# ayotoasset/AdditiveCausalExpansion

Measured on NVIDIA B200. Metric: nadam_iters_per_sec, higher is better.
Workload: dtype f64

## Files before the change

additivecausalexpansion_b200/_lib.py:

```python
from __future__ import annotations

import ctypes as C
import os
import subprocess

_HERE = os.path.dirname(os.path.abspath(__file__))
SO_PATH = os.environ.get("ACE_B200_LIB") or os.path.join(_HERE, "libace_b200.so")
CSRC = os.path.join(_HERE, "csrc")
HEADER = os.path.join(os.path.dirname(_HERE), "include", "ace_b200.h")

c_double_p = C.POINTER(C.c_double)
c_int_p = C.POINTER(C.c_int)


class AceFitConfig(C.Structure):

    _fields_ = [
        ("kernel", C.c_int),
        ("optimizer", C.c_int),
        ("learning_rate", C.c_double),
        ("beta1", C.c_double),
        ("beta2", C.c_double),
        ("momentum", C.c_double),
        ("norm_clip", C.c_int),
        ("clip_at", C.c_double),
        ("std_y", C.c_double),
        ("device", C.c_int),
        ("use_graph", C.c_int),
    ]


def build(force: bool = False, verbose: bool = False) -> str:
    srcs = [os.path.join(CSRC, f) for f in os.listdir(CSRC) if f.endswith((".cu", ".cuh", ".inl"))] + [HEADER]
    stale = (not os.path.exists(SO_PATH)) or any(os.path.getmtime(s) > os.path.getmtime(SO_PATH) for s in srcs)
    if force or stale:
        cmd = ["make", "-j", str(min(8, os.cpu_count() or 1)), "-C", CSRC, "../libace_b200.so"] + (["-B"] if force else [])
        subprocess.check_call(cmd, stdout=None if verbose else subprocess.DEVNULL)
    return SO_PATH


_LIB = None

_d, _i, _p, _ip = C.c_double, C.c_int, c_double_p, c_int_p
_vp = C.c_void_p
SIGNATURES = {
    "ace_last_error": (C.c_char_p, []),
    "ace_version": (C.c_char_p, []),
    "ace_device_count": (_i, []),
    "ace_set_device": (_i, [_i]),
    "ace_kernmat_SE_cpp": (_i, [_p, _p, _p, _p, _i, _i, _i, _i, _p, _p, _p]),
    "ace_kernmat_Matern32_cpp": (_i, [_p, _p, _p, _p, _i, _i, _i, _i, _p, _p, _p]),
    "ace_kernmat_SE_symmetric_cpp": (_i, [_p, _p, _i, _i, _i, _p, _p, _p]),
    "ace_kernmat_Matern32_symmetric_cpp": (_i, [_p, _p, _i, _i, _i, _p, _p, _p]),
    "ace_invkernel_cpp": (_i, [_p, _i, _d, _p, _p]),
    "ace_grad_SE_cpp": (_i, [_p, _p, _p, _p, _p, _p, _p, _p, _p, C.c_uint, _d, _i, _i, _p]),
    "ace_grad_Matern_cpp": (_i, [_p, _p, _p, _p, _p, _p, _p, _p, _p, C.c_uint, _d, _i, _i, _p]),
    "ace_stats_cpp": (_i, [_p, _p, _p, _p, _d, _d, _i, _p]),
    "ace_mu_solution_cpp": (_i, [_p, _p, _i, _p]),
    "ace_pred_cpp": (_i, [_p, _d, _d, _p, _p, _p, _d, _d, _i, _i, _p, _p, _p]),
    "ace_pred_marginal_cpp": (_i, [_p, _p, _d, _d, _p, _p, _p, _d, _d, _d, _i, _i, _i, _i, _p, _p, _p, _p]),
    "ace_norm_clip_cpp": (None, [_i, _p, _i, _d]),
    "ace_Nesterov_cpp": (_i, [_d, _d, _p, _p, _p, _i]),
    "ace_Nadam_cpp": (_i, [_d, _d, _d, _d, _d, _p, _p, _p, _p, _i]),
    "ace_Adam_cpp": (_i, [_d, _d, _d, _d, _d, _p, _p, _p, _p, _i]),
    "ace_fit_default_config": (None, [C.POINTER(AceFitConfig)]),
    "ace_fit_create": (_i, [C.POINTER(_vp), _p, _p, _p, _i, _i, _i, _p, C.POINTER(AceFitConfig)]),
    "ace_fit_destroy": (_i, [_vp]),
    "ace_fit_para_update": (_i, [_vp, _i, _p, _p]),
    "ace_fit_run": (_i, [_vp, _i, _i, _d, _d, _p, _ip]),
    "ace_fit_get_train_stats": (_i, [_vp, _p]),
    "ace_comm_unique_id": (_i, [C.c_char_p]),
    "ace_shard_plan": (_i, [_i, _i, _i, _ip, _ip]),
    "ace_fit_shard": (_i, [_vp, C.c_char_p, _i, _i]),
    "ace_fit_shard_emulate": (_i, [_vp, _i]),
    "ace_dbg_shard_trace_dump": (_i, [_i]),
    "ace_fit_upload_data": (_i, [_vp, _p, _p, _p]),
    "ace_fit_kernel_launches": (_i, [_vp, _ip]),
    "ace_fit_timer_start": (_i, [_vp]),
    "ace_fit_timer_stop": (_i, [_vp, _p]),
    "ace_fit_get_parameters": (_i, [_vp, _p]),
    "ace_fit_set_parameters": (_i, [_vp, _p]),
    "ace_fit_get_gradients": (_i, [_vp, _p]),
    "ace_fit_get_optimizer_state": (_i, [_vp, _p, _p]),
    "ace_fit_get_invKmatn": (_i, [_vp, _p]),
    "ace_fit_get_alpha": (_i, [_vp, _p]),
    "ace_fit_dims": (_i, [_vp, _ip, _ip, _ip, _ip]),
    "ace_fit_last_timing": (_i, [_vp, _p]),
    "ace_fit_predict": (_i, [_vp, _p, _p, _i, _d, _d, _p, _p, _p]),
    "ace_fit_predict_marginal": (_i, [_vp, _p, _p, _p, _i, _d, _d, _d, _i, _p, _p, _p, _p]),
    "ace_fit_predict_marginal_batch": (_i, [_vp, _p, _p, _p, _i, _d, _d, _d, C.POINTER(C.c_ubyte), _i, _p, _p, _p, _p, _ip]),
    "ace_dbg_gemm_nt": (_i, [_p, _p, _p, _i, _i, _i, _d, _d, _i]),
    "ace_dbg_spd_inverse": (_i, [_p, _i, _p, _p, _p, _p]),
    "ace_dbg_spd_inverse_fused": (_i, [_p, _i, _p, _p]),
    "ace_dbg_diag_block": (_i, [_p, _i, _p, _p, _p, _p]),
    "ace_dbg_diag_block_timeline": (_i, [C.POINTER(C.c_longlong), _i]),
    "ace_bench_dense": (_i, [_i, _i, _p]),
    "ace_dbg_set_trtri_max_h": (_i, [_i]),
    "ace_dbg_trtri_raw": (_i, [_p, _i, _p, _p, _p, _p]),
    "ace_dbg_uut_engines": (_i, [_p, _i, C.POINTER(C.c_int), _i, _p, _p, _p]),
    "ace_dbg_fit_set_uut_engine": (_i, [_vp, _i]),
    "ace_ncs_basis": (_i, [_p, _i, _p, _i, _p]),
    "ace_ncs_basis_deriv": (_i, [_p, _i, _p, _i, _p]),
    "ace_normalize_train": (_i, [_p, _p, _p, _i, _i, _i, _p]),
    "ace_normalize_test": (_i, [_p, _p, _i, _i, _i, _p]),
    "ace_normalize_train_gpu": (_i, [_p, _p, _p, _i, _i, _i, _p]),
    "ace_normalize_test_gpu": (_i, [_p, _p, _i, _i, _i, _p]),
}


def lib():
    global _LIB
    if _LIB is None:
        if not os.path.exists(SO_PATH):
            raise RuntimeError(
                f"{SO_PATH} is missing: run `python -c 'import __graft_entry__ as g; g.build()'` "
                "(there is no CPU fallback for the ACE hot path)")
        L = C.CDLL(SO_PATH)
        for name, (res, args) in SIGNATURES.items():
            fn = getattr(L, name)
            fn.restype = res
            fn.argtypes = args
        _LIB = L
    return _LIB


class AceError(RuntimeError):
    def __init__(self, status: int, where: str):
        self.status = status
        msg = lib().ace_last_error()
        super().__init__(f"{where}: status {status}: {msg.decode() if msg else ''}")


class NotFiniteError(AceError, FloatingPointError):
    """The reference's stop("Some gradients are not finite, NaN, or NA. ...")."""


ACE_ERR_NOT_FINITE = 1073741824


def check(status: int, where: str) -> None:
    if status == 0:
        return
    if status == ACE_ERR_NOT_FINITE:
        raise NotFiniteError(status, where)
    raise AceError(status, where)
```

additivecausalexpansion_b200/api.py:

```python
from __future__ import annotations

import ctypes as C

import numpy as np

from ._lib import AceError, c_double_p, check, lib


def _f(a, two_d=False):
    a = np.asfortranarray(np.asarray(a, dtype=np.float64))
    if two_d and a.ndim == 1:
        a = np.asfortranarray(a.reshape(-1, 1))
    return a


def _p(a):
    return None if a is None else a.ctypes.data_as(c_double_p)


def _inplace(a, name):
    if not (isinstance(a, np.ndarray) and a.dtype == np.float64 and a.flags.c_contiguous):
        raise TypeError(f"{name} must be a C-contiguous float64 ndarray (it is updated in place)")
    return a


def _kernmat(fn, name, X1, X2, Z1, Z2, parameters, elements=True):
    X1, X2, Z1, Z2 = _f(X1, True), _f(X2, True), _f(Z1, True), _f(Z2, True)
    par = _f(parameters).ravel()
    n1, n2, p, Bz = X1.shape[0], X2.shape[0], X2.shape[1], Z1.shape[1]
    full = np.empty((n1, n2), order="F")
    el = np.empty((n1, n2, Bz + 1), order="F") if elements else None
    check(fn(_p(X1), _p(X2), _p(Z1), _p(Z2), n1, n2, p, Bz, _p(par), _p(full), _p(el)), name)
    return {"full": full, "elements": el}


def _kernmat_sym(fn, name, X, Z, parameters, elements=True):
    X, Z = _f(X, True), _f(Z, True)
    par = _f(parameters).ravel()
    n, p, Bz = X.shape[0], X.shape[1], Z.shape[1]
    full = np.empty((n, n), order="F")
    el = np.empty((n, n, Bz + 1), order="F") if elements else None
    check(fn(_p(X), _p(Z), n, p, Bz, _p(par), _p(full), _p(el)), name)
    return {"full": full, "elements": el}


def kernmat_SE_cpp(X1, X2, Z1, Z2, parameters, elements=True):
    return _kernmat(lib().ace_kernmat_SE_cpp, "kernmat_SE_cpp", X1, X2, Z1, Z2, parameters, elements)


def kernmat_SE_symmetric_cpp(X, Z, parameters, elements=True):
    return _kernmat_sym(lib().ace_kernmat_SE_symmetric_cpp, "kernmat_SE_symmetric_cpp", X, Z, parameters, elements)


def kernmat_Matern32_cpp(X1, X2, Z1, Z2, parameters, elements=True):
    return _kernmat(lib().ace_kernmat_Matern32_cpp, "kernmat_Matern32_cpp", X1, X2, Z1, Z2, parameters, elements)


def kernmat_Matern32_symmetric_cpp(X, Z, parameters, elements=True):
    return _kernmat_sym(lib().ace_kernmat_Matern32_symmetric_cpp, "kernmat_Matern32_symmetric_cpp", X, Z,
                        parameters, elements)


def invkernel_cpp(pdmat, sigma):
    K = _f(pdmat)
    n = K.shape[0]
    eig = np.empty(n)
    inv = np.empty((n, n), order="F")
    check(lib().ace_invkernel_cpp(_p(K), n, float(sigma), _p(eig), _p(inv)), "invkernel_cpp")
    return {"eigenval": eig, "inv": inv}


def _grad(fn, name, y, X, Z, Kfull, K, invKmatn, eigenval, parameters, stats, B, std_y):
    y, X, Z = _f(y).ravel(), _f(X, True), _f(Z, True)
    invKmatn, eigenval, par = _f(invKmatn), _f(eigenval).ravel(), _f(parameters).ravel()
    _inplace(stats, "stats")
    n, p = X.shape
    g = np.empty(par.size)
    check(fn(_p(y), _p(X), _p(Z), None, None, _p(invKmatn), _p(eigenval), _p(par), _p(stats), int(B), float(std_y),
             n, p, _p(g)), name)
    return g


def grad_SE_cpp(y, X, Z, Kfull, K, invKmatn, eigenval, parameters, stats, B, std_y):
    return _grad(lib().ace_grad_SE_cpp, "grad_SE_cpp", y, X, Z, Kfull, K, invKmatn, eigenval, parameters, stats, B,
                 std_y)


def grad_Matern_cpp(y, X, Z, Kfull, K, invKmatn, eigenval, parameters, stats, B, std_y):
    return _grad(lib().ace_grad_Matern_cpp, "grad_Matern_cpp", y, X, Z, Kfull, K, invKmatn, eigenval, parameters,
                 stats, B, std_y)


def stats_cpp(y, Kmat, invKmatn, eigenval, mu, std_y=1.0):
    y, Kmat, invKmatn, eigenval = _f(y).ravel(), _f(Kmat), _f(invKmatn), _f(eigenval).ravel()
    out = np.zeros(2)
    check(lib().ace_stats_cpp(_p(y), _p(Kmat), _p(invKmatn), _p(eigenval), float(mu), float(std_y), y.size, _p(out)),
          "stats_cpp")
    return out


def mu_solution_cpp(y, invKmat):
    y, invKmat = _f(y).ravel(), _f(invKmat)
    mu = C.c_double(0.0)
    check(lib().ace_mu_solution_cpp(_p(y), _p(invKmat), y.size, C.cast(C.byref(mu), c_double_p)), "mu_solution_cpp")
    return mu.value


def norm_clip_cpp(flag, grads, max_length):
    _inplace(grads, "grads")
    lib().ace_norm_clip_cpp(int(bool(flag)), _p(grads), grads.size, float(max_length))


def Nesterov_cpp(learn_rate, momentum, nu, grad, para):
    _inplace(nu, "nu"), _inplace(para, "para")
    g = np.ascontiguousarray(grad, dtype=np.float64).ravel()
    return bool(lib().ace_Nesterov_cpp(float(learn_rate), float(momentum), _p(nu), _p(g), _p(para), para.size))


def Nadam_cpp(iter, learn_rate, beta1, beta2, eps, m, v, grad, para):
    _inplace(m, "m"), _inplace(v, "v"), _inplace(para, "para")
    g = np.ascontiguousarray(grad, dtype=np.float64).ravel()
    return bool(lib().ace_Nadam_cpp(float(iter), float(learn_rate), float(beta1), float(beta2), float(eps), _p(m),
                                    _p(v), _p(g), _p(para), para.size))


def Adam_cpp(iter, learn_rate, beta1, beta2, eps, m, v, grad, para):
    _inplace(m, "m"), _inplace(v, "v"), _inplace(para, "para")
    g = np.ascontiguousarray(grad, dtype=np.float64).ravel()
    return bool(lib().ace_Adam_cpp(float(iter), float(learn_rate), float(beta1), float(beta2), float(eps), _p(m),
                                   _p(v), _p(g), _p(para), para.size))


def pred_cpp(y_X, sigma, mu, invK_XX, K_xX, K_xx, mean_y, std_y):
    y_X, invK_XX, K_xX, K_xx = _f(y_X).ravel(), _f(invK_XX), _f(K_xX, True), _f(K_xx, True)
    nx, nX = K_xX.shape
    m, ci, var = np.empty(nx), np.empty((nx, 2), order="F"), np.empty(nx)
    check(lib().ace_pred_cpp(_p(y_X), float(sigma), float(mu), _p(invK_XX), _p(K_xX), _p(K_xx), float(mean_y),
                             float(std_y), nx, nX, _p(m), _p(ci), _p(var)), "pred_cpp")
    return {"map": m, "ci": ci, "var": var}


def _avg(out, avg):
    for k, name in enumerate(("ate", "att", "atu")):
        out[name] = {"map": avg[4 * k], "ci": avg[4 * k + 1:4 * k + 3].copy(), "var": avg[4 * k + 3]}


def pred_marginal_cpp(y_X, Z_x, sigma, mu, invK_XX, K_xX, K_xx, mean_y, std_y, std_Z, calculate_ate):
    y_X, Z_x, invK_XX = _f(y_X).ravel(), _f(Z_x).ravel(), _f(invK_XX)
    K_xX, K_xx = _f(K_xX), _f(K_xx)
    nx, nX, B = K_xX.shape
    m, ci, var, avg = np.empty(nx), np.empty((nx, 2), order="F"), np.empty(nx), np.zeros(12)
    check(lib().ace_pred_marginal_cpp(_p(y_X), _p(Z_x), float(sigma), float(mu), _p(invK_XX), _p(K_xX), _p(K_xx),
                                      float(mean_y), float(std_y), float(std_Z), int(bool(calculate_ate)), nx, nX, B,
                                      _p(m), _p(ci), _p(var), _p(avg)), "pred_marginal_cpp")
    out = {"map": m, "ci": ci, "var": var}
    if calculate_ate:
        _avg(out, avg)
    return out


def ncs_basis(x, knots):
    x, knots = _f(x).ravel(), _f(knots).ravel()
    K = lib().ace_ncs_basis(_p(x), x.size, _p(knots), knots.size, None)
    check(0 if K > 0 else K, "ncs_basis")
    out = np.empty((x.size, K), order="F")
    lib().ace_ncs_basis(_p(x), x.size, _p(knots), knots.size, _p(out))
    return out


def ncs_basis_deriv(x, knots):
    x, knots = _f(x).ravel(), _f(knots).ravel()
    K = lib().ace_ncs_basis_deriv(_p(x), x.size, _p(knots), knots.size, None)
    check(0 if K > 0 else K, "ncs_basis_deriv")
    out = np.empty((x.size, K), order="F")
    lib().ace_ncs_basis_deriv(_p(x), x.size, _p(knots), knots.size, _p(out))
    return out


def normalize_train(y, X, Z, gpu=False):
    for a, nm in ((y, "y"), (X, "X"), (Z, "Z")):
        if not (isinstance(a, np.ndarray) and a.dtype == np.float64 and a.flags.f_contiguous):
            raise TypeError(f"{nm} must be a Fortran-contiguous float64 ndarray (normalised in place)")
    n, px = X.shape
    pz = Z.shape[1]
    mom = np.empty((1 + px + pz, 3), order="F")
    fn = lib().ace_normalize_train_gpu if gpu else lib().ace_normalize_train
    check(fn(_p(y), _p(X), _p(Z), n, px, pz, _p(mom)), "normalize_train")
    return mom


def normalize_test(X, Z, moments, gpu=False):
    for a, nm in ((X, "X"), (Z, "Z")):
        if not (isinstance(a, np.ndarray) and a.dtype == np.float64 and a.flags.f_contiguous):
            raise TypeError(f"{nm} must be a Fortran-contiguous float64 ndarray (normalised in place)")
    mom = _f(moments)
    fn = lib().ace_normalize_test_gpu if gpu else lib().ace_normalize_test
    check(fn(_p(X), _p(Z), X.shape[0], X.shape[1], Z.shape[1], _p(mom)), "normalize_test")


def dbg_gemm_nt(A, B, C_, alpha=1.0, beta=0.0, lower_only=False):
    A, B, Cm = _f(A), _f(B), _f(C_).copy(order="F")
    M, K = A.shape
    N = B.shape[0]
    check(lib().ace_dbg_gemm_nt(_p(A), _p(B), _p(Cm), M, N, K, float(alpha), float(beta), int(lower_only)),
          "dbg_gemm_nt")
    return Cm


def dbg_spd_inverse(A, want_L=True, want_inv=True):
    A = _f(A)
    n = A.shape[0]
    L = np.empty((n, n), order="F") if want_L else None
    inv = np.empty((n, n), order="F") if want_inv else None
    d = np.empty(n)
    ms = np.zeros(3)
    check(lib().ace_dbg_spd_inverse(_p(A), n, _p(L), _p(inv), _p(d), _p(ms)), "dbg_spd_inverse")
    return {"L": L, "inv": inv, "diagL": d, "ms": ms}


def dbg_spd_inverse_fused(A):
    A = _f(A)
    n = A.shape[0]
    inv, d = np.empty((n, n), order="F"), np.empty(n)
    check(lib().ace_dbg_spd_inverse_fused(_p(A), n, _p(inv), _p(d)), "dbg_spd_inverse_fused")
    return {"inv": inv, "diagL": d}


def dbg_uut_engines(A, engines=(1, 2), want_inv=True):
    A = _f(A)
    n = A.shape[0]
    eng = (C.c_int * len(engines))(*engines)
    ms = np.zeros(len(engines))
    inv = {e: (np.empty((n, n), order="F") if want_inv and e in engines else None) for e in (1, 2)}
    check(lib().ace_dbg_uut_engines(_p(A), n, eng, len(engines), _p(ms), _p(inv[1]), _p(inv[2])),
          "dbg_uut_engines")
    return {"ms": ms, "dmma": inv[1], "i8": inv[2]}


def dbg_diag_block(A):
    A = _f(A)
    n = A.shape[0]
    X, U, L = (np.empty((n, n), order="F") for _ in range(3))
    d = np.empty(n)
    check(lib().ace_dbg_diag_block(_p(A), n, _p(X), _p(U), _p(d), _p(L)), "dbg_diag_block")
    return {"X": X, "U": U, "diagL": d, "Ldiag": L}


def bench_dense(n, reps=1):
    ms = np.zeros(3)
    check(lib().ace_bench_dense(int(n), int(reps), _p(ms)), "bench_dense")
    return ms
```

additivecausalexpansion_b200/csrc/ace_b200.cu:

```cuda
#include "../../include/ace_b200.h"

#include <algorithm>
#include <chrono>
#include <cmath>
#include <cstdlib>
#include <cstring>
#include <mutex>
#include <new>
#include <string>
#include <vector>

#include "chol.cuh"
#include "nccl_dyn.h"
#include "shard_dense.cuh"
#include "gp_kernels.cuh"
#include "pair_kernels.cuh"
#include "grad2_kernel.cuh"
#include "grad3_kernel.cuh"
#include "kernmat2_kernel.cuh"
#include "pred_kernels.cuh"
#include "prep_kernels.cuh"

namespace ace {

static thread_local std::string g_err;
void set_error(const std::string& msg) { g_err = msg; }

static int usage(const std::string& m) {
  set_error(m);
  return ACE_ERR_USAGE;
}

static inline int round_up(int x, int m) { return (x + m - 1) / m * m; }

template <typename T>
struct DBuf {
  T* p = nullptr;
  size_t count = 0;
  DBuf() = default;
  DBuf(const DBuf&) = delete;
  DBuf& operator=(const DBuf&) = delete;
  ~DBuf() { release(); }
  int alloc(size_t n) {
    release();
    if (n == 0) n = 1;
    cudaError_t e = cudaMalloc(&p, n * sizeof(T));
    if (e != cudaSuccess) {
      p = nullptr;
      set_error(std::string("cudaMalloc of ") + std::to_string(n * sizeof(T)) + " bytes: " + cudaGetErrorString(e));
      return -(int)e - 1000;
    }
    count = n;
    return 0;
  }
  void release() {
    if (p) cudaFree(p);
    p = nullptr;
    count = 0;
  }
};

static int check_device() {
  int cnt = 0;
  cudaError_t e = cudaGetDeviceCount(&cnt);
  if (e != cudaSuccess || cnt <= 0) {
    set_error(std::string("no CUDA device available (") + cudaGetErrorString(e) +
              "); this library has no CPU fallback");
    return ACE_ERR_NO_DEVICE;
  }
  return 0;
}

static int configure_kernels_once() {
  static std::mutex mu;
  static std::vector<int> done;
  int dev = 0;
  ACE_CUDA(cudaGetDevice(&dev));
  std::lock_guard<std::mutex> lk(mu);
  if (std::find(done.begin(), done.end(), dev) != done.end()) return 0;
  ACE_TRY(configure_dense_kernels());
  done.push_back(dev);
  return 0;
}

static int upload_matrix(double* dst, long ld_dev, int rows_pad, const double* src, int rows, int cols,
                         cudaStream_t st) {
  ACE_CUDA(cudaMemsetAsync(dst, 0, sizeof(double) * (size_t)ld_dev * (size_t)std::max(cols, 1), st));
  (void)rows_pad;
  if (rows > 0 && cols > 0)
    ACE_CUDA(cudaMemcpy2DAsync(dst, sizeof(double) * ld_dev, src, sizeof(double) * rows, sizeof(double) * rows,
                               cols, cudaMemcpyHostToDevice, st));
  return 0;
}

static int download_matrix(double* dst, int rows, int cols, const double* src, long ld_dev, cudaStream_t st) {
  if (rows > 0 && cols > 0)
    ACE_CUDA(cudaMemcpy2DAsync(dst, sizeof(double) * rows, src, sizeof(double) * ld_dev, sizeof(double) * rows,
                               cols, cudaMemcpyDeviceToHost, st));
  return 0;
}

__global__ void pad_identity_kernel(double* A, long ld, int n, int n_pad) {
  const int i = n + blockIdx.x * blockDim.x + threadIdx.x;
  if (i < n_pad) A[i + (size_t)i * ld] = 1.0;
}

__global__ void add_diag_kernel(double* A, long ld, int n, double v) {
  const int i = blockIdx.x * blockDim.x + threadIdx.x;
  if (i < n) A[i + (size_t)i * ld] += v;
}

__global__ void synth_spd_kernel(double* A, long ld, int n) {
  const size_t idx = (size_t)blockIdx.x * blockDim.x + threadIdx.x;
  if (idx >= (size_t)n * n) return;
  const int i = (int)(idx % n), j = (int)(idx / n);
  const double t = 8.0 * (double)(i - j) / (double)n;
  A[i + (size_t)j * ld] = exp(-t * t) + (i == j ? 0.5 : 0.0);
}

struct ConstChain {
  std::mutex mu;
  cudaEvent_t ev = nullptr;
  bool recorded = false;
};
static ConstChain& const_chain(int which, int dev) {
  static ConstChain chains[2][64];
  return chains[which][dev & 63];
}
template <class F>
static int with_const_chain(int which, cudaStream_t st, F&& launch) {
  int dev = 0;
  ACE_CUDA(cudaGetDevice(&dev));
  ConstChain& ch = const_chain(which, dev);
  std::lock_guard<std::mutex> lk(ch.mu);
  if (ch.ev == nullptr) ACE_CUDA(cudaEventCreateWithFlags(&ch.ev, cudaEventDisableTiming));
  cudaStreamCaptureStatus cs = cudaStreamCaptureStatusNone;
  ACE_CUDA(cudaStreamIsCapturing(st, &cs));
  const bool cap = cs != cudaStreamCaptureStatusNone;
  if (ch.recorded) ACE_CUDA(cudaStreamWaitEvent(st, ch.ev, cap ? cudaEventWaitExternal : cudaEventWaitDefault));
  ACE_TRY(launch());
  ACE_CUDA(cudaEventRecordWithFlags(ch.ev, st, cap ? cudaEventRecordExternal : cudaEventRecordDefault));
  ch.recorded = true;
  return 0;
}

int launch_kernmat2_k0(const KernArgs&, unsigned, size_t, cudaStream_t);
int launch_kernmat2_k1(const KernArgs&, unsigned, size_t, cudaStream_t);

static int launch_kernmat(const KernArgs& a, int kind, cudaStream_t st) {
  const int B = a.B;
  if (B < 1 || B > BMAXT || a.p < 1 || a.p > PMAX) {
    set_error("kernel build supports 1 <= p <= 64 and B = Bz+1 <= 32");
    return ACE_ERR_UNSUPPORTED;
  }
  const size_t smem = kb::smem_bytes(a.p, B - 1, a.sym != 0);
  if (smem > 227 * 1024) {
    set_error("kernel build: p and Bz too large for one shared-memory tile");
    return ACE_ERR_UNSUPPORTED;
  }
  unsigned grid;
  if (a.sym) {
    const long T = a.n1_pad / kb::T;
    grid = (unsigned)(T * (T + 1) / 2);
  } else {
    grid = (unsigned)((a.n1_pad / kb::T) * (a.n2_pad / kb::T));
  }
  static const int impl = [] {
    const char* e = std::getenv("ACE_KERNMAT_IMPL");
    return e ? std::atoi(e) : 2;
  }();
  if (impl == 2 && B <= G3_LAM && a.p <= G3_PD) {
    const size_t smem2 = kb2::smem_bytes(a.p, B - 1, a.sym != 0);
    return with_const_chain(1, st, [&]() -> int {
      return kind == 0 ? launch_kernmat2_k0(a, grid, smem2, st) : launch_kernmat2_k1(a, grid, smem2, st);
    });
  }
  auto go = [&](auto kern) -> int {
    ACE_CUDA(cudaFuncSetAttribute(kern, cudaFuncAttributeMaxDynamicSharedMemorySize, (int)smem));
    kern<<<grid, 256, smem, st>>>(a);
    return 0;
  };
  const int bc = kb::chunk_terms(B);
  if (kind == 0) {
    if (bc == 4) ACE_TRY(go(kernmat_kernel<0, 4, 4>));
    else if (bc == 8) ACE_TRY(go(kernmat_kernel<0, 8, 2>));
    else ACE_TRY(go(kernmat_kernel<0, 12, 2>));
  } else {
    if (bc == 4) ACE_TRY(go(kernmat_kernel<1, 4, 4>));
    else if (bc == 8) ACE_TRY(go(kernmat_kernel<1, 8, 2>));
    else ACE_TRY(go(kernmat_kernel<1, 12, 2>));
  }
  ACE_CUDA(cudaGetLastError());
  return 0;
}

struct GradPlan {
  int PD = 0, BT = 0, groups = 0, gy = 0, threads = 0, gx = 0;
  size_t smem = 0;
  int v2 = 0, PD8 = 0, BD8 = 0;
  int nw2 = 8;
  int cw3 = 1;
  int v3 = 0, NT3 = 0;
};

int launch_grad3_k0_nt1(const GradArgs&, int, size_t, int, cudaStream_t);
int launch_grad3_k0_nt2(const GradArgs&, int, size_t, int, cudaStream_t);
int launch_grad3_k0_nt3(const GradArgs&, int, size_t, int, cudaStream_t);
int launch_grad3_k0_nt4(const GradArgs&, int, size_t, int, cudaStream_t);
int launch_grad3_k1_nt1(const GradArgs&, int, size_t, int, cudaStream_t);
int launch_grad3_k1_nt2(const GradArgs&, int, size_t, int, cudaStream_t);
int launch_grad3_k1_nt3(const GradArgs&, int, size_t, int, cudaStream_t);
int launch_grad3_k1_nt4(const GradArgs&, int, size_t, int, cudaStream_t);

static int plan_grad(int p, int B, int kind, int sms, GradPlan* pl) {
  static const int table[][2] = {{4, 16}, {8, 8}, {12, 5}, {16, 4}, {20, 3}, {24, 2}, {32, 2}, {48, 1}, {64, 1}};
  for (auto& t : table) {
    if (p <= t[0]) {
      pl->PD = t[0];
      pl->BT = t[1];
      break;
    }
  }
  if (pl->PD == 0 || B > BMAXT) {
    set_error("gradient pass supports p <= 64 and B <= 32");
    return ACE_ERR_UNSUPPORTED;
  }
  int gpc_max = gk::GROUPS_PER_CTA;
  if (pl->PD == 20) {
    if (const char* e = std::getenv("ACE_GRAD_BT")) pl->BT = (std::atoi(e) == 2) ? 2 : 3;
  }
  if (const char* e = std::getenv("ACE_GRAD_GPC")) gpc_max = std::max(1, std::min(4, std::atoi(e)));
  pl->groups = (B + pl->BT - 1) / pl->BT;
  const int gpc = std::min(pl->groups, gpc_max);
  pl->gy = (pl->groups + gpc - 1) / gpc;
  pl->threads = 64 * gpc;
  pl->smem = gk::smem_bytes(pl->PD, B - 1, pl->BT, kind);
  if (pl->smem > 227 * 1024) {
    set_error("gradient pass: p and Bz too large for one shared-memory tile");
    return ACE_ERR_UNSUPPORTED;
  }
  pl->gx = 2 * sms;
  const int PD8 = (p + 7) / 8 * 8, BD8 = (B + 7) / 8 * 8;
  const char* impl = std::getenv("ACE_GRAD_IMPL");
  const int want = impl ? std::atoi(impl) : 3;
  const bool want2 = want >= 2;
  if (want == 3 && p <= 32 && B <= 16) {
    const int NT = (p + 7) / 8;
    const size_t sm3 = g3::smem_bytes(NT, B, kind, 16);
    if (sm3 <= 227 * 1024) {
      pl->v3 = 1; pl->NT3 = NT; pl->smem = sm3; pl->gy = 1; pl->threads = 512;
      if (const char* e = std::getenv("ACE_GRAD3_CW")) pl->cw3 = std::atoi(e) != 0;
      return 0;
    }
  }
  if (PD8 <= 32 && BD8 <= 16 && want2) {
    int nw = 16;
    if (const char* e = std::getenv("ACE_GRAD2_WARPS")) nw = (std::atoi(e) == 8) ? 8 : 16;
    size_t sm2 = g2::smem_bytes(PD8, BD8, B - 1, nw, kind);
    if (sm2 > 227 * 1024 && nw == 16) {
      nw = 8;
      sm2 = g2::smem_bytes(PD8, BD8, B - 1, nw, kind);
    }
    if (sm2 <= 227 * 1024) {
      pl->v2 = 1; pl->PD8 = PD8; pl->BD8 = BD8; pl->smem = sm2; pl->gy = 1; pl->threads = 32 * nw; pl->nw2 = nw;
    }
  }
  return 0;
}

template <int PD8, int BD8, int KIND, int NW>
static int launch_grad2_k(const GradArgs& a, const GradPlan& pl, cudaStream_t st) {
  ACE_CUDA(cudaFuncSetAttribute(grad2_kernel<PD8, BD8, KIND, NW>, cudaFuncAttributeMaxDynamicSharedMemorySize, (int)pl.smem));
  grad2_kernel<PD8, BD8, KIND, NW><<<pl.gx, NW * 32, pl.smem, st>>>(a);
  ACE_CUDA(cudaGetLastError());
  return 0;
}

template <int PD8, int BD8>
static int launch_grad2_t(const GradArgs& a, int kind, const GradPlan& pl, cudaStream_t st) {
  if (pl.nw2 == 16) return kind == 0 ? launch_grad2_k<PD8, BD8, 0, 16>(a, pl, st) : launch_grad2_k<PD8, BD8, 1, 16>(a, pl, st);
  return kind == 0 ? launch_grad2_k<PD8, BD8, 0, 8>(a, pl, st) : launch_grad2_k<PD8, BD8, 1, 8>(a, pl, st);
}

static int launch_grad2(const GradArgs& a, int kind, const GradPlan& pl, cudaStream_t st) {
  const int key = pl.PD8 * 100 + pl.BD8;
  switch (key) {
    case 808: return launch_grad2_t<8, 8>(a, kind, pl, st);
    case 816: return launch_grad2_t<8, 16>(a, kind, pl, st);
    case 1608: return launch_grad2_t<16, 8>(a, kind, pl, st);
    case 1616: return launch_grad2_t<16, 16>(a, kind, pl, st);
    case 2408: return launch_grad2_t<24, 8>(a, kind, pl, st);
    case 2416: return launch_grad2_t<24, 16>(a, kind, pl, st);
    case 3208: return launch_grad2_t<32, 8>(a, kind, pl, st);
    default: return launch_grad2_t<32, 16>(a, kind, pl, st);
  }
}

template <int PD, int BT>
static int launch_grad_t(const GradArgs& a, int kind, const GradPlan& pl, cudaStream_t st) {
  dim3 grid(pl.gx, pl.gy);
  if (kind == 0) {
    ACE_CUDA(cudaFuncSetAttribute(grad_kernel<PD, BT, 0>, cudaFuncAttributeMaxDynamicSharedMemorySize, (int)pl.smem));
    grad_kernel<PD, BT, 0><<<grid, pl.threads, pl.smem, st>>>(a);
  } else {
    ACE_CUDA(cudaFuncSetAttribute(grad_kernel<PD, BT, 1>, cudaFuncAttributeMaxDynamicSharedMemorySize, (int)pl.smem));
    grad_kernel<PD, BT, 1><<<grid, pl.threads, pl.smem, st>>>(a);
  }
  ACE_CUDA(cudaGetLastError());
  return 0;
}

static int launch_grad2(const GradArgs& a, int kind, const GradPlan& pl, cudaStream_t st);

static int launch_grad(const GradArgs& a, int kind, const GradPlan& pl, cudaStream_t st) {
  if (pl.v3) {
    auto go = [&](int cw) -> int {
      switch (kind * 10 + pl.NT3) {
        case 1: return launch_grad3_k0_nt1(a, pl.gx, pl.smem, cw, st);
        case 2: return launch_grad3_k0_nt2(a, pl.gx, pl.smem, cw, st);
        case 3: return launch_grad3_k0_nt3(a, pl.gx, pl.smem, cw, st);
        case 4: return launch_grad3_k0_nt4(a, pl.gx, pl.smem, cw, st);
        case 11: return launch_grad3_k1_nt1(a, pl.gx, pl.smem, cw, st);
        case 12: return launch_grad3_k1_nt2(a, pl.gx, pl.smem, cw, st);
        case 13: return launch_grad3_k1_nt3(a, pl.gx, pl.smem, cw, st);
        default: return launch_grad3_k1_nt4(a, pl.gx, pl.smem, cw, st);
      }
    };
    if (!pl.cw3) return go(0);
    return with_const_chain(0, st, [&]() -> int { return go(1); });
  }
  if (pl.v2) return launch_grad2(a, kind, pl, st);
  switch (pl.PD) {
    case 4: return launch_grad_t<4, 16>(a, kind, pl, st);
    case 8: return launch_grad_t<8, 8>(a, kind, pl, st);
    case 12: return launch_grad_t<12, 5>(a, kind, pl, st);
    case 16: return launch_grad_t<16, 4>(a, kind, pl, st);
    case 20: return pl.BT == 2 ? launch_grad_t<20, 2>(a, kind, pl, st) : launch_grad_t<20, 3>(a, kind, pl, st);
    case 24: return launch_grad_t<24, 2>(a, kind, pl, st);
    case 32: return launch_grad_t<32, 2>(a, kind, pl, st);
    case 48: return launch_grad_t<48, 1>(a, kind, pl, st);
    default: return launch_grad_t<64, 1>(a, kind, pl, st);
  }
}

struct Core {
  int device = 0, sms = 148;
  int n = 0, n_pad = 0, p = 0, Bz = 0, B = 0, P = 0, kind = 0;
  cudaStream_t st = nullptr, side = nullptr, aux = nullptr, bgst = nullptr;
  cudaEvent_t ev[8] = {nullptr, nullptr, nullptr, nullptr, nullptr, nullptr, nullptr, nullptr};
  DBuf<double> Wp0, Wp1, Wsmall;
  DBuf<double> diag_ws;
  DBuf<int8_t> oz_planes;
  DBuf<unsigned long long> oz_rowmax;
  DBuf<int> oz_ex;
  int uut_engine = 0;
  int panel_blocks = 4;
  cudaEvent_t tev[8] = {};
  DBuf<double> X, Z, LZ, y, theta, m, v, grad, tab, sc, A, Bf, DX, DU, dvec, alpha, uvec, svec, Ka, pu, ps, partials;
  DBuf<int> info;
  double* h_sc = nullptr;
  GradPlan gp;
  int nchunks = 0;
  int shard_rank = 0, shard_world = 1;
  DBuf<double> red;
  double* ka() { return red.p ? red.p + P : Ka.p; }
  bool shard_dense = false;
  bool shard_emulate = false;
  int shard_hmin = 16;
  bool kinv_partial = false;
  bool u_valid = false;
  DBuf<double> tvy, tv1, pdg, kdg;
  bool shard_incr = true;
  bool shard_potrf = false;
  std::vector<cudaEvent_t> shard_events;
  DBuf<double> head0, head1;
  cudaStream_t bulk = nullptr;
  int rank_lo() const { return shard_emulate ? 0 : shard_rank; }
  int rank_hi() const { return shard_emulate ? shard_world : shard_rank + 1; }
  DBuf<double> chain_ws;
  DBuf<double> mid0, mid1;
  cudaStream_t mids = nullptr;
  ShardCtx shard_ctx(ncclComm_t comm, ncclComm_t comm2, ncclComm_t comm3 = nullptr) const {
    ShardCtx cx;
    cx.rank = shard_rank; cx.world = shard_world; cx.emulate = shard_emulate; cx.comm = comm; cx.h_min = shard_hmin;
    cx.comm2 = comm2;
    cx.events = const_cast<cudaEvent_t*>(shard_events.data());
    cx.head[0] = head0.p; cx.head[1] = head1.p; cx.bulk_stream = bulk;
    cx.chain_ws = chain_ws.p;
    cx.comm3 = comm3; cx.mid[0] = mid0.p; cx.mid[1] = mid1.p; cx.mid_stream = mids;
    cx.incr = shard_incr;
    return cx;
  }
  int alloc_shard() {
    ACE_TRY(red.alloc((size_t)P + n_pad));
    ACE_CUDA(cudaMemsetAsync(red.p, 0, sizeof(double) * ((size_t)P + n_pad), st));
    const char* e = std::getenv("ACE_SHARD_DENSE");
    shard_dense = e ? (std::atoi(e) != 0) : true;
    if (const char* h = std::getenv("ACE_SHARD_HMIN")) shard_hmin = std::max(1, std::atoi(h));
    if (shard_dense) {
      const char* sp = std::getenv("ACE_SHARD_POTRF");
      const bool pow2 = (panel_blocks & (panel_blocks - 1)) == 0;
      if ((sp ? std::atoi(sp) != 0 : true) && pow2 && panel_blocks >= 2) {
        const size_t N = (size_t)n_pad;
        if (!Wp0.p) {
          ACE_TRY(Wp0.alloc(N * panel_blocks * TB));
          ACE_TRY(Wp1.alloc(N * panel_blocks * TB));
          ACE_TRY(Wsmall.alloc((size_t)(panel_blocks * TB / 2) * (panel_blocks * TB / 2)));
        }
        const size_t pw = (size_t)panel_blocks * TB;
        ACE_TRY(head0.alloc(2 * pw * pw));
        ACE_TRY(head1.alloc(2 * pw * pw));
        if (!bulk) {
          int lo = 0, hi = 0;
          ACE_CUDA(cudaDeviceGetStreamPriorityRange(&lo, &hi));
          int pb_ = (hi + lo) / 2;
          if (const char* e = std::getenv("ACE_SHARD_BULK_PRIO")) pb_ = std::max(hi, std::min(lo, std::atoi(e)));
          ACE_CUDA(cudaStreamCreateWithPriority(&bulk, cudaStreamNonBlocking, pb_));
        }
        {
          const char* sk = std::getenv("ACE_SHARD_SPLITK");
          if (!(sk && std::atoi(sk) == 0)) ACE_TRY(chain_ws.alloc(4 * pw * pw));
        }
        {
          const char* sm = std::getenv("ACE_SHARD_MID");
          if (!(sm && std::atoi(sm) == 0)) {
            ACE_TRY(mid0.alloc(pw * pw));
            ACE_TRY(mid1.alloc(pw * pw));
            if (!mids) {
              int lo = 0, hi = 0;
              ACE_CUDA(cudaDeviceGetStreamPriorityRange(&lo, &hi));
              ACE_CUDA(cudaStreamCreateWithPriority(&mids, cudaStreamNonBlocking, std::min(lo, hi + 1)));
            }
          }
        }
        const int NP = shard_panels(n_pad / TB, panel_blocks);
        while ((int)shard_events.size() < SHARD_EVENT_KINDS * NP) {
          cudaEvent_t e;
          ACE_CUDA(cudaEventCreateWithFlags(&e, cudaEventDisableTiming));
          shard_events.push_back(e);
        }
        shard_potrf = true;
        {
          const double nn = (double)n_pad;
          const double chain_s = NP * 0.85e-3, update_s = nn * nn * nn / (3.0 * shard_world * 3.5e13);
          shard_incr = 2.0 * chain_s >= update_s;
        }
        if (const char* si = std::getenv("ACE_SHARD_INCR")) shard_incr = std::atoi(si) != 0;
      }
    }
    return 0;
  }
  int ensure_full_inverse() {
    if (!kinv_partial) return 0;
    DenseWork w = dense(A.p, Bf.p);
    ACE_TRY(uut_inverse(w));
    kinv_partial = false;
    return 0;
  }

  ~Core() {
    if (h_sc) cudaFreeHost(h_sc);
    for (auto& e : ev)
      if (e) cudaEventDestroy(e);
    for (auto& e : tev)
      if (e) cudaEventDestroy(e);
    for (auto& e : shard_events) cudaEventDestroy(e);
    if (bulk) cudaStreamDestroy(bulk);
    if (mids) cudaStreamDestroy(mids);
    if (st) cudaStreamDestroy(st);
    if (side) cudaStreamDestroy(side);
    if (aux) cudaStreamDestroy(aux);
    if (bgst) cudaStreamDestroy(bgst);
  }

  int init(int dev, int n_, int p_, int Bz_, int kind_, bool need_dense, bool need_grad) {
    ACE_TRY(check_device());
    device = dev;
    ACE_CUDA(cudaSetDevice(dev));
    ACE_TRY(configure_kernels_once());
    cudaDeviceProp prop;
    ACE_CUDA(cudaGetDeviceProperties(&prop, dev));
    if (prop.major < 10) {
      set_error("this library is built for sm_100a (B200) only");
      return ACE_ERR_NO_DEVICE;
    }
    sms = prop.multiProcessorCount;
    n = n_; p = p_; Bz = Bz_; B = Bz_ + 1; P = 2 + B + B * p; kind = kind_;
    n_pad = round_up(n, TB);
    ACE_CUDA(cudaStreamCreateWithFlags(&st, cudaStreamNonBlocking));
    int lo = 0, hi = 0;
    ACE_CUDA(cudaDeviceGetStreamPriorityRange(&lo, &hi));
    ACE_CUDA(cudaStreamCreateWithPriority(&side, cudaStreamNonBlocking, hi));
    ACE_CUDA(cudaStreamCreateWithPriority(&aux, cudaStreamNonBlocking, lo));
    ACE_CUDA(cudaStreamCreateWithPriority(&bgst, cudaStreamNonBlocking, lo));
    for (auto& e : ev) ACE_CUDA(cudaEventCreateWithFlags(&e, cudaEventDisableTiming));
    for (auto& e : tev) ACE_CUDA(cudaEventCreate(&e));
    ACE_CUDA(cudaMallocHost(&h_sc, sizeof(double) * (SC_COUNT + 2)));
    const size_t N = (size_t)n_pad;
    ACE_TRY(X.alloc(N * p));
    ACE_TRY(Z.alloc(N * std::max(Bz, 1)));
    ACE_TRY(LZ.alloc(N * std::max(Bz, 1)));
    ACE_TRY(y.alloc(N));
    ACE_TRY(theta.alloc(P));
    ACE_TRY(m.alloc(P));
    ACE_TRY(v.alloc(P));
    ACE_TRY(grad.alloc(P));
    ACE_TRY(tab.alloc(TAB_SIZE));
    ACE_TRY(sc.alloc(SC_COUNT));
    ACE_TRY(info.alloc(1));
    ACE_CUDA(cudaMemsetAsync(sc.p, 0, sizeof(double) * SC_COUNT, st));
    ACE_CUDA(cudaMemsetAsync(m.p, 0, sizeof(double) * P, st));
    ACE_CUDA(cudaMemsetAsync(v.p, 0, sizeof(double) * P, st));
    ACE_CUDA(cudaMemsetAsync(grad.p, 0, sizeof(double) * P, st));
    ACE_CUDA(cudaMemsetAsync(info.p, 0, sizeof(int), st));
    if (need_dense) {
      ACE_TRY(A.alloc(N * N));
      ACE_TRY(Bf.alloc(N * N));
      ACE_TRY(DX.alloc(N * TB));
      ACE_TRY(DU.alloc(N * TB));
      ACE_TRY(dvec.alloc(N));
      if (const char* e = std::getenv("ACE_PANEL_BLOCKS")) {
        const int v = std::atoi(e);
        if (v >= 1 && v <= 64) panel_blocks = v;
      }
      const char* fu = std::getenv("ACE_FUSED_TRSM");
      const bool pow2 = (panel_blocks & (panel_blocks - 1)) == 0;
      const bool want = fu ? (std::atoi(fu) != 0) : true;
      ACE_TRY(alloc_uut_engine());
      if (pow2 && panel_blocks >= 2 && want) {
        ACE_TRY(Wp0.alloc(N * panel_blocks * TB));
        ACE_TRY(Wp1.alloc(N * panel_blocks * TB));
        ACE_TRY(Wsmall.alloc((size_t)(panel_blocks * TB / 2) * (panel_blocks * TB / 2)));
        const char* df = std::getenv("ACE_DIAG_FUSED");
        if (!(df && std::atoi(df) == 0)) ACE_TRY(diag_ws.alloc(dg::ws_doubles(panel_blocks)));
      }
    }
    if (need_grad) {
      ACE_TRY(plan_grad(p, B, kind, sms, &gp));
      nchunks = (n + gv::CHUNK - 1) / gv::CHUNK;
      ACE_TRY(alpha.alloc(N));
      ACE_TRY(uvec.alloc(N));
      ACE_TRY(svec.alloc(N));
      ACE_TRY(Ka.alloc(N));
      ACE_TRY(pu.alloc(N * nchunks));
      ACE_TRY(ps.alloc(N * nchunks));
      ACE_TRY(partials.alloc((size_t)gp.gx * gp.gy * P));
      if (!dvec.p) ACE_TRY(dvec.alloc(N));
      ACE_TRY(tvy.alloc(N));
      ACE_TRY(tv1.alloc(N));
      ACE_TRY(pdg.alloc(N * nchunks));
      ACE_TRY(kdg.alloc(N));
    }
    return 0;
  }

  int alloc_uut_engine() {
    if (uut_engine == 2 && n_pad > oz::MAX_N) {
      set_error("the INT8 U U^T engine covers n_pad <= " + std::to_string(oz::MAX_N) + " (INT32 accumulator bound)");
      return ACE_ERR_UNSUPPORTED;
    }
    if (!uut_uses_i8(n_pad, uut_engine)) {
      oz_planes.release();
      oz_rowmax.release();
      oz_ex.release();
      return 0;
    }
    if (oz_planes.p) return 0;
    ACE_TRY(oz_planes.alloc(oz::plane_bytes(n_pad / TB)));
    ACE_TRY(oz_rowmax.alloc(n_pad));
    ACE_TRY(oz_ex.alloc(n_pad));
    return 0;
  }

  int upload_data(const double* hy, const double* hX, const double* hZ) {
    if (hX) ACE_TRY(upload_matrix(X.p, n_pad, n_pad, hX, n, p, st));
    if (hZ) {
      ACE_TRY(upload_matrix(Z.p, n_pad, n_pad, hZ, n, Bz, st));
      const size_t cnt = (size_t)n_pad * Bz;
      if (cnt) logabs_kernel<<<(unsigned)((cnt + 255) / 256), 256, 0, st>>>(Z.p, LZ.p, cnt);
      ACE_CUDA(cudaGetLastError());
    }
    if (hy) ACE_TRY(upload_matrix(y.p, n_pad, n_pad, hy, n, 1, st));
    return 0;
  }

  int upload_theta(const double* hpar) {
    ACE_CUDA(cudaMemcpyAsync(theta.p, hpar, sizeof(double) * P, cudaMemcpyHostToDevice, st));
    return 0;
  }

  DenseWork dense(double* Abuf, double* Bbuf, bool allow_fused = true) {
    DenseWork w;
    w.panel_blocks = panel_blocks;
    if (allow_fused && Wp0.p) {
      w.Wp[0] = Wp0.p; w.Wp[1] = Wp1.p; w.Wsmall = Wsmall.p; w.ev_copy[0] = ev[6]; w.ev_copy[1] = ev[7];
      w.diag_ws = diag_ws.p;
    }
    w.A = Abuf; w.ld = n_pad; w.nb = n_pad / TB; w.DX = DX.p; w.DU = DU.p; w.dvec = dvec.p; w.info = info.p;
    w.Bf = Bbuf; w.main = st; w.side = side; w.aux = aux; w.bg = bgst; w.ev_half = ev[4]; w.ev_aux = ev[5];
    w.ev_panel[0] = ev[0]; w.ev_panel[1] = ev[1]; w.ev_upd[0] = ev[2]; w.ev_upd[1] = ev[3];
    w.oz.planes = oz_planes.p; w.oz.rowmax = oz_rowmax.p; w.oz.ex = oz_ex.p; w.uut_engine = uut_engine;

    return w;
  }

  int enqueue_prep() {
    prep_tables_kernel<<<1, 256, 0, st>>>(theta.p, p, B, tab.p);
    ACE_CUDA(cudaGetLastError());
    return 0;
  }

  int enqueue_build_sym(double* out, int add_noise, double* cube, long cube_slice) {
    KernArgs a{};
    a.X1 = a.X2 = X.p; a.Z1 = a.Z2 = Z.p; a.LZ1 = a.LZ2 = LZ.p; a.ld1 = a.ld2 = n_pad;
    a.n1 = a.n2 = n; a.n1_pad = a.n2_pad = n_pad; a.p = p; a.B = B; a.tab = tab.p;
    a.K = out; a.ldk = n_pad; a.cube = cube; a.cube_slice = cube_slice;
    a.sym = 1; a.add_noise = add_noise; a.pad_identity = add_noise;
    return launch_kernmat(a, kind, st);
  }

  int enqueue_build_blocks(double* out) {
    const int w = shard_block_width(n_pad, shard_world);
    for (int blk = 0; blk < 2 * shard_world; ++blk) {
      const int owner = shard_block_owner(blk, shard_world);
      if (owner < rank_lo() || owner >= rank_hi()) continue;
      const int c0 = blk * w, r0 = c0;
      KernArgs a{};
      a.X1 = X.p + r0; a.Z1 = Z.p + r0; a.LZ1 = LZ.p + r0; a.ld1 = n_pad;
      a.X2 = X.p + c0; a.Z2 = Z.p + c0; a.LZ2 = LZ.p + c0; a.ld2 = n_pad;
      a.n1 = std::max(0, n - r0); a.n2 = std::max(0, std::min(w, n - c0));
      a.n1_pad = n_pad - r0; a.n2_pad = w; a.p = p; a.B = B; a.tab = tab.p;
      a.K = out + r0 + (size_t)c0 * n_pad; a.ldk = n_pad;
      a.sym = 0; a.add_noise = 1; a.pad_identity = 1; a.row_off = r0; a.col_off = c0;
      ACE_TRY(launch_kernmat(a, kind, st));
    }
    return 0;
  }

  int enqueue_build_panels(double* out) {
    const int nb = n_pad / TB, NP = shard_panels(nb, panel_blocks);
    for (int c = 0; c < NP; ++c) {
      if (!(shard_emulate || c % shard_world == shard_rank)) continue;
      const int c0 = c * panel_blocks * TB, w = std::min(panel_blocks * TB, n_pad - c0), r0 = c0;
      KernArgs a{};
      a.X1 = X.p + r0; a.Z1 = Z.p + r0; a.LZ1 = LZ.p + r0; a.ld1 = n_pad;
      a.X2 = X.p + c0; a.Z2 = Z.p + c0; a.LZ2 = LZ.p + c0; a.ld2 = n_pad;
      a.n1 = std::max(0, n - r0); a.n2 = std::max(0, std::min(w, n - c0));
      a.n1_pad = n_pad - r0; a.n2_pad = w; a.p = p; a.B = B; a.tab = tab.p;
      a.K = out + r0 + (size_t)c0 * n_pad; a.ldk = n_pad;
      a.sym = 0; a.add_noise = 1; a.pad_identity = 1; a.row_off = r0; a.col_off = c0;
      ACE_TRY(launch_kernmat(a, kind, st));
    }
    return 0;
  }

  int enqueue_alpha(const double* Kinv, int set_mu_first_iter) {
    dim3 grid((n_pad + gv::ROWS - 1) / gv::ROWS, nchunks);
    gemv2_kernel<<<grid, gv::ROWS, 0, st>>>(Kinv, n_pad, n, y.p, pu.p, ps.p, n_pad);
    ACE_CUDA(cudaGetLastError());
    alpha_kernel<<<1, 1024, 0, st>>>(pu.p, ps.p, nchunks, n, n_pad, theta.p, uvec.p, svec.p, alpha.p, ka(), sc.p,
                                     set_mu_first_iter);
    ACE_CUDA(cudaGetLastError());
    return 0;
  }

  int enqueue_alpha_tri(const double* Afac, int set_mu_first_iter, const double* DUfac = nullptr) {
    if (!DUfac) DUfac = DU.p;
    utv2_kernel<<<(n_pad + 7) / 8, 256, 0, st>>>(Afac, n_pad, DUfac, n, n_pad, y.p, tvy.p, tv1.p);
    ACE_CUDA(cudaGetLastError());
    dim3 grid((n_pad + gv::ROWS - 1) / gv::ROWS, nchunks);
    uv2_kernel<<<grid, gv::ROWS, 0, st>>>(Afac, n_pad, DUfac, n_pad, tvy.p, tv1.p, pu.p, ps.p, pdg.p);
    ACE_CUDA(cudaGetLastError());
    alpha_kernel<<<1, 1024, 0, st>>>(pu.p, ps.p, nchunks, n, n_pad, theta.p, uvec.p, svec.p, alpha.p, ka(), sc.p,
                                     set_mu_first_iter, pdg.p, kdg.p);
    ACE_CUDA(cudaGetLastError());
    return 0;
  }

  bool alpha_from_factor() const { return uut_uses_i8(n_pad, uut_engine); }
  int enqueue_alpha_any(const double* Afac, int set_mu_first_iter, const double* DUfac = nullptr,
                        const double* Kinv = nullptr) {
    if (alpha_from_factor()) return enqueue_alpha_tri(Afac, set_mu_first_iter, DUfac);
    return enqueue_alpha(Kinv ? Kinv : Bf.p, set_mu_first_iter);
  }

  int enqueue_grad(const double* Kinv, int tile_rank = 0, int tile_world = 1, int tile_mode = 0) {
    GradArgs g{};
    g.X = X.p; g.Z = Z.p; g.LZ = LZ.p; g.ldx = n_pad; g.Kinv = Kinv; g.ld = n_pad; g.alpha = alpha.p; g.Ka = ka();
    g.tab = tab.p; g.partials = partials.p; g.n = n; g.p = p; g.B = B; g.P = P;
    g.ntiles_side = (n + gk::T - 1) / gk::T;
    g.tile_rank = tile_rank; g.tile_world = tile_world; g.tile_mode = tile_mode; g.gemm_rows = n_pad / TB;
    return launch_grad(g, kind, gp, st);
  }

  int enqueue_finalize(const double* Kinv, const ace_fit_config& c, int do_update, bool reduced = false,
                       const double* kdiag = nullptr, const double* dvec_alt = nullptr) {
    FinalizeArgs f{};
    f.partials = partials.p; f.nparts = gp.gx * gp.gy; f.y = y.p; f.alpha = alpha.p; f.Ka = ka();
    f.dvec = dvec_alt ? dvec_alt : dvec.p;
    if (reduced) {
      f.partials = red.p;
      f.nparts = 1;
    }
    f.kdiag = kdiag;
    f.Kinv = Kinv; f.ld = n_pad; f.tab = tab.p; f.theta = theta.p; f.m = m.p; f.v = v.p; f.grad = grad.p; f.sc = sc.p;
    f.n = n; f.p = p; f.B = B; f.P = P; f.kind = kind; f.optimizer = c.optimizer; f.lr = c.learning_rate;
    f.beta1 = c.beta1; f.beta2 = c.beta2; f.eps = 1e-8; f.momentum = c.momentum; f.std_y = c.std_y;
    f.clip_at = c.clip_at; f.norm_clip = c.norm_clip; f.do_update = do_update;
    finalize_kernel<<<1, 1024, 0, st>>>(f);
    ACE_CUDA(cudaGetLastError());
    return 0;
  }

  int fetch_scalars() {
    ACE_CUDA(cudaMemcpyAsync(h_sc, sc.p, sizeof(double) * SC_COUNT, cudaMemcpyDeviceToHost, st));
    ACE_CUDA(cudaMemcpyAsync(h_sc + SC_COUNT, info.p, sizeof(int), cudaMemcpyDeviceToHost, st));
    ACE_CUDA(cudaStreamSynchronize(st));
    return 0;
  }
  int h_info() const { return *reinterpret_cast<const int*>(h_sc + SC_COUNT); }
};

}

using namespace ace;

struct ace_fit {
  Core c;
  ace_fit_config cfg;
  cudaEvent_t sw0 = nullptr, sw1 = nullptr;
  int launches = -1;
  cudaGraph_t graph = nullptr;
  cudaGraphExec_t gexec = nullptr;
  double iter_dev = 0.0;
  double ms[6] = {0, 0, 0, 0, 0, 0};
  ncclComm_t comm = nullptr, comm2 = nullptr, comm3 = nullptr;
  ~ace_fit() {
    if (comm2 && nccl_api().ok) nccl_api().CommDestroy(comm2);
    if (comm3 && nccl_api().ok) nccl_api().CommDestroy(comm3);
    if (comm && nccl_api().ok) nccl_api().CommDestroy(comm);
    if (sw0) cudaEventDestroy(sw0);
    if (sw1) cudaEventDestroy(sw1);
    if (gexec) cudaGraphExecDestroy(gexec);
    if (graph) cudaGraphDestroy(graph);
  }
};

static int enqueue_iteration(ace_fit* f, bool timed) {
  Core& c = f->c;
  DenseWork w = c.dense(c.A.p, c.Bf.p);
  if (timed) ACE_CUDA(cudaEventRecord(c.tev[0], c.st));
  ACE_TRY(c.enqueue_prep());
  const bool sharded = c.shard_world > 1;
  const bool comm = sharded && !c.shard_emulate;
  const bool spotrf = sharded && c.shard_dense && c.shard_potrf;
  if (!sharded) {
    ACE_TRY(c.enqueue_build_sym(c.A.p, 1, nullptr, 0));
  } else if (spotrf) {
    ACE_TRY(c.enqueue_build_panels(c.A.p));
  } else {
    ACE_TRY(c.enqueue_build_blocks(c.A.p));
    if (comm) {
      NcclApi& nc = nccl_api();
      const int wdt = shard_block_width(c.n_pad, c.shard_world);
      const size_t cnt = (size_t)wdt * c.n_pad;
      ACE_NCCL(nc.GroupStart());
      for (int blk = 0; blk < 2 * c.shard_world; ++blk) {
        double* ptr = c.A.p + (size_t)blk * cnt;
        ACE_NCCL(nc.Broadcast(ptr, ptr, cnt, ncclFloat64, shard_block_owner(blk, c.shard_world), f->comm, c.st));
      }
      ACE_NCCL(nc.GroupEnd());
    }
  }
  if (timed) ACE_CUDA(cudaEventRecord(c.tev[1], c.st));
  const bool sdense = sharded && c.shard_dense;
  if (!sdense) {
    ACE_TRY(potrf_trtri(w));
    if (timed) ACE_CUDA(cudaEventRecord(c.tev[2], c.st));
    if (timed) ACE_CUDA(cudaEventRecord(c.tev[3], c.st));
    ACE_TRY(uut_inverse(w));
    if (timed) ACE_CUDA(cudaEventRecord(c.tev[4], c.st));
    ACE_TRY(c.enqueue_alpha_any(c.A.p, 1));
  } else {
    const ShardCtx cx = c.shard_ctx(f->comm, f->comm2, f->comm3);
    if (spotrf) {
      static const bool host_time = std::getenv("ACE_SHARD_HOSTTIME") != nullptr;
      const auto h0 = std::chrono::steady_clock::now();
      ACE_TRY(potrf_sharded(w, cx));
      if (host_time)
        std::fprintf(stderr, "[rank %d] potrf_sharded: host enqueue %.3f ms\n", c.shard_rank,
                     std::chrono::duration<double, std::milli>(std::chrono::steady_clock::now() - h0).count());
    } else {
      const int s = potrf_blocked(w);
      if (s < 0) return s;
    }
    if (timed) ACE_CUDA(cudaEventRecord(c.tev[2], c.st));
    if (spotrf && cx.incr)
      ACE_TRY(gather_inverse_sharded(w, cx));
    else
      ACE_TRY(trtri_merge_sharded(w, cx));
    if (timed) ACE_CUDA(cudaEventRecord(c.tev[3], c.st));
    ACE_TRY(uut_inverse_sharded(w, cx));
    if (timed) ACE_CUDA(cudaEventRecord(c.tev[4], c.st));
    ACE_TRY(c.enqueue_alpha_tri(c.A.p, 1));
  }
  if (!sharded) {
    ACE_TRY(c.enqueue_grad(c.Bf.p));
  } else {
    for (int r = c.rank_lo(); r < c.rank_hi(); ++r) {
      ACE_TRY(c.enqueue_grad(c.Bf.p, r, c.shard_world, sdense ? 1 : 0));
      partials_reduce_kernel<<<1, 1024, 0, c.st>>>(c.partials.p, c.gp.gx * c.gp.gy, c.P, c.red.p, r > c.rank_lo());
      ACE_CUDA(cudaGetLastError());
    }
    if (comm)
      ACE_NCCL(nccl_api().AllReduce(c.red.p, c.red.p, (size_t)c.P + c.n_pad, ncclFloat64, ncclSum, f->comm, c.st));
  }
  ACE_TRY(c.enqueue_finalize(c.Bf.p, f->cfg, 1, sharded, (sdense || c.alpha_from_factor()) ? c.kdg.p : nullptr));
  if (timed) ACE_CUDA(cudaEventRecord(c.tev[5], c.st));
  return 0;
}

extern "C" {

const char* ace_last_error(void) { return g_err.c_str(); }
const char* ace_version(void) { return "ace_b200 0.1 (sm_100a; FP64 DMMA; TMA bulk)"; }

int ace_device_count(void) {
  int cnt = 0;
  if (cudaGetDeviceCount(&cnt) != cudaSuccess) {
    cudaGetLastError();
    return 0;
  }
  return cnt;
}

static thread_local int g_device = 0;
int ace_set_device(int device) {
  ACE_TRY(check_device());
  ACE_CUDA(cudaSetDevice(device));
  g_device = device;
  return 0;
}

void ace_fit_default_config(ace_fit_config* cfg) {
  cfg->kernel = ACE_KERNEL_SE;
  cfg->optimizer = ACE_OPT_NADAM;
  cfg->learning_rate = 0.01;
  cfg->beta1 = 0.9;
  cfg->beta2 = 0.999;
  cfg->momentum = 0.0;
  cfg->norm_clip = 1;
  cfg->clip_at = 1.0;
  cfg->std_y = 1.0;
  cfg->device = 0;
  cfg->use_graph = 1;
}

int ace_fit_create(ace_fit** out, const double* y, const double* X, const double* Z, int n, int p, int Bz,
                   const double* parameters, const ace_fit_config* cfg) {
  if (!out || !y || !X || (Bz > 0 && !Z) || !parameters || !cfg) return usage("ace_fit_create: null argument");
  if (n < 1 || p < 1 || Bz < 0) return usage("ace_fit_create: need n >= 1, p >= 1, Bz >= 0");
  *out = nullptr;
  ace_fit* f = new (std::nothrow) ace_fit();
  if (!f) return usage("out of host memory");
  f->cfg = *cfg;
  int s = f->c.init(cfg->device, n, p, Bz, cfg->kernel, true, true);
  if (s == 0) s = f->c.upload_data(y, X, Z);
  if (s == 0) s = f->c.upload_theta(parameters);
  if (s == 0) {
    cudaError_t e = cudaStreamSynchronize(f->c.st);
    if (e != cudaSuccess) {
      set_error(std::string("ace_fit_create: ") + cudaGetErrorString(e));
      s = -(int)e - 1000;
    }
  }
  if (s != 0) {
    delete f;
    return s;
  }
  *out = f;
  return 0;
}

int ace_fit_destroy(ace_fit* fit) {
  if (!fit) return 0;
  cudaSetDevice(fit->c.device);
  cudaDeviceSynchronize();
  delete fit;
  return 0;
}

int ace_fit_para_update(ace_fit* f, int iter, double* stats, double* gnorm) {
  if (!f) return usage("null handle");
  Core& c = f->c;
  ACE_CUDA(cudaSetDevice(c.device));
  if ((double)iter != f->iter_dev) {
    c.h_sc[SC_COUNT + 1] = (double)iter;
    ACE_CUDA(cudaMemcpyAsync(c.sc.p + SC_ITER, c.h_sc + SC_COUNT + 1, sizeof(double), cudaMemcpyHostToDevice, c.st));
    f->iter_dev = (double)iter;
  }
  const bool use_graph = f->cfg.use_graph && !(c.shard_world > 1 && !c.shard_emulate);
  if (use_graph) {
    if (!f->gexec) {
      ACE_CUDA(cudaStreamBeginCapture(c.st, cudaStreamCaptureModeThreadLocal));
      int s = enqueue_iteration(f, false);
      cudaGraph_t g = nullptr;
      cudaError_t e = cudaStreamEndCapture(c.st, &g);
      if (s != 0) {
        if (g) cudaGraphDestroy(g);
        return s;
      }
      ACE_CUDA(e);
      f->graph = g;
      ACE_CUDA(cudaGraphInstantiate(&f->gexec, f->graph, 0));
    }
    ACE_CUDA(cudaEventRecord(c.tev[6], c.st));
    ACE_CUDA(cudaGraphLaunch(f->gexec, c.st));
    ACE_CUDA(cudaEventRecord(c.tev[7], c.st));
  } else {
    ACE_CUDA(cudaEventRecord(c.tev[6], c.st));
    ACE_TRY(enqueue_iteration(f, true));
    ACE_CUDA(cudaEventRecord(c.tev[7], c.st));
  }
  c.u_valid = true;
  c.kinv_partial = c.shard_world > 1 && c.shard_dense && !c.shard_emulate;
  ACE_TRY(c.fetch_scalars());
  f->iter_dev = c.h_sc[SC_ITER];
  float t = 0;
  ACE_CUDA(cudaEventElapsedTime(&t, c.tev[6], c.tev[7]));
  f->ms[5] = t;
  if (!use_graph) {
    for (int k = 0; k < 5; ++k) {
      ACE_CUDA(cudaEventElapsedTime(&t, c.tev[k], c.tev[k + 1]));
      f->ms[k] = t;
    }
  }
  if (stats) {
    stats[0] = c.h_sc[SC_RMSE];
    stats[1] = c.h_sc[SC_EVID];
  }
  if (gnorm) *gnorm = c.h_sc[SC_GNORM];
  if (c.h_info() > 0) {
    set_error("matrix not positive definite at pivot " + std::to_string(c.h_info()));
    return c.h_info();
  }
  if (c.h_sc[SC_FINITE] == 0.0) {
    set_error("Some gradients are not finite, NaN, or NA. Often this is due to too large learning rates.");
    return ACE_ERR_NOT_FINITE;
  }
  return 0;
}

int ace_fit_run(ace_fit* f, int iter_start, int max_iter, double tol, double prev_evidence, double* stats_out,
                int* iters_done) {
  if (!f || !iters_done) return usage("null argument");
  double prev = prev_evidence;
  int done = 0;
  for (int k = 0; k < max_iter; ++k) {
    const int iter = iter_start + k;
    double st[2];
    int s = ace_fit_para_update(f, iter, st, nullptr);
    if (s != 0) {
      *iters_done = done;
      return s;
    }
    ++done;
    if (stats_out) {
      stats_out[2 * k] = st[0];
      stats_out[2 * k + 1] = st[1];
    }
    const double change = std::fabs(st[1] - prev);
    prev = st[1];
    if (change < tol && iter > 3) break;
  }
  *iters_done = done;
  return 0;
}

int ace_dbg_fit_set_uut_engine(ace_fit* f, int engine) {
  if (!f) return usage("null handle");
  if (engine < 0 || engine > 2) return usage("dbg_fit_set_uut_engine: engine must be 0 (by size), 1 (DMMA) or 2 (INT8)");
  Core& c = f->c;
  ACE_CUDA(cudaSetDevice(c.device));
  ACE_CUDA(cudaStreamSynchronize(c.st));
  c.uut_engine = engine;
  ACE_TRY(c.alloc_uut_engine());
  if (f->gexec) cudaGraphExecDestroy(f->gexec);
  if (f->graph) cudaGraphDestroy(f->graph);
  f->gexec = nullptr;
  f->graph = nullptr;
  return 0;
}

int ace_fit_get_train_stats(ace_fit* f, double* stats) {
  if (!f || !stats) return usage("null argument");
  Core& c = f->c;
  ACE_CUDA(cudaSetDevice(c.device));
  DBuf<double> B2, DX2, DU2, dv2;
  ACE_TRY(B2.alloc((size_t)c.n_pad * c.n_pad));
  double* Fac = c.Bf.p;
  DenseWork w = c.dense(Fac, B2.p);
  if (c.u_valid) {
    ACE_TRY(DX2.alloc((size_t)c.n_pad * TB));
    ACE_TRY(DU2.alloc((size_t)c.n_pad * TB));
    ACE_TRY(dv2.alloc(c.n_pad));
    w.DX = DX2.p; w.DU = DU2.p; w.dvec = dv2.p;
    c.kinv_partial = true;
  } else {
    Fac = c.A.p;
    w = c.dense(Fac, B2.p);
  }
  ACE_TRY(c.enqueue_prep());
  ACE_TRY(c.enqueue_build_sym(Fac, 1, nullptr, 0));
  ACE_TRY(spd_inverse(w));
  ACE_TRY(c.enqueue_alpha_any(Fac, 0, w.DU, B2.p));
  ACE_TRY(c.enqueue_grad(B2.p));
  ACE_TRY(c.enqueue_finalize(B2.p, f->cfg, 0, false, c.alpha_from_factor() ? c.kdg.p : nullptr, w.dvec));
  ACE_TRY(c.fetch_scalars());
  stats[0] = c.h_sc[SC_RMSE];
  stats[1] = c.h_sc[SC_EVID];
  if (c.h_info() > 0) return c.h_info();
  return 0;
}

int ace_comm_unique_id(char* id128) {
  if (!id128) return usage("null argument");
  NcclApi& nc = nccl_api();
  if (!nc.ok) {
    set_error(nc.why);
    return ACE_ERR_UNSUPPORTED;
  }
  ncclUniqueId id;
  ACE_NCCL(nc.GetUniqueId(&id));
  static_assert(sizeof(id) == 128, "ncclUniqueId is 128 bytes");
  std::memcpy(id128, &id, 128);
  return 0;
}

int ace_shard_plan(int n, int world, int rank, int* blocks2, int* width) {
  if (!blocks2 || !width || world < 1 || rank < 0 || rank >= world) return usage("ace_shard_plan: bad argument");
  const int n_pad = round_up(n, TB);
  *width = shard_block_width(n_pad, world);
  if (*width == 0) {
    set_error("sharding needs ceil(n/128)*128 divisible by 128*world");
    return ACE_ERR_UNSUPPORTED;
  }
  blocks2[0] = rank;
  blocks2[1] = 2 * world - 1 - rank;
  return 0;
}

int ace_fit_shard(ace_fit* f, const char* id128, int rank, int world) {
  if (!f || !id128 || world < 1 || rank < 0 || rank >= world) return usage("ace_fit_shard: bad argument");
  if (world == 1) return 0;
  Core& c = f->c;
  ACE_CUDA(cudaSetDevice(c.device));
  if (shard_block_width(c.n_pad, world) == 0) {
    set_error("sharding needs ceil(n/128)*128 divisible by 128*world");
    return ACE_ERR_UNSUPPORTED;
  }
  NcclApi& nc = nccl_api();
  if (!nc.ok) {
    set_error(nc.why);
    return ACE_ERR_UNSUPPORTED;
  }
  ncclUniqueId id;
  std::memcpy(&id, id128, 128);
  ACE_NCCL(nc.CommInitRank(&f->comm, world, id, rank));
  {
    ncclUniqueId id2;
    DBuf<double> box;
    ACE_TRY(box.alloc(16));
    if (rank == 0) {
      ACE_NCCL(nc.GetUniqueId(&id2));
      ACE_CUDA(cudaMemcpyAsync(box.p, &id2, 128, cudaMemcpyHostToDevice, c.st));
    }
    ACE_NCCL(nc.Broadcast(box.p, box.p, 16, ncclFloat64, 0, f->comm, c.st));
    ACE_CUDA(cudaMemcpyAsync(&id2, box.p, 128, cudaMemcpyDeviceToHost, c.st));
    ACE_CUDA(cudaStreamSynchronize(c.st));
    ACE_NCCL(nc.CommInitRank(&f->comm2, world, id2, rank));
  }
  {
    ncclUniqueId id3;
    DBuf<double> box;
    ACE_TRY(box.alloc(16));
    if (rank == 0) {
      ACE_NCCL(nc.GetUniqueId(&id3));
      ACE_CUDA(cudaMemcpyAsync(box.p, &id3, 128, cudaMemcpyHostToDevice, c.st));
    }
    ACE_NCCL(nc.Broadcast(box.p, box.p, 16, ncclFloat64, 0, f->comm, c.st));
    ACE_CUDA(cudaMemcpyAsync(&id3, box.p, 128, cudaMemcpyDeviceToHost, c.st));
    ACE_CUDA(cudaStreamSynchronize(c.st));
    ACE_NCCL(nc.CommInitRank(&f->comm3, world, id3, rank));
  }
  c.shard_rank = rank;
  c.shard_world = world;
  ACE_TRY(c.alloc_shard());
  if (f->gexec) {
    cudaGraphExecDestroy(f->gexec);
    cudaGraphDestroy(f->graph);
    f->gexec = nullptr;
    f->graph = nullptr;
  }
  f->launches = -1;
  return 0;
}

int ace_fit_shard_emulate(ace_fit* f, int world) {
  if (!f || world < 1) return usage("ace_fit_shard_emulate: bad argument");
  Core& c = f->c;
  if (world == 1) return 0;
  ACE_CUDA(cudaSetDevice(c.device));
  if (shard_block_width(c.n_pad, world) == 0) {
    set_error("sharding needs ceil(n/128)*128 divisible by 128*world");
    return ACE_ERR_UNSUPPORTED;
  }
  c.shard_rank = 0;
  c.shard_world = world;
  c.shard_emulate = true;
  ACE_TRY(c.alloc_shard());
  if (f->gexec) {
    cudaGraphExecDestroy(f->gexec);
    cudaGraphDestroy(f->graph);
    f->gexec = nullptr;
    f->graph = nullptr;
  }
  f->launches = -1;
  return 0;
}

int ace_dbg_shard_trace_dump(int rank) {
  shard_trace_dump(rank);
  return 0;
}

int ace_fit_upload_data(ace_fit* f, const double* y, const double* X, const double* Z) {
  if (!f) return usage("null handle");
  ACE_CUDA(cudaSetDevice(f->c.device));
  return f->c.upload_data(y, X, Z);
}

static int count_kernel_nodes(cudaGraph_t g, int* out) {
  size_t nn = 0;
  ACE_CUDA(cudaGraphGetNodes(g, nullptr, &nn));
  std::vector<cudaGraphNode_t> nodes(nn);
  if (nn) ACE_CUDA(cudaGraphGetNodes(g, nodes.data(), &nn));
  int k = 0;
  for (size_t i = 0; i < nn; ++i) {
    cudaGraphNodeType t;
    ACE_CUDA(cudaGraphNodeGetType(nodes[i], &t));
    if (t == cudaGraphNodeTypeKernel) ++k;
  }
  *out = k;
  return 0;
}

int ace_fit_kernel_launches(ace_fit* f, int* launches) {
  if (!f || !launches) return usage("null argument");
  Core& c = f->c;
  ACE_CUDA(cudaSetDevice(c.device));
  if (f->launches < 0) {
    if (f->graph) {
      ACE_TRY(count_kernel_nodes(f->graph, &f->launches));
    } else {
      ACE_CUDA(cudaStreamBeginCapture(c.st, cudaStreamCaptureModeThreadLocal));
      int s = enqueue_iteration(f, false);
      cudaGraph_t g = nullptr;
      cudaError_t e = cudaStreamEndCapture(c.st, &g);
      if (s != 0 || e != cudaSuccess) {
        if (g) cudaGraphDestroy(g);
        return s != 0 ? s : -(int)e - 1000;
      }
      s = count_kernel_nodes(g, &f->launches);
      cudaGraphDestroy(g);
      ACE_TRY(s);
    }
  }
  *launches = f->launches;
  return 0;
}

int ace_fit_timer_start(ace_fit* f) {
  if (!f) return usage("null handle");
  ACE_CUDA(cudaSetDevice(f->c.device));
  if (!f->sw0) {
    ACE_CUDA(cudaEventCreate(&f->sw0));
    ACE_CUDA(cudaEventCreate(&f->sw1));
  }
  ACE_CUDA(cudaEventRecord(f->sw0, f->c.st));
  return 0;
}

int ace_fit_timer_stop(ace_fit* f, double* ms) {
  if (!f || !ms || !f->sw0) return usage("timer not started");
  ACE_CUDA(cudaSetDevice(f->c.device));
  ACE_CUDA(cudaEventRecord(f->sw1, f->c.st));
  ACE_CUDA(cudaEventSynchronize(f->sw1));
  float t = 0;
  ACE_CUDA(cudaEventElapsedTime(&t, f->sw0, f->sw1));
  *ms = t;
  return 0;
}

int ace_fit_get_parameters(ace_fit* f, double* par) {
  if (!f || !par) return usage("null argument");
  ACE_CUDA(cudaSetDevice(f->c.device));
  ACE_CUDA(cudaMemcpyAsync(par, f->c.theta.p, sizeof(double) * f->c.P, cudaMemcpyDeviceToHost, f->c.st));
  ACE_CUDA(cudaStreamSynchronize(f->c.st));
  return 0;
}

int ace_fit_set_parameters(ace_fit* f, const double* par) {
  if (!f || !par) return usage("null argument");
  ACE_CUDA(cudaSetDevice(f->c.device));
  ACE_TRY(f->c.upload_theta(par));
  ACE_CUDA(cudaStreamSynchronize(f->c.st));
  return 0;
}

int ace_fit_get_gradients(ace_fit* f, double* g) {
  if (!f || !g) return usage("null argument");
  ACE_CUDA(cudaSetDevice(f->c.device));
  ACE_CUDA(cudaMemcpyAsync(g, f->c.grad.p, sizeof(double) * f->c.P, cudaMemcpyDeviceToHost, f->c.st));
  ACE_CUDA(cudaStreamSynchronize(f->c.st));
  return 0;
}

int ace_fit_get_optimizer_state(ace_fit* f, double* m, double* v) {
  if (!f) return usage("null argument");
  ACE_CUDA(cudaSetDevice(f->c.device));
  if (m) ACE_CUDA(cudaMemcpyAsync(m, f->c.m.p, sizeof(double) * f->c.P, cudaMemcpyDeviceToHost, f->c.st));
  if (v) ACE_CUDA(cudaMemcpyAsync(v, f->c.v.p, sizeof(double) * f->c.P, cudaMemcpyDeviceToHost, f->c.st));
  ACE_CUDA(cudaStreamSynchronize(f->c.st));
  return 0;
}

int ace_fit_get_invKmatn(ace_fit* f, double* inv) {
  if (!f || !inv) return usage("null argument");
  ACE_CUDA(cudaSetDevice(f->c.device));
  ACE_TRY(f->c.ensure_full_inverse());
  ACE_TRY(download_matrix(inv, f->c.n, f->c.n, f->c.Bf.p, f->c.n_pad, f->c.st));
  ACE_CUDA(cudaStreamSynchronize(f->c.st));
  return 0;
}

int ace_fit_get_alpha(ace_fit* f, double* a) {
  if (!f || !a) return usage("null argument");
  ACE_CUDA(cudaSetDevice(f->c.device));
  ACE_CUDA(cudaMemcpyAsync(a, f->c.alpha.p, sizeof(double) * f->c.n, cudaMemcpyDeviceToHost, f->c.st));
  ACE_CUDA(cudaStreamSynchronize(f->c.st));
  return 0;
}

int ace_fit_dims(ace_fit* f, int* n, int* p, int* B, int* P) {
  if (!f) return usage("null argument");
  if (n) *n = f->c.n;
  if (p) *p = f->c.p;
  if (B) *B = f->c.B;
  if (P) *P = f->c.P;
  return 0;
}

int ace_fit_last_timing(ace_fit* f, double* ms6) {
  if (!f || !ms6) return usage("null argument");
  for (int k = 0; k < 6; ++k) ms6[k] = f->ms[k];
  return 0;
}

}

namespace ace {

struct PostOut {
  DBuf<double> T, map, var, p1, p2;
};

static int posterior_rows(Core& c, const double* Kinv, const double* Kx, const double* kdiag, int nx, int nx_pad,
                          double mu, double noise, PostOut& o) {
  const int n = c.n, n_pad = c.n_pad;
  ACE_TRY(o.T.alloc((size_t)nx_pad * n_pad));
  GemmNT g{};
  g.A = Kx; g.lda = nx_pad; g.B = Kinv; g.ldb = n_pad; g.C = o.T.p; g.ldc = nx_pad;
  g.M = nx_pad; g.N = n_pad; g.K = n_pad; g.alpha = 1.0; g.beta = 0.0;
  ACE_TRY(launch_gemm_nt(g, c.st));
  const int chunks = (n + pk::CHUNK - 1) / pk::CHUNK;
  ACE_TRY(o.p1.alloc((size_t)nx_pad * chunks));
  ACE_TRY(o.p2.alloc((size_t)nx_pad * chunks));
  ACE_TRY(o.map.alloc(nx_pad));
  ACE_TRY(o.var.alloc(nx_pad));
  dim3 grid((nx_pad + pk::ROWS - 1) / pk::ROWS, chunks);
  rowdot2_kernel<<<grid, pk::ROWS, 0, c.st>>>(o.T.p, Kx, nx_pad, nx_pad, n, c.y.p, mu, o.p1.p, o.p2.p);
  ACE_CUDA(cudaGetLastError());
  post_finish_kernel<<<(nx_pad + 255) / 256, 256, 0, c.st>>>(o.p1.p, o.p2.p, chunks, nx, nx_pad, kdiag, noise,
                                                            o.map.p, o.var.p);
  ACE_CUDA(cudaGetLastError());
  return 0;
}

static int posterior_rows_tri(Core& c, const double* Kx, const double* kdiag, int nx, int nx_pad, double mu,
                              double noise, PostOut& o) {
  const int n = c.n, n_pad = c.n_pad;
  ACE_TRY(o.T.alloc((size_t)nx_pad * n_pad));
  GemmNT g{};
  g.A = Kx; g.lda = nx_pad; g.B = c.A.p; g.ldb = n_pad; g.b_tri = 2; g.Bdiag = c.DX.p;
  g.C = o.T.p; g.ldc = nx_pad;
  g.M = nx_pad; g.N = n_pad; g.K = n_pad; g.alpha = 1.0; g.beta = 0.0;
  ACE_TRY(launch_gemm_nt(g, c.st));
  utv2_kernel<<<(n_pad + 7) / 8, 256, 0, c.st>>>(c.A.p, n_pad, c.DU.p, n, n_pad, c.y.p, c.tvy.p, c.tv1.p);
  ACE_CUDA(cudaGetLastError());
  const int chunks = (n + pk::CHUNK - 1) / pk::CHUNK;
  ACE_TRY(o.p1.alloc((size_t)nx_pad * chunks));
  ACE_TRY(o.p2.alloc((size_t)nx_pad * chunks));
  ACE_TRY(o.map.alloc(nx_pad));
  ACE_TRY(o.var.alloc(nx_pad));
  dim3 grid((nx_pad + pk::ROWS - 1) / pk::ROWS, chunks);
  rowdot_tri_kernel<<<grid, pk::ROWS, 0, c.st>>>(o.T.p, nx_pad, nx_pad, n, c.tvy.p, c.tv1.p, mu, o.p1.p, o.p2.p);
  ACE_CUDA(cudaGetLastError());
  post_finish_kernel<<<(nx_pad + 255) / 256, 256, 0, c.st>>>(o.p1.p, o.p2.p, chunks, nx, nx_pad, kdiag, noise,
                                                            o.map.p, o.var.p);
  ACE_CUDA(cudaGetLastError());
  return 0;
}

}

extern "C" {

int ace_fit_predict(ace_fit* f, const double* X2, const double* Z2, int nx, double mean_y, double std_y,
                    double* map, double* ci, double* var) {
  if (!f || !X2 || (f->c.Bz > 0 && !Z2) || !map || !ci || !var || nx < 1) return usage("ace_fit_predict: bad argument");
  Core& c = f->c;
  ACE_CUDA(cudaSetDevice(c.device));
  const bool split = c.shard_world > 1 && !c.shard_emulate && c.u_valid && f->comm != nullptr;
  const int G = split ? c.shard_world : 1, r = split ? c.shard_rank : 0;
  const int chunk = round_up((nx + G - 1) / G, TB);
  const int nx_all = chunk * G;
  const int lo = r * chunk, cnt = std::max(0, std::min(nx, lo + chunk) - lo);
  DBuf<double> dX2, dZ2, dLZ2, Kx, kd, res;
  ACE_TRY(dX2.alloc((size_t)nx_all * c.p));
  ACE_TRY(dZ2.alloc((size_t)nx_all * std::max(c.Bz, 1)));
  ACE_TRY(dLZ2.alloc((size_t)nx_all * std::max(c.Bz, 1)));
  ACE_TRY(Kx.alloc((size_t)chunk * c.n_pad));
  ACE_TRY(kd.alloc(chunk));
  ACE_TRY(res.alloc((size_t)2 * nx_all));
  ACE_TRY(upload_matrix(dX2.p, nx_all, nx_all, X2, nx, c.p, c.st));
  ACE_TRY(upload_matrix(dZ2.p, nx_all, nx_all, Z2, nx, c.Bz, c.st));
  if (c.Bz > 0)
    logabs_kernel<<<(unsigned)(((size_t)nx_all * c.Bz + 255) / 256), 256, 0, c.st>>>(dZ2.p, dLZ2.p, (size_t)nx_all * c.Bz);
  ACE_CUDA(cudaGetLastError());
  ACE_TRY(c.enqueue_prep());
  KernArgs a{};
  a.X1 = dX2.p + lo; a.Z1 = dZ2.p + lo; a.LZ1 = dLZ2.p + lo; a.ld1 = nx_all;
  a.X2 = c.X.p; a.Z2 = c.Z.p; a.LZ2 = c.LZ.p; a.ld2 = c.n_pad;
  a.n1 = cnt; a.n2 = c.n; a.n1_pad = chunk; a.n2_pad = c.n_pad; a.p = c.p; a.B = c.B; a.tab = c.tab.p;
  a.K = Kx.p; a.ldk = chunk;
  ACE_TRY(launch_kernmat(a, c.kind, c.st));
  kdiag_kernel<<<(chunk + 255) / 256, 256, 0, c.st>>>(dZ2.p + lo, dLZ2.p + lo, nx_all, cnt, c.B, c.kind, c.tab.p, 0, kd.p);
  ACE_CUDA(cudaGetLastError());
  double hpar[2];
  ACE_CUDA(cudaMemcpyAsync(hpar, c.theta.p, sizeof(double) * 2, cudaMemcpyDeviceToHost, c.st));
  ACE_CUDA(cudaStreamSynchronize(c.st));
  PostOut o;
  if (c.u_valid) {
    ACE_TRY(posterior_rows_tri(c, Kx.p, kd.p, cnt, chunk, hpar[1], std::exp(hpar[0]), o));
  } else {
    ACE_TRY(c.ensure_full_inverse());
    ACE_TRY(posterior_rows(c, c.Bf.p, Kx.p, kd.p, cnt, chunk, hpar[1], std::exp(hpar[0]), o));
  }
  ACE_CUDA(cudaMemcpyAsync(res.p + (size_t)r * chunk, o.map.p, sizeof(double) * chunk, cudaMemcpyDeviceToDevice, c.st));
  ACE_CUDA(cudaMemcpyAsync(res.p + nx_all + (size_t)r * chunk, o.var.p, sizeof(double) * chunk, cudaMemcpyDeviceToDevice,
                           c.st));
  if (split) {
    NcclApi& nc = nccl_api();
    ACE_NCCL(nc.GroupStart());
    ACE_NCCL(nc.AllGather(res.p + (size_t)r * chunk, res.p, chunk, ncclFloat64, f->comm, c.st));
    ACE_NCCL(nc.AllGather(res.p + nx_all + (size_t)r * chunk, res.p + nx_all, chunk, ncclFloat64, f->comm, c.st));
    ACE_NCCL(nc.GroupEnd());
  }
  std::vector<double> h((size_t)2 * nx_all);
  ACE_CUDA(cudaMemcpyAsync(h.data(), res.p, sizeof(double) * 2 * nx_all, cudaMemcpyDeviceToHost, c.st));
  ACE_CUDA(cudaStreamSynchronize(c.st));
  for (int i = 0; i < nx; ++i) {
    map[i] = mean_y + std_y * (h[i] + hpar[1]);
    const double sd = std_y * std::sqrt(std::fabs(h[(size_t)nx_all + i]));
    ci[i] = map[i] - 1.96 * sd;
    ci[i + nx] = map[i] + 1.96 * sd;
    var[i] = sd * sd;
  }
  return 0;
}

}

#include "api_functions.inl"
```

additivecausalexpansion_b200/csrc/chol.cuh:

```cuda
#pragma once
#include "dgemm_nt.cuh"
#include "fastmath.cuh"
#include "diag_block.cuh"
#include "uut_i8.cuh"

#include <cstdlib>
#include <vector>

namespace ace {

namespace leaf {
constexpr int LD = 129;
constexpr size_t SMEM_BYTES = (size_t)(128 * LD + 2 * 128 + 2 * 128 + 128 + 128) * 8;
}

template <int JB>
__device__ __forceinline__ void leaf_chol_block(double (&r)[8][8], double* Ls, double* colbuf, double* dg, double* idg,
                                                int tx, int ty, int* info, int blk) {
  using namespace leaf;
#pragma unroll 1
  for (int jx = 0; jx < 16; ++jx) {
    const int j = 16 * JB + jx;
    double* cb = colbuf + (j & 1) * 128;
    if (tx == jx) {
#pragma unroll
      for (int a = JB; a < 8; ++a) {
        const int i = 16 * a + ty;
        if (i >= j) cb[i] = r[a][JB];
      }
    }
    __syncthreads();
    const double pj = cb[j];
    const double inv = fast_rsqrt(pj);
    if (tx == jx) {
#pragma unroll
      for (int a = JB; a < 8; ++a) {
        const int i = 16 * a + ty;
        if (i > j) Ls[i + j * LD] = r[a][JB] * inv;
        if (i == j) {
          double s = pj * inv;
          s = fma(fma(-s, s, pj), 0.5 * inv, s);
          dg[j] = s;
          idg[j] = inv;
          if (!(pj > 0.0)) atomicCAS(info, 0, blk * 128 + j + 1);
        }
      }
    }
    const double invp = inv * inv;
    double lm[8], cm[8];
#pragma unroll
    for (int a = JB; a < 8; ++a) {
      lm[a] = cb[16 * a + ty] * invp;
      cm[a] = cb[16 * a + tx];
    }
    lm[JB] = (ty > jx) ? lm[JB] : 0.0;
    cm[JB] = (tx > jx) ? cm[JB] : 0.0;
#pragma unroll
    for (int a = JB; a < 8; ++a)
#pragma unroll
      for (int b = JB; b <= a; ++b) r[a][b] = fma(-lm[a], cm[b], r[a][b]);
  }
}

template <int JB>
__device__ __forceinline__ void leaf_inv_block(double (&r)[8][8], double* Ls, double* rowbuf, const double* idg,
                                               int tx, int ty) {
  using namespace leaf;
#pragma unroll 1
  for (int jx = 0; jx < 16; ++jx) {
    const int j = 16 * JB + jx;
    double* rb = rowbuf + (j & 1) * 128;
    if (ty == jx) {
      const double dj = idg[j];
#pragma unroll
      for (int b = 0; b <= JB; ++b) {
        const int k = 16 * b + tx;
        if (k <= j) {
          const double x = r[JB][b] * dj;
          rb[k] = x;
          if (k < j) Ls[k + j * LD] = x;
        }
      }
    }
    __syncthreads();
    double lm[8], xm[8];
#pragma unroll
    for (int a = JB; a < 8; ++a) lm[a] = Ls[16 * a + ty + j * LD];
    lm[JB] = (ty > jx) ? lm[JB] : 0.0;
#pragma unroll
    for (int b = 0; b <= JB; ++b) xm[b] = rb[16 * b + tx];
    xm[JB] = (tx <= jx) ? xm[JB] : 0.0;
#pragma unroll
    for (int a = JB; a < 8; ++a)
#pragma unroll
      for (int b = 0; b <= JB; ++b) r[a][b] = fma(-lm[a], xm[b], r[a][b]);
  }
}

__global__ void __launch_bounds__(256, 1) potrf_leaf_kernel(double* __restrict__ A, long ld, int blk,
                                                            double* __restrict__ DX, double* __restrict__ DU,
                                                            double* __restrict__ dvec, int* info) {
  using namespace leaf;
  extern __shared__ __align__(16) double sm[];
  double* Ls = sm;
  double* colbuf = Ls + 128 * LD;
  double* rowbuf = colbuf + 256;
  double* dg = rowbuf + 256;
  double* idg = dg + 128;
  const int tx = threadIdx.x & 15, ty = threadIdx.x >> 4;
  double* At = A + (size_t)blk * 128 * (ld + 1);

  for (int idx = threadIdx.x; idx < 128 * 128; idx += 256) {
    const int i = idx & 127, k = idx >> 7;
    Ls[i + k * LD] = At[i + (size_t)k * ld];
  }
  __syncthreads();
  double r[8][8];
#pragma unroll
  for (int a = 0; a < 8; ++a)
#pragma unroll
    for (int b = 0; b < 8; ++b) {
      const int i = 16 * a + ty, k = 16 * b + tx;
      r[a][b] = (k <= i) ? Ls[i + k * LD] : 0.0;
    }
  __syncthreads();

  leaf_chol_block<0>(r, Ls, colbuf, dg, idg, tx, ty, info, blk);
  leaf_chol_block<1>(r, Ls, colbuf, dg, idg, tx, ty, info, blk);
  leaf_chol_block<2>(r, Ls, colbuf, dg, idg, tx, ty, info, blk);
  leaf_chol_block<3>(r, Ls, colbuf, dg, idg, tx, ty, info, blk);
  leaf_chol_block<4>(r, Ls, colbuf, dg, idg, tx, ty, info, blk);
  leaf_chol_block<5>(r, Ls, colbuf, dg, idg, tx, ty, info, blk);
  leaf_chol_block<6>(r, Ls, colbuf, dg, idg, tx, ty, info, blk);
  leaf_chol_block<7>(r, Ls, colbuf, dg, idg, tx, ty, info, blk);
  __syncthreads();
#pragma unroll
  for (int a = 0; a < 8; ++a)
#pragma unroll
    for (int b = 0; b < 8; ++b) r[a][b] = (16 * a + ty == 16 * b + tx) ? 1.0 : 0.0;
  __syncthreads();

  leaf_inv_block<0>(r, Ls, rowbuf, idg, tx, ty);
  leaf_inv_block<1>(r, Ls, rowbuf, idg, tx, ty);
  leaf_inv_block<2>(r, Ls, rowbuf, idg, tx, ty);
  leaf_inv_block<3>(r, Ls, rowbuf, idg, tx, ty);
  leaf_inv_block<4>(r, Ls, rowbuf, idg, tx, ty);
  leaf_inv_block<5>(r, Ls, rowbuf, idg, tx, ty);
  leaf_inv_block<6>(r, Ls, rowbuf, idg, tx, ty);
  leaf_inv_block<7>(r, Ls, rowbuf, idg, tx, ty);
  __syncthreads();

  double* DXt = DX + (size_t)blk * 128 * 128;
  double* DUt = DU + (size_t)blk * 128 * 128;
  for (int idx = threadIdx.x; idx < 128 * 128; idx += 256) {
    const int i = idx & 127, k = idx >> 7;
    if (i > k) {
      At[i + (size_t)k * ld] = Ls[i + k * LD];
      DXt[idx] = Ls[k + i * LD];
      DUt[idx] = 0.0;
    } else if (i == k) {
      At[i + (size_t)k * ld] = dg[i];
      DXt[idx] = idg[i];
      DUt[idx] = idg[i];
    } else {
      DXt[idx] = 0.0;
      DUt[idx] = Ls[i + k * LD];
    }
  }
  if (threadIdx.x < 128) dvec[blk * 128 + threadIdx.x] = dg[threadIdx.x];
}

namespace trsml {
constexpr int ROWS = 64, LDA = ROWS + 4, LDB = 128 + 4, KH = 64;
constexpr size_t SMEM_BYTES = (size_t)(128 * LDA + KH * LDB) * 8 + 16;
constexpr uint32_t TX0_BYTES = (128 * ROWS + KH * 128) * 8, TX1_BYTES = KH * 128 * 8;
}

__global__ void __launch_bounds__(128, 1) trsm_leaf_kernel(double* __restrict__ P, long ld,
                                                           const double* __restrict__ DXt) {
  using namespace trsml;
  extern __shared__ __align__(128) unsigned char smraw[];
  double* As = reinterpret_cast<double*>(smraw);
  double* Bs = As + 128 * LDA;
  uint64_t* bar = reinterpret_cast<uint64_t*>(Bs + KH * LDB);
  const int warp = threadIdx.x >> 5, lane = threadIdx.x & 31;
  double* Pr = P + (size_t)blockIdx.x * ROWS;
  if (threadIdx.x == 0) {
    mbar_init(&bar[0], 1);
    mbar_init(&bar[1], 1);
    fence_mbar_init();
  }
  __syncthreads();
  if (warp == 0) {
    if (lane == 0) mbar_arrive_expect_tx(&bar[0], TX0_BYTES);
    __syncwarp();
    for (int kk = lane; kk < 128; kk += 32) tma_bulk_g2s(As + kk * LDA, Pr + (size_t)kk * ld, ROWS * 8, &bar[0]);
    for (int kk = lane; kk < KH; kk += 32) tma_bulk_g2s(Bs + kk * LDB, DXt + (size_t)kk * 128, 128 * 8, &bar[0]);
  }
  mbar_wait(&bar[0], 0);

  const int g = lane >> 2, tq = lane & 3;
  double acc[8][4][2];
#pragma unroll
  for (int mt = 0; mt < 8; ++mt)
#pragma unroll
    for (int nt = 0; nt < 4; ++nt) acc[mt][nt][0] = acc[mt][nt][1] = 0.0;
  const double* as = As + g;
  const double* bs = Bs + warp * 32 + g;
  const int ks_end = 8 * (warp + 1);
#pragma unroll 1
  for (int half = 0; half < 2; ++half) {
    if (half == 1) {
      __syncthreads();
      if (warp == 0) {
        if (lane == 0) mbar_arrive_expect_tx(&bar[1], TX1_BYTES);
        __syncwarp();
        for (int kk = lane; kk < KH; kk += 32)
          tma_bulk_g2s(Bs + kk * LDB, DXt + (size_t)(KH + kk) * 128, 128 * 8, &bar[1]);
      }
      if (ks_end <= KH / 4) break;
      mbar_wait(&bar[1], 0);
    }
    const int ks_lo = half * (KH / 4), ks_hi = min(ks_end, (half + 1) * (KH / 4));
#pragma unroll 2
    for (int ks = ks_lo; ks < ks_hi; ++ks) {
      const int k = ks * 4 + tq;
      double a[8], b[4];
#pragma unroll
      for (int mt = 0; mt < 8; ++mt) a[mt] = as[k * LDA + mt * 8];
#pragma unroll
      for (int nt = 0; nt < 4; ++nt) b[nt] = bs[(k - half * KH) * LDB + nt * 8];
#pragma unroll
      for (int mt = 0; mt < 8; ++mt)
#pragma unroll
        for (int nt = 0; nt < 4; ++nt) dmma884(acc[mt][nt][0], acc[mt][nt][1], a[mt], b[nt]);
    }
  }
  const int col0 = warp * 32 + 2 * tq;
#pragma unroll
  for (int nt = 0; nt < 4; ++nt)
#pragma unroll
    for (int e = 0; e < 2; ++e) {
      double* cc = Pr + (size_t)(col0 + nt * 8 + e) * ld + g;
#pragma unroll
      for (int mt = 0; mt < 8; ++mt) cc[mt * 8] = acc[mt][nt][e];
    }
}

struct PotrfTrace {
  std::vector<cudaEvent_t> panel_begin, panel_end, upd_begin, upda_end, updb_end;
  cudaEvent_t t0 = nullptr;
};

struct DenseWork {
  double* A = nullptr;
  long ld = 0;
  int nb = 0;
  double* DX = nullptr;
  double* DU = nullptr;
  double* dvec = nullptr;
  int* info = nullptr;
  double* Bf = nullptr;
  cudaStream_t main = nullptr, side = nullptr, aux = nullptr;
  cudaStream_t bg = nullptr;
  cudaEvent_t ev_panel[2] = {nullptr, nullptr}, ev_upd[2] = {nullptr, nullptr};
  cudaEvent_t ev_half = nullptr, ev_aux = nullptr;
  int panel_blocks = 4;
  PotrfTrace* trace = nullptr;
  double* Wp[2] = {nullptr, nullptr};
  double* Wsmall = nullptr;
  cudaEvent_t ev_copy[2] = {nullptr, nullptr};
  double* diag_ws = nullptr;
  long long* diag_dbg = nullptr;
  OzWork oz;
  int uut_engine = 0;
};

inline int configure_dense_kernels() {
  ACE_CUDA(cudaFuncSetAttribute(dgemm_nt_kernel, cudaFuncAttributeMaxDynamicSharedMemorySize,
                                (int)gemm::SMEM_BYTES));
  ACE_CUDA(cudaFuncSetAttribute(potrf_leaf_kernel, cudaFuncAttributeMaxDynamicSharedMemorySize,
                                (int)leaf::SMEM_BYTES));
  ACE_CUDA(cudaFuncSetAttribute(trsm_leaf_kernel, cudaFuncAttributeMaxDynamicSharedMemorySize,
                                (int)trsml::SMEM_BYTES));
  ACE_TRY(configure_diag_kernel());
  ACE_TRY(configure_uut_i8_kernel());
  return 0;
}

inline double* blkptr(const DenseWork& w, int rb, int cb) { return w.A + (size_t)rb * TB + (size_t)cb * TB * w.ld; }

inline int gemm_plain(const DenseWork& w, const double* A, const double* B, double* C, int M, int N, int K,
                      double alpha, double beta, int lower_only, cudaStream_t st) {
  GemmNT p{};
  p.A = A; p.lda = w.ld; p.B = B; p.ldb = w.ld; p.C = C; p.ldc = w.ld;
  p.M = M; p.N = N; p.K = K; p.alpha = alpha; p.beta = beta; p.lower_only = lower_only;
  return launch_gemm_nt(p, st);
}

inline int trsm_rec(const DenseWork& w, int r0, int r1, int a, int c, cudaStream_t st) {
  if (r1 <= r0) return 0;
  if (c - a == 1) {
    trsm_leaf_kernel<<<(unsigned)((r1 - r0) * TB / trsml::ROWS), 128, trsml::SMEM_BYTES, st>>>(
        blkptr(w, r0, a), w.ld, w.DX + (size_t)a * TB * TB);
    ACE_CUDA(cudaGetLastError());
    return 0;
  }
  const int m = a + (c - a + 1) / 2;
  ACE_TRY(trsm_rec(w, r0, r1, a, m, st));
  ACE_TRY(gemm_plain(w, blkptr(w, r0, a), blkptr(w, m, a), blkptr(w, r0, m), (r1 - r0) * TB, (c - m) * TB,
                     (m - a) * TB, -1.0, 1.0, 0, st));
  return trsm_rec(w, r0, r1, m, c, st);
}

inline int potrf_rec(const DenseWork& w, int a, int b, cudaStream_t st) {
  if (b - a == 1) {
    potrf_leaf_kernel<<<1, 256, leaf::SMEM_BYTES, st>>>(w.A, w.ld, a, w.DX, w.DU, w.dvec, w.info);
    ACE_CUDA(cudaGetLastError());
    return 0;
  }
  const int c = a + (b - a + 1) / 2;
  ACE_TRY(potrf_rec(w, a, c, st));
  ACE_TRY(trsm_rec(w, c, b, a, c, st));
  ACE_TRY(gemm_plain(w, blkptr(w, c, a), blkptr(w, c, a), blkptr(w, c, c), (b - c) * TB, (b - c) * TB,
                     (c - a) * TB, -1.0, 1.0, 1, st));
  return potrf_rec(w, c, b, st);
}

inline int trtri_merge_range(const DenseWork& w, int lo, int hi, cudaStream_t st, double* ws, int h_min = 1);

inline int diag_block_factor_invert(const DenseWork& w, int j0, int j1, cudaStream_t st, int share = 1) {
  if (w.diag_ws != nullptr) {
    DiagArgs a{};
    a.A = w.A; a.ld = w.ld; a.blk0 = j0; a.nblk = j1 - j0; a.DX = w.DX; a.DU = w.DU; a.dvec = w.dvec; a.info = w.info;
    a.S = w.diag_ws;
    a.W = w.diag_ws + (size_t)w.panel_blocks * TB * w.panel_blocks * TB;
    a.dbg = w.diag_dbg;
    const long rest = (long)(w.nb - j1) * TB;
    return launch_diag_block(a, st, rest <= 6144L * share);
  }
  ACE_TRY(potrf_rec(w, j0, j1, st));
  return trtri_merge_range(w, j0, j1, st, w.Wsmall);
}

inline int potrf_blocked(const DenseWork& w, int fork_at = 0, int fork_when = 0, bool incremental = false) {
  const int nb = w.nb, pb = w.panel_blocks;
  bool forked = false;
  ACE_CUDA(cudaMemsetAsync(w.info, 0, sizeof(int), w.main));
  ACE_CUDA(cudaEventRecord(w.ev_upd[1], w.main));
  ACE_CUDA(cudaStreamWaitEvent(w.side, w.ev_upd[1], 0));
  int J = 0;
  for (int j0 = 0; j0 < nb; j0 += pb, ++J) {
    const int j1 = min(j0 + pb, nb), j2 = min(j1 + pb, nb);
    auto mark = [&](std::vector<cudaEvent_t>* v, cudaStream_t st) {
      if (!v) return;
      cudaEvent_t e;
      cudaEventCreate(&e);
      cudaEventRecord(e, st);
      v->push_back(e);
    };
    mark(w.trace ? &w.trace->panel_begin : nullptr, w.side);
    const bool fused = (w.Wp[0] != nullptr);
    const double* panel = blkptr(w, j1 < nb ? j1 : j0, j0);
    if (!fused) {
      ACE_TRY(potrf_rec(w, j0, j1, w.side));
      ACE_TRY(trsm_rec(w, j1, nb, j0, j1, w.side));
    } else {
      ACE_TRY(diag_block_factor_invert(w, j0, j1, w.side));
      if (j1 < nb) {
        if (J >= 2) ACE_CUDA(cudaStreamWaitEvent(w.side, w.ev_copy[J & 1], 0));
        GemmNT t{};
        t.A = blkptr(w, j1, j0); t.lda = w.ld;
        t.B = blkptr(w, j0, j0); t.ldb = w.ld; t.b_tri = 2; t.Bdiag = w.DX + (size_t)j0 * TB * TB;
        t.C = w.Wp[J & 1] + (size_t)j1 * TB; t.ldc = w.ld;
        t.M = (nb - j1) * TB; t.N = (j1 - j0) * TB; t.K = (j1 - j0) * TB; t.alpha = 1.0; t.beta = 0.0;
        ACE_TRY(launch_gemm_nt(t, w.side));
        panel = w.Wp[J & 1] + (size_t)j1 * TB;
      }
    }
    mark(w.trace ? &w.trace->panel_end : nullptr, w.side);
    ACE_CUDA(cudaEventRecord(w.ev_panel[J & 1], w.side));
    if (fused && j1 < nb) {
      ACE_CUDA(cudaStreamWaitEvent(w.aux, w.ev_panel[J & 1], 0));
      ACE_CUDA(cudaMemcpy2DAsync(blkptr(w, j1, j0), sizeof(double) * w.ld, w.Wp[J & 1] + (size_t)j1 * TB,
                                 sizeof(double) * w.ld, sizeof(double) * (size_t)(nb - j1) * TB, (size_t)(j1 - j0) * TB,
                                 cudaMemcpyDeviceToDevice, w.aux));
      ACE_CUDA(cudaEventRecord(w.ev_copy[J & 1], w.aux));
    }
    if (incremental && fused && J >= 1) {
      cudaStream_t bg = w.bg ? w.bg : w.aux;
      ACE_CUDA(cudaStreamWaitEvent(bg, w.ev_panel[J & 1], 0));
      ACE_CUDA(cudaStreamWaitEvent(bg, w.ev_copy[(J - 1) & 1], 0));
      const int s1 = j0 * TB, s2 = (j1 - j0) * TB;
      GemmNT p{};
      p.A = w.A; p.lda = w.ld; p.a_tri = 1; p.Adiag = w.DU;
      p.B = blkptr(w, j0, 0); p.ldb = w.ld;
      p.C = w.Bf; p.ldc = s1;
      p.M = s1; p.N = s2; p.K = s1; p.alpha = 1.0; p.beta = 0.0;
      ACE_TRY(launch_gemm_nt(p, bg));
      GemmNT r{};
      r.A = blkptr(w, j0, j0); r.lda = w.ld; r.a_tri = 2; r.Adiag = w.DX + (size_t)j0 * TB * TB;
      r.B = w.Bf; r.ldb = s1;
      r.C = blkptr(w, j0, 0); r.ldc = w.ld;
      r.Ct = blkptr(w, 0, j0); r.ldct = w.ld;
      r.M = s2; r.N = s1; r.K = s2; r.alpha = -1.0; r.beta = 0.0;
      ACE_TRY(launch_gemm_nt(r, bg));
      ACE_CUDA(cudaEventRecord(w.ev_aux, bg));
      forked = true;
    }
    if (fork_at > 0 && !forked && j1 >= fork_at && j1 >= fork_when && j1 < nb) {
      ACE_CUDA(cudaEventRecord(w.ev_half, w.side));
      ACE_CUDA(cudaStreamWaitEvent(w.aux, w.ev_half, 0));
      ACE_TRY(trtri_merge_range(w, 0, fork_at, w.aux, w.Bf, w.Wp[0] ? w.panel_blocks : 1));
      ACE_CUDA(cudaEventRecord(w.ev_aux, w.aux));
      forked = true;
    }
    if (j1 >= nb) break;
    ACE_CUDA(cudaStreamWaitEvent(w.main, w.ev_panel[J & 1], 0));
    const int K = (j1 - j0) * TB;
    mark(w.trace ? &w.trace->upd_begin : nullptr, w.main);
    ACE_TRY(gemm_plain(w, panel, panel, blkptr(w, j1, j1), (nb - j1) * TB, (j2 - j1) * TB, K, -1.0, 1.0, 0, w.main));
    mark(w.trace ? &w.trace->upda_end : nullptr, w.main);
    ACE_CUDA(cudaEventRecord(w.ev_upd[J & 1], w.main));
    ACE_CUDA(cudaStreamWaitEvent(w.side, w.ev_upd[J & 1], 0));
    if (j2 < nb)
      ACE_TRY(gemm_plain(w, panel + (size_t)(j2 - j1) * TB, panel + (size_t)(j2 - j1) * TB, blkptr(w, j2, j2),
                         (nb - j2) * TB, (nb - j2) * TB, K, -1.0, 1.0, 1, w.main));
    mark(w.trace ? &w.trace->updb_end : nullptr, w.main);
  }
  ACE_CUDA(cudaStreamWaitEvent(w.main, w.ev_panel[J & 1], 0));
  if (w.Wp[0] != nullptr && J >= 1) {
    ACE_CUDA(cudaStreamWaitEvent(w.main, w.ev_copy[0], 0));
    if (J >= 2) ACE_CUDA(cudaStreamWaitEvent(w.main, w.ev_copy[1], 0));
  }
  return forked ? 1 : 0;
}

inline int& dbg_trtri_max_h() {
  static int v = 1 << 30;
  return v;
}

inline int trtri_level(const DenseWork& w, int lo, int len, int h, cudaStream_t st, double* ws) {
  const int nodes = (len + 2 * h - 1) / (2 * h);
  const int s1 = h * TB;
  int nreg = 0;
  while (nreg < nodes && (nreg * 2 * h + 2 * h) <= len) ++nreg;
  for (int pass = 0; pass < 2; ++pass) {
    int q0, cnt, s2;
    if (pass == 0) {
      q0 = 0; cnt = nreg; s2 = s1;
    } else {
      q0 = nreg; cnt = nodes - nreg;
      if (cnt == 0) break;
      const int c_local = q0 * 2 * h + h;
      if (c_local >= len) break;
      s2 = (len - c_local) * TB;
    }
    if (cnt == 0) continue;
    const int a = lo + q0 * 2 * h, c = a + h;
    const long node_stride = (long)2 * h * TB * (w.ld + 1);
    double* Wt = ws + (size_t)q0 * s1 * s1;
    GemmNT p{};
    p.A = blkptr(w, a, a); p.lda = w.ld; p.a_tri = 1; p.Adiag = w.DU + (size_t)a * TB * TB;
    p.B = blkptr(w, c, a); p.ldb = w.ld;
    p.C = Wt; p.ldc = s1;
    p.M = s1; p.N = s2; p.K = s1; p.alpha = 1.0; p.beta = 0.0;
    p.batch = cnt; p.sA = node_stride; p.sB = node_stride; p.sC = (long)s1 * s1;
    p.sAdiag = (long)2 * h * TB * TB;
    ACE_TRY(launch_gemm_nt(p, st));
    GemmNT r{};
    r.A = blkptr(w, c, c); r.lda = w.ld; r.a_tri = 2; r.Adiag = w.DX + (size_t)c * TB * TB;
    r.B = Wt; r.ldb = s1;
    r.C = blkptr(w, c, a); r.ldc = w.ld;
    r.Ct = blkptr(w, a, c); r.ldct = w.ld;
    r.M = s2; r.N = s1; r.K = s2; r.alpha = -1.0; r.beta = 0.0;
    r.batch = cnt; r.sA = node_stride; r.sB = (long)s1 * s1; r.sC = node_stride; r.sCt = node_stride;
    r.sAdiag = (long)2 * h * TB * TB;
    ACE_TRY(launch_gemm_nt(r, st));
  }
  return 0;
}

inline int trtri_merge_range(const DenseWork& w, int lo, int hi, cudaStream_t st, double* ws, int h_min) {
  for (int h = h_min; h < hi - lo && h <= dbg_trtri_max_h(); h *= 2) ACE_TRY(trtri_level(w, lo, hi - lo, h, st, ws));
  return 0;
}

inline int trtri_hmin(const DenseWork& w) { return w.Wp[0] ? w.panel_blocks : 1; }

inline int trtri_merge(const DenseWork& w) { return trtri_merge_range(w, 0, w.nb, w.main, w.Bf, trtri_hmin(w)); }

inline int potrf_trtri(const DenseWork& w) {
  const int nb = w.nb;
  int h_top = 1;
  while (2 * h_top < nb) h_top *= 2;
  if (nb < 8 || w.aux == nullptr || dbg_trtri_max_h() < (1 << 30)) {
    int s = potrf_blocked(w);
    if (s < 0) return s;
    return trtri_merge(w);
  }
  static const int incr = std::getenv("ACE_INCR_TRTRI") ? std::atoi(std::getenv("ACE_INCR_TRTRI")) : 1;
  if (incr && w.Wp[0] != nullptr) {
    const int forked = potrf_blocked(w, 0, 0, true);
    if (forked < 0) return forked;
    if (forked) ACE_CUDA(cudaStreamWaitEvent(w.main, w.ev_aux, 0));
    return 0;
  }
  double frac = 0.75;
  if (const char* e = std::getenv("ACE_FORK_FRAC")) frac = std::atof(e);
  const int forked = potrf_blocked(w, h_top, (int)(frac * nb));
  if (forked < 0) return forked;
  const size_t left_ws = (size_t)(h_top * TB / 2) * (h_top * TB / 2);
  if (!forked) ACE_TRY(trtri_merge_range(w, 0, h_top, w.main, w.Bf, trtri_hmin(w)));
  ACE_TRY(trtri_merge_range(w, h_top, nb, w.main, w.Bf + left_ws, trtri_hmin(w)));
  if (forked) ACE_CUDA(cudaStreamWaitEvent(w.main, w.ev_aux, 0));
  return trtri_level(w, 0, nb, h_top, w.main, w.Bf);
}

constexpr int UUT_I8_MIN_N = 8192;

inline bool uut_uses_i8(int n_pad, int engine) {
  if (engine != 0) return engine == 2;
  return n_pad >= UUT_I8_MIN_N && n_pad <= oz::MAX_N;
}

inline int uut_inverse(const DenseWork& w) {
  if (uut_uses_i8(w.nb * TB, w.uut_engine)) return launch_uut_i8(w.oz, w.A, w.DU, w.nb, w.Bf, w.main);
  GemmNT p{};
  p.A = w.A; p.lda = w.ld; p.a_tri = 1; p.Adiag = w.DU;
  p.B = w.A; p.ldb = w.ld; p.Bdiag = w.DU;
  p.C = w.Bf; p.ldc = w.ld; p.Ct = w.Bf; p.ldct = w.ld;
  p.M = p.N = p.K = w.nb * TB;
  p.alpha = 1.0; p.beta = 0.0; p.lower_only = 1;
  return launch_gemm_nt(p, w.main);
}

inline int spd_inverse(const DenseWork& w) {
  ACE_TRY(potrf_trtri(w));
  return uut_inverse(w);
}

}
```

additivecausalexpansion_b200/csrc/shard_dense.cuh:

```cuda
#pragma once
#include <cstdio>
#include "chol.cuh"
#include "nccl_dyn.h"

namespace ace {

struct ShardCtx {
  int rank = 0, world = 1;
  bool emulate = false;
  ncclComm_t comm = nullptr;
  int h_min = 16;
  ncclComm_t comm2 = nullptr;
  cudaEvent_t* events = nullptr;
  double* head[2] = {nullptr, nullptr};
  cudaStream_t bulk_stream = nullptr;
  ncclComm_t comm3 = nullptr;
  double* mid[2] = {nullptr, nullptr};
  cudaStream_t mid_stream = nullptr;
  double* chain_ws = nullptr;
  bool incr = false;
  bool mine(int panel) const { return emulate || panel % world == rank; }
};

inline int shard_panels(int nb, int pb) { return (nb + pb - 1) / pb; }

__global__ void __launch_bounds__(256) splitk_sum_kernel(const double* __restrict__ part, int S, size_t len, size_t total,
                                                         double* __restrict__ out) {
  const size_t idx = (size_t)blockIdx.x * 256 + threadIdx.x;
  if (idx >= total) return;
  const size_t prob = idx / len, e = idx % len;
  const double* src = part + prob * (size_t)S * len + e;
  double acc = src[0];
  for (int s2 = 1; s2 < S; ++s2) acc += src[(size_t)s2 * len];
  out[idx] = acc;
}

__global__ void __launch_bounds__(256) splitk_sum_ld_kernel(const double* __restrict__ part, int S, int R, int Cc,
                                                            double* __restrict__ C, long ldc, double beta) {
  const size_t idx = (size_t)blockIdx.x * 256 + threadIdx.x, len = (size_t)R * Cc;
  if (idx >= len) return;
  double acc = part[idx];
  for (int s2 = 1; s2 < S; ++s2) acc += part[(size_t)s2 * len + idx];
  double* dst = C + (idx % R) + (idx / R) * ldc;
  *dst = (beta != 0.0) ? fma(beta, *dst, acc) : acc;
}

inline int chain_gemm(GemmNT g, double* ws, cudaStream_t st) {
  const int S = g.K / TB;
  if (ws == nullptr || S <= 1 || g.K % TB || g.batch > 1 || g.ksplit > 1) return launch_gemm_nt(g, st);
  double* C = g.C;
  const long ldc = g.ldc;
  const double beta = g.beta;
  g.C = ws; g.ldc = g.M; g.beta = 0.0;
  g.ksplit = S; g.klen = TB; g.sA = 0; g.sB = 0; g.sC = (long)g.M * g.N;
  ACE_TRY(launch_gemm_nt(g, st));
  const size_t len = (size_t)g.M * g.N;
  splitk_sum_ld_kernel<<<(unsigned)((len + 255) / 256), 256, 0, st>>>(ws, S, g.M, g.N, C, ldc, beta);
  ACE_CUDA(cudaGetLastError());
  return 0;
}

constexpr int SHARD_EVENT_KINDS = 8;

struct ShardTrace {
  cudaEvent_t t0 = nullptr;
  std::vector<cudaEvent_t> ev;
  int np = 0;
  std::vector<cudaEvent_t> lev;
  std::vector<int> lev_h;
  void level_mark(int h, int k, cudaStream_t st) {
    if (!t0) return;
    if (k == 0) lev_h.push_back(h);
    cudaEvent_t e;
    cudaEventCreate(&e);
    cudaEventRecord(e, st);
    lev.push_back(e);
  }
  void mark(int J, int k, cudaStream_t st) {
    if (!t0) return;
    cudaEventRecord(ev[(size_t)J * 14 + k], st);
  }
};
inline ShardTrace& shard_trace() {
  static ShardTrace t;
  return t;
}
inline void shard_trace_begin(int NP, cudaStream_t st) {
  ShardTrace& t = shard_trace();
  static const bool on = std::getenv("ACE_SHARD_TRACE") != nullptr;
  if (!on) return;
  if (!t.t0) cudaEventCreate(&t.t0);
  while ((int)t.ev.size() < 14 * NP) {
    cudaEvent_t e;
    cudaEventCreate(&e);
    t.ev.push_back(e);
  }
  t.np = NP;
  for (auto e : t.lev) cudaEventDestroy(e);
  t.lev.clear();
  t.lev_h.clear();
  cudaEventRecord(t.t0, st);
}
inline void shard_trace_dump(int rank) {
  ShardTrace& t = shard_trace();
  if (!t.t0) return;
  cudaDeviceSynchronize();
  std::fprintf(stderr, "[shard trace rank %d] J: factor_begin head_ready head_bcast diag_applied | bulk_trsm bulk_bcast la_applied | main_begin main_end | mid_begin mid_trsm mid_bcast mid_applied | diag_kernel_done (ms)\n", rank);
  for (int J = 0; J < t.np; ++J) {
    float v[14];
    for (int k = 0; k < 14; ++k)
      if (cudaEventElapsedTime(&v[k], t.t0, t.ev[(size_t)J * 14 + k]) != cudaSuccess) v[k] = -1.f;
    std::fprintf(stderr, "[shard trace rank %d] %2d: %7.3f %7.3f %7.3f %7.3f | %7.3f %7.3f %7.3f | %7.3f %7.3f | %7.3f %7.3f %7.3f %7.3f | %7.3f\n",
                 rank, J, v[0], v[1], v[2], v[3], v[4], v[5], v[6], v[7], v[8], v[9], v[10], v[11], v[12], v[13]);
  }
  for (size_t l = 0; l < t.lev_h.size(); ++l) {
    float v[5];
    for (int k = 0; k < 5; ++k)
      if (cudaEventElapsedTime(&v[k], t.t0, t.lev[l * 5 + k]) != cudaSuccess) v[k] = -1.f;
    std::fprintf(stderr, "[shard trace rank %d] trtri level h=%d (%s): begin %.3f gemm1 +%.3f gemm2 +%.3f gather +%.3f unpack +%.3f\n",
                 rank, t.lev_h[l] < 0 ? -t.lev_h[l] : t.lev_h[l], t.lev_h[l] < 0 ? "redundant" : "split", v[0], v[1] - v[0],
                 v[2] - v[1], v[3] - v[2], v[4] - v[3]);
  }
  cudaGetLastError();
}

inline int potrf_sharded(const DenseWork& w, const ShardCtx& cx) {
  const int nb = w.nb, pb = w.panel_blocks, NP = shard_panels(nb, pb);
  if (!w.Wp[0] || !cx.events || !cx.head[0] || !cx.bulk_stream) {
    set_error("potrf_sharded: packed panel buffers missing");
    return -2;
  }
  cudaEvent_t* ev_head = cx.events;
  cudaEvent_t* ev_bulk = cx.events + NP;
  cudaEvent_t* ev_la = cx.events + 2 * NP;
  cudaEvent_t* ev_first = cx.events + 3 * NP;
  cudaEvent_t* ev_step = cx.events + 4 * NP;
  cudaEvent_t* ev_copy = cx.events + 5 * NP;
  cudaEvent_t* ev_diag = cx.events + 6 * NP;
  cudaEvent_t* ev_midla = cx.events + 7 * NP;
  const bool use_mid = cx.mid[0] != nullptr && cx.mid_stream != nullptr && (cx.emulate || cx.comm3 != nullptr);
  cudaStream_t mids = cx.mid_stream;
  NcclApi& nc = nccl_api();
  cudaStream_t bulk = cx.bulk_stream;
  ACE_CUDA(cudaMemsetAsync(w.info, 0, sizeof(int), w.main));
  ACE_CUDA(cudaEventRecord(w.ev_upd[1], w.main));
  ACE_CUDA(cudaStreamWaitEvent(w.side, w.ev_upd[1], 0));
  ACE_CUDA(cudaStreamWaitEvent(bulk, w.ev_upd[1], 0));
  if (use_mid) ACE_CUDA(cudaStreamWaitEvent(mids, w.ev_upd[1], 0));
  ACE_CUDA(cudaStreamWaitEvent(w.aux, w.ev_upd[1], 0));
  shard_trace_begin(NP, w.main);
  ShardTrace& tr = shard_trace();
  for (int J = 0; J < NP; ++J) {
    const int j0 = J * pb, j1 = std::min(j0 + pb, nb), j2 = std::min(j1 + pb, nb);
    const long wJ = (long)(j1 - j0) * TB, wN = (long)(j2 - j1) * TB;
    const long hJ = wJ + wN, mB = (long)(nb - j2) * TB;
    const int j3 = std::min(j2 + pb, nb);
    const long wM = use_mid ? (long)(j3 - j2) * TB : 0;
    double* Hd = cx.head[J & 1];
    double* Wp = w.Wp[J & 1];
    double* Md = cx.mid[J & 1];
    const bool mine = cx.mine(J), la = (J + 1 < NP) && cx.mine(J + 1);
    if (J >= 2) {
      ACE_CUDA(cudaStreamWaitEvent(w.side, ev_la[J - 2], 0));
      if (use_mid) ACE_CUDA(cudaStreamWaitEvent(w.side, ev_midla[J - 2], 0));
      ACE_CUDA(cudaStreamWaitEvent(w.side, ev_copy[J - 2], 0));
    }
    tr.mark(J, 0, w.side);
    if (mine) {
      ACE_TRY(diag_block_factor_invert(w, j0, j1, w.side, cx.world));
      tr.mark(J, 13, w.side);
      ACE_CUDA(cudaMemcpy2DAsync(Hd, sizeof(double) * hJ, blkptr(w, j0, j0), sizeof(double) * w.ld,
                                 sizeof(double) * wJ, (size_t)wJ, cudaMemcpyDeviceToDevice, w.side));
      if (wN > 0) {
        if (J >= 1) ACE_CUDA(cudaStreamWaitEvent(w.side, use_mid ? ev_midla[J - 1] : ev_la[J - 1], 0));
        GemmNT t{};
        t.A = blkptr(w, j1, j0); t.lda = w.ld;
        t.B = blkptr(w, j0, j0); t.ldb = w.ld; t.b_tri = 2; t.Bdiag = w.DX + (size_t)j0 * TB * TB;
        t.C = Hd + wJ; t.ldc = hJ;
        t.M = (int)wN; t.N = (int)wJ; t.K = (int)wJ; t.alpha = 1.0; t.beta = 0.0;
        ACE_TRY(chain_gemm(t, cx.chain_ws, w.side));
      }
    }
    tr.mark(J, 1, w.side);
    if (!cx.emulate) {
      const int root = J % cx.world;
      double* dx = w.DX + (size_t)j0 * TB * TB;
      double* du = w.DU + (size_t)j0 * TB * TB;
      double* dv = w.dvec + (size_t)j0 * TB;
      ACE_NCCL(nc.GroupStart());
      ACE_NCCL(nc.Broadcast(Hd, Hd, (size_t)hJ * wJ, ncclFloat64, root, cx.comm, w.side));
      ACE_NCCL(nc.Broadcast(dx, dx, (size_t)wJ * TB, ncclFloat64, root, cx.comm, w.side));
      ACE_NCCL(nc.Broadcast(du, du, (size_t)wJ * TB, ncclFloat64, root, cx.comm, w.side));
      ACE_NCCL(nc.Broadcast(dv, dv, (size_t)wJ, ncclFloat64, root, cx.comm, w.side));
      ACE_NCCL(nc.GroupEnd());
    }
    ACE_CUDA(cudaEventRecord(ev_head[J], w.side));
    tr.mark(J, 2, w.side);
    if (la) {
      if (J >= 1) ACE_CUDA(cudaStreamWaitEvent(w.side, ev_first[J - 1], 0));
      GemmNT g{};
      g.A = Hd + wJ; g.lda = hJ; g.B = Hd + wJ; g.ldb = hJ; g.C = blkptr(w, j1, j1); g.ldc = w.ld;
      g.M = (int)wN; g.N = (int)wN; g.K = (int)wJ; g.alpha = -1.0; g.beta = 1.0;
      ACE_TRY(chain_gemm(g, cx.chain_ws, w.side));
    }
    ACE_CUDA(cudaEventRecord(ev_diag[J], w.side));
    tr.mark(J, 3, w.side);
    if (J >= 2) {
      ACE_CUDA(cudaStreamWaitEvent(bulk, ev_step[J - 2], 0));
      ACE_CUDA(cudaStreamWaitEvent(bulk, ev_copy[J - 2], 0));
    }
    ACE_CUDA(cudaStreamWaitEvent(bulk, ev_head[J], 0));
    if (mB > 0) {
      if (mine) {
        GemmNT t{};
        t.A = blkptr(w, j2, j0); t.lda = w.ld;
        t.B = blkptr(w, j0, j0); t.ldb = w.ld; t.b_tri = 2; t.Bdiag = w.DX + (size_t)j0 * TB * TB;
        t.C = Wp; t.ldc = mB;
        t.M = (int)mB; t.N = (int)wJ; t.K = (int)wJ; t.alpha = 1.0; t.beta = 0.0;
        ACE_TRY(launch_gemm_nt(t, bulk));
      }
      tr.mark(J, 4, bulk);
      if (!cx.emulate) ACE_NCCL(nc.Broadcast(Wp, Wp, (size_t)mB * wJ, ncclFloat64, J % cx.world, cx.comm2, bulk));
    } else {
      tr.mark(J, 4, bulk);
    }
    ACE_CUDA(cudaEventRecord(ev_bulk[J], bulk));
    tr.mark(J, 5, bulk);
    if (la && mB > wM) {
      if (J >= 1) ACE_CUDA(cudaStreamWaitEvent(bulk, ev_first[J - 1], 0));
      GemmNT g{};
      g.A = Wp + wM; g.lda = mB; g.B = Hd + wJ; g.ldb = hJ; g.C = blkptr(w, j2, j1) + wM; g.ldc = w.ld;
      g.M = (int)(mB - wM); g.N = (int)wN; g.K = (int)wJ; g.alpha = -1.0; g.beta = 1.0;
      ACE_TRY(launch_gemm_nt(g, bulk));
    }
    ACE_CUDA(cudaEventRecord(ev_la[J], bulk));
    tr.mark(J, 6, bulk);
    if (use_mid) {
      ACE_CUDA(cudaStreamWaitEvent(mids, ev_head[J], 0));
      tr.mark(J, 9, mids);
      if (wM > 0) {
        if (mine) {
          if (J >= 1) ACE_CUDA(cudaStreamWaitEvent(mids, ev_la[J - 1], 0));
          GemmNT t{};
          t.A = blkptr(w, j2, j0); t.lda = w.ld;
          t.B = blkptr(w, j0, j0); t.ldb = w.ld; t.b_tri = 2; t.Bdiag = w.DX + (size_t)j0 * TB * TB;
          t.C = Md; t.ldc = wM;
          t.M = (int)wM; t.N = (int)wJ; t.K = (int)wJ; t.alpha = 1.0; t.beta = 0.0;
          ACE_TRY(launch_gemm_nt(t, mids));
        }
        tr.mark(J, 10, mids);
        if (!cx.emulate) ACE_NCCL(nc.Broadcast(Md, Md, (size_t)wM * wJ, ncclFloat64, J % cx.world, cx.comm3, mids));
        tr.mark(J, 11, mids);
        if (la) {
          if (J >= 1) ACE_CUDA(cudaStreamWaitEvent(mids, ev_first[J - 1], 0));
          GemmNT g{};
          g.A = Md; g.lda = wM; g.B = Hd + wJ; g.ldb = hJ; g.C = blkptr(w, j2, j1); g.ldc = w.ld;
          g.M = (int)wM; g.N = (int)wN; g.K = (int)wJ; g.alpha = -1.0; g.beta = 1.0;
          ACE_TRY(launch_gemm_nt(g, mids));
        }
      }
      ACE_CUDA(cudaEventRecord(ev_midla[J], mids));
      tr.mark(J, 12, mids);
    }
    ACE_CUDA(cudaStreamWaitEvent(w.aux, ev_head[J], 0));
    ACE_CUDA(cudaStreamWaitEvent(w.aux, ev_bulk[J], 0));
    if (use_mid) ACE_CUDA(cudaStreamWaitEvent(w.aux, ev_midla[J], 0));
    {
      const long skip = mine ? wJ : 0;
      if (hJ > skip)
        ACE_CUDA(cudaMemcpy2DAsync(blkptr(w, j0, j0) + skip, sizeof(double) * w.ld, Hd + skip, sizeof(double) * hJ,
                                   sizeof(double) * (hJ - skip), (size_t)wJ, cudaMemcpyDeviceToDevice, w.aux));
      if (mB > 0)
        ACE_CUDA(cudaMemcpy2DAsync(blkptr(w, j2, j0), sizeof(double) * w.ld, Wp, sizeof(double) * mB,
                                   sizeof(double) * mB, (size_t)wJ, cudaMemcpyDeviceToDevice, w.aux));
    }
    ACE_CUDA(cudaEventRecord(ev_copy[J], w.aux));
    if (cx.incr && J >= 1 && w.bg) {
      const int Gs = cx.world;
      const int r_lo = cx.emulate ? 0 : cx.rank, r_hi = cx.emulate ? cx.world : cx.rank + 1;
      const long pw = (long)pb * TB, step = (long)Gs * pw;
      const int KL = 2048;
      const int S = std::max(1, (j0 * TB + KL - 1) / KL);
      const size_t len = (size_t)pw * wJ;
      auto count_of = [&](int cf) { return (cf < J) ? (J - cf + Gs - 1) / Gs : 0; };
      size_t total_cnt = 0;
      for (int cf = r_lo; cf < r_hi; ++cf) total_cnt += (size_t)count_of(cf);
      ACE_CUDA(cudaStreamWaitEvent(w.bg, ev_copy[J], 0));
      size_t off = 0;
      for (int cf = r_lo; cf < r_hi; ++cf) {
        const int cnt = count_of(cf);
        if (cnt <= 0) continue;
        double* Wt = w.Bf + off * len;
        double* part = (S > 1) ? w.Bf + total_cnt * len : Wt;
        GemmNT p{};
        p.A = w.A + (size_t)cf * pw; p.lda = w.ld; p.a_tri = 1; p.a_row_off = (int)(cf * pw); p.s_row_off = (int)step;
        p.Adiag = w.DU;
        p.B = blkptr(w, j0, 0); p.ldb = w.ld;
        p.C = part; p.ldc = pw;
        p.M = (int)pw; p.N = (int)wJ; p.K = j0 * TB; p.alpha = 1.0; p.beta = 0.0;
        p.batch = cnt; p.sA = step; p.sB = 0; p.sC = (long)len;
        if (S > 1) {
          p.ksplit = S; p.klen = KL;
        }
        ACE_TRY(launch_gemm_nt(p, w.bg));
        if (S > 1) {
          const size_t total = (size_t)cnt * len;
          splitk_sum_kernel<<<(unsigned)((total + 255) / 256), 256, 0, w.bg>>>(part, S, len, total, Wt);
          ACE_CUDA(cudaGetLastError());
        }
        off += (size_t)cnt;
      }
      off = 0;
      for (int cf = r_lo; cf < r_hi; ++cf) {
        const int cnt = count_of(cf);
        if (cnt <= 0) continue;
        GemmNT r{};
        r.A = blkptr(w, j0, j0); r.lda = w.ld; r.a_tri = 2; r.Adiag = w.DX + (size_t)j0 * TB * TB;
        r.B = w.Bf + off * len; r.ldb = pw;
        r.C = blkptr(w, j0, cf * pb); r.ldc = w.ld;
        r.Ct = blkptr(w, cf * pb, j0); r.ldct = w.ld;
        r.M = (int)wJ; r.N = (int)pw; r.K = (int)wJ; r.alpha = -1.0; r.beta = 0.0;
        r.batch = cnt; r.sA = 0; r.sB = pw * wJ; r.sC = step * w.ld; r.sCt = step;
        ACE_TRY(launch_gemm_nt(r, w.bg));
        off += (size_t)cnt;
      }
      ACE_CUDA(cudaEventRecord(w.ev_aux, w.bg));
    }
    ACE_CUDA(cudaStreamWaitEvent(w.main, ev_bulk[J], 0));
    tr.mark(J, 7, w.main);
    bool first = true;
    {
      const int G = cx.world;
      auto apply = [&](int c, int count) -> int {
        const int c0 = c * pb, c1 = std::min(c0 + pb, nb);
        const double* pan = Wp + (size_t)(c0 - j2) * TB;
        GemmNT g{};
        g.A = pan; g.lda = mB; g.B = pan; g.ldb = mB; g.C = blkptr(w, c0, c0); g.ldc = w.ld;
        g.M = (nb - c0) * TB; g.N = (c1 - c0) * TB; g.K = (int)wJ; g.alpha = -1.0; g.beta = 1.0;
        if (count > 1) {
          const long step = (long)G * pb * TB;
          g.batch = count; g.sA = step; g.sB = step; g.sC = step * (w.ld + 1); g.m_dec = (int)step;
        }
        return launch_gemm_nt(g, w.main);
      };
      const int nplay = cx.emulate ? G : 1;
      for (int k = 0; k < nplay; ++k) {
        const int r = cx.emulate ? (J + 2 + k) % G : cx.rank;
        int cf = J + 2;
        while (cf < NP && cf % G != r) ++cf;
        if (cf >= NP) continue;
        ACE_TRY(apply(cf, 1));
        if (first) {
          ACE_CUDA(cudaEventRecord(ev_first[J], w.main));
          first = false;
        }
        int cnt = 0, last_ragged = -1;
        for (int c = cf + G; c < NP; c += G) {
          if ((c + 1) * pb > nb) last_ragged = c; else ++cnt;
        }
        if (cnt > 0) ACE_TRY(apply(cf + G, cnt));
        if (last_ragged >= 0) ACE_TRY(apply(last_ragged, 1));
      }
    }
    if (first) ACE_CUDA(cudaEventRecord(ev_first[J], w.main));
    ACE_CUDA(cudaEventRecord(ev_step[J], w.main));
    tr.mark(J, 8, w.main);
  }
  ACE_CUDA(cudaStreamWaitEvent(w.main, ev_diag[NP - 1], 0));
  ACE_CUDA(cudaStreamWaitEvent(w.main, ev_la[NP - 1], 0));
  if (use_mid) ACE_CUDA(cudaStreamWaitEvent(w.main, ev_midla[NP - 1], 0));
  ACE_CUDA(cudaStreamWaitEvent(w.main, ev_copy[NP - 1], 0));
  if (!cx.emulate)
    ACE_NCCL(nc.AllReduce(w.info, w.info, 1, ncclInt32, ncclMax, cx.comm, w.main));
  return 0;
}

__global__ void __launch_bounds__(256) unpack_piece_kernel(const double* __restrict__ src, int R, int C,
                                                           double* __restrict__ dst, long ldd,
                                                           double* __restrict__ dstT, long lddt) {
  __shared__ double tile[32][33];
  const int r0 = blockIdx.x * 32, c0 = blockIdx.y * 32;
  const int tx = threadIdx.x & 31, ty = threadIdx.x >> 5;
#pragma unroll
  for (int k = 0; k < 4; ++k) {
    const int c = c0 + ty + 8 * k;
    const double v = src[(size_t)c * R + r0 + tx];
    dst[(size_t)c * ldd + r0 + tx] = v;
    tile[ty + 8 * k][tx] = v;
  }
  if (dstT == nullptr) return;
  __syncthreads();
#pragma unroll
  for (int k = 0; k < 4; ++k) {
    const int r = r0 + ty + 8 * k;
    dstT[(size_t)r * lddt + c0 + tx] = tile[tx][ty + 8 * k];
  }
}

inline bool level_is_split(const ShardCtx& cx, int h) {
  return cx.world > 1 && h >= cx.h_min && h % (2 * cx.world) == 0;
}

inline int trtri_level_sharded(const DenseWork& w, int lo, int len, int h, cudaStream_t st, double* ws,
                               const ShardCtx& cx, bool need_lower) {
  const int G = cx.world;
  const int hs = h / (2 * G);
  const int Rs = hs * TB, s1 = h * TB;
  struct Node { int a, c, s2; size_t off; };
  std::vector<Node> nodes;
  size_t chunk = 0;
  for (int q = 0; q * 2 * h < len; ++q) {
    const int a = lo + q * 2 * h, c = a + h;
    if (c >= lo + len) break;
    const int s2 = std::min(h, lo + len - c) * TB;
    nodes.push_back({a, c, s2, chunk});
    chunk += (size_t)2 * Rs * s2;
  }
  if (nodes.empty()) return 0;
  double* stage = ws;
  double* wt = ws + (size_t)G * chunk;
  const int r_lo = cx.emulate ? 0 : cx.rank, r_hi = cx.emulate ? G : cx.rank + 1;
  auto slice_of = [&](int r, int e) { return e == 0 ? r : 2 * G - 1 - r; };
  cudaStream_t ss[3] = {st, w.side, w.aux};
  const int ns = (w.side && w.aux && st == w.main) ? 3 : 1;
  auto fork = [&]() -> int {
    if (ns == 1) return 0;
    ACE_CUDA(cudaEventRecord(w.ev_upd[0], st));
    ACE_CUDA(cudaStreamWaitEvent(ss[1], w.ev_upd[0], 0));
    ACE_CUDA(cudaStreamWaitEvent(ss[2], w.ev_upd[0], 0));
    return 0;
  };
  auto join = [&]() -> int {
    if (ns == 1) return 0;
    ACE_CUDA(cudaEventRecord(w.ev_panel[0], ss[1]));
    ACE_CUDA(cudaEventRecord(w.ev_panel[1], ss[2]));
    ACE_CUDA(cudaStreamWaitEvent(st, w.ev_panel[0], 0));
    ACE_CUDA(cudaStreamWaitEvent(st, w.ev_panel[1], 0));
    return 0;
  };
  shard_trace().level_mark(h, 0, st);
  ACE_TRY(fork());
  int li = 0;
  for (int r = r_lo; r < r_hi; ++r)
    for (const Node& nd : nodes)
      for (int e = 0; e < 2; ++e) {
        const int ro = slice_of(r, e) * Rs;
        GemmNT p{};
        p.A = blkptr(w, nd.a, nd.a) + ro; p.lda = w.ld; p.a_tri = 1; p.a_row_off = ro;
        p.Adiag = w.DU + (size_t)nd.a * TB * TB;
        p.B = blkptr(w, nd.c, nd.a); p.ldb = w.ld;
        p.C = wt + (size_t)(r - r_lo) * chunk + nd.off + (size_t)e * Rs * nd.s2; p.ldc = Rs;
        p.M = Rs; p.N = nd.s2; p.K = s1; p.alpha = 1.0; p.beta = 0.0;
        ACE_TRY(launch_gemm_nt(p, ss[li++ % ns]));
      }
  ACE_TRY(join());
  shard_trace().level_mark(h, 1, st);
  ACE_TRY(fork());
  li = 0;
  for (int r = r_lo; r < r_hi; ++r)
    for (const Node& nd : nodes)
      for (int e = 0; e < 2; ++e) {
        const int ro = slice_of(r, e) * Rs;
        GemmNT q{};
        q.A = blkptr(w, nd.c, nd.c); q.lda = w.ld; q.a_tri = 2; q.Adiag = w.DX + (size_t)nd.c * TB * TB;
        q.B = wt + (size_t)(r - r_lo) * chunk + nd.off + (size_t)e * Rs * nd.s2; q.ldb = Rs;
        q.C = blkptr(w, nd.c, nd.a) + (size_t)ro * w.ld; q.ldc = w.ld;
        q.Ct = stage + (size_t)r * chunk + nd.off + (size_t)e * Rs * nd.s2; q.ldct = Rs;
        q.M = nd.s2; q.N = Rs; q.K = nd.s2; q.alpha = -1.0; q.beta = 0.0;
        ACE_TRY(launch_gemm_nt(q, ss[li++ % ns]));
      }
  ACE_TRY(join());
  shard_trace().level_mark(h, 2, st);
  if (!cx.emulate) {
    NcclApi& nc = nccl_api();
    ACE_NCCL(nc.AllGather(stage + (size_t)cx.rank * chunk, stage, chunk, ncclFloat64, cx.comm, st));
  }
  shard_trace().level_mark(h, 3, st);
  for (int r = 0; r < G; ++r)
    for (const Node& nd : nodes)
      for (int e = 0; e < 2; ++e) {
        const int sl = slice_of(r, e);
        const double* src = stage + (size_t)r * chunk + nd.off + (size_t)e * Rs * nd.s2;
        dim3 grid(Rs / 32, nd.s2 / 32);
        unpack_piece_kernel<<<grid, 256, 0, st>>>(src, Rs, nd.s2, blkptr(w, nd.a + sl * hs, nd.c), w.ld,
                                                  need_lower ? blkptr(w, nd.c, nd.a + sl * hs) : nullptr, w.ld);
        ACE_CUDA(cudaGetLastError());
      }
  shard_trace().level_mark(h, 4, st);
  return 0;
}

inline int gather_inverse_sharded(const DenseWork& w, const ShardCtx& cx) {
  const int nb = w.nb, pb = w.panel_blocks, NP = shard_panels(nb, pb);
  cudaStream_t st = w.main;
  if (NP >= 2) ACE_CUDA(cudaStreamWaitEvent(st, w.ev_aux, 0));
  shard_trace().level_mark(1 << 20, 0, st);
  const int G = cx.world;
  std::vector<size_t> off(NP, 0), tot(G, 0);
  for (int c = 0; c < NP; ++c) {
    const int c0 = c * pb, c1 = std::min(c0 + pb, nb);
    off[c] = tot[c % G];
    tot[c % G] += (size_t)(nb - c1) * TB * (size_t)(c1 - c0) * TB;
  }
  size_t chunk = 0;
  for (int q = 0; q < G; ++q) chunk = std::max(chunk, tot[q]);
  double* stage = w.Bf;
  if ((size_t)G * chunk > (size_t)w.ld * w.ld) {
    set_error("gather_inverse_sharded: staging does not fit");
    return -2;
  }
  for (int c = 0; c < NP; ++c) {
    const int c0 = c * pb, c1 = std::min(c0 + pb, nb);
    const long mC = (long)(nb - c1) * TB, wC = (long)(c1 - c0) * TB;
    if (mC == 0 || !cx.mine(c)) continue;
    ACE_CUDA(cudaMemcpy2DAsync(stage + (size_t)(c % G) * chunk + off[c], sizeof(double) * mC, blkptr(w, c1, c0),
                               sizeof(double) * w.ld, sizeof(double) * mC, (size_t)wC, cudaMemcpyDeviceToDevice, st));
  }
  shard_trace().level_mark(1 << 20, 1, st);
  shard_trace().level_mark(1 << 20, 2, st);
  if (!cx.emulate && chunk > 0) {
    NcclApi& nc = nccl_api();
    ACE_NCCL(nc.AllGather(stage + (size_t)cx.rank * chunk, stage, chunk, ncclFloat64, cx.comm, st));
  }
  shard_trace().level_mark(1 << 20, 3, st);
  for (int c = 0; c < NP; ++c) {
    const int c0 = c * pb, c1 = std::min(c0 + pb, nb);
    const int mC = (nb - c1) * TB, wC = (c1 - c0) * TB;
    if (mC == 0) continue;
    dim3 grid(mC / 32, wC / 32);
    unpack_piece_kernel<<<grid, 256, 0, st>>>(stage + (size_t)(c % G) * chunk + off[c], mC, wC, blkptr(w, c1, c0), w.ld,
                                              blkptr(w, c0, c1), w.ld);
    ACE_CUDA(cudaGetLastError());
  }
  shard_trace().level_mark(1 << 20, 4, st);
  return 0;
}

inline int trtri_merge_sharded(const DenseWork& w, const ShardCtx& cx) {
  for (int h = trtri_hmin(w); h < w.nb; h *= 2) {
    if (level_is_split(cx, h))
      ACE_TRY(trtri_level_sharded(w, 0, w.nb, h, w.main, w.Bf, cx, true));
    else {
      shard_trace().level_mark(-h, 0, w.main);
      ACE_TRY(trtri_level(w, 0, w.nb, h, w.main, w.Bf));
      for (int k = 1; k < 5; ++k) shard_trace().level_mark(-h, k, w.main);
    }
  }
  return 0;
}

inline int uut_inverse_sharded(const DenseWork& w, const ShardCtx& cx) {
  const int r_lo = cx.emulate ? 0 : cx.rank, r_hi = cx.emulate ? cx.world : cx.rank + 1;
  for (int r = r_lo; r < r_hi; ++r) {
    GemmNT p{};
    p.A = w.A; p.lda = w.ld; p.a_tri = 1; p.Adiag = w.DU;
    p.B = w.A; p.ldb = w.ld; p.Bdiag = w.DU;
    p.C = w.Bf; p.ldc = w.ld; p.Ct = w.Bf; p.ldct = w.ld;
    p.M = p.N = p.K = w.nb * TB;
    p.alpha = 1.0; p.beta = 0.0; p.lower_only = 1;
    p.tile_first = r; p.tile_stride = cx.world;
    ACE_TRY(launch_gemm_nt(p, w.main));
  }
  return 0;
}

}
```

additivecausalexpansion_b200/csrc/uut_i8.cuh:

```cuda
#pragma once
#include "common.cuh"

namespace ace {

namespace oz {
constexpr int S = 8;
constexpr int DMAX = 64;
constexpr int BM = 128, BN = 64, BK = 32;
constexpr int CPB = TB / BK;
constexpr int STAGES = 4;
constexpr int A_PLANE = BM * BK, B_PLANE = BN * BK;
constexpr int STAGE_BYTES = S * (A_PLANE + B_PLANE);
constexpr size_t SMEM_BYTES = 1024 + (size_t)STAGES * STAGE_BYTES + 128;
static_assert(SMEM_BYTES <= 227 * 1024, "pipeline exceeds the shared memory of one block");
constexpr int TMEM_COLS = 512;
constexpr int THREADS = 192;
constexpr long KMAX = 2147483647L / ((long)S * DMAX * DMAX);
constexpr int MAX_N = (int)(KMAX / TB) * TB;
static_assert(S * BN <= TMEM_COLS, "S accumulators of BN columns must fit the 512 TMEM columns");
static_assert((long)S * DMAX * DMAX * MAX_N <= 2147483647L, "INT32 accumulators may overflow");
constexpr uint32_t IDESC = (2u << 4) | (1u << 7) | (1u << 10) | ((uint32_t)(BN >> 3) << 17) | ((uint32_t)(BM >> 4) << 24);

__host__ __device__ inline size_t block_off(int nb, int t, int rb, int c) {
  const long nc = (long)nb * CPB;
  const long per_plane = (long)nb * nc - (long)CPB * nb * (nb - 1) / 2;
  const long off = (long)rb * nc - (long)CPB * rb * (rb - 1) / 2 + (c - (long)CPB * rb);
  return ((size_t)t * per_plane + off) * (size_t)(BM * BK);
}
inline size_t plane_bytes(int nb) { return block_off(nb, S, 0, 0); }
}

__device__ __forceinline__ uint64_t oz_smem_desc(uint32_t saddr) {
  return (uint64_t)((saddr >> 4) & 0x3FFF) | ((uint64_t)(128 >> 4) << 16) | ((uint64_t)(256 >> 4) << 32) |
         (1ull << 46);
}

__device__ __forceinline__ void tc_fence_before() { asm volatile("tcgen05.fence::before_thread_sync;" ::: "memory"); }
__device__ __forceinline__ void tc_fence_after() { asm volatile("tcgen05.fence::after_thread_sync;" ::: "memory"); }

__device__ __forceinline__ void tc_mma_i8(uint32_t d_tmem, uint64_t adesc, uint64_t bdesc, uint32_t accumulate) {
  asm volatile(
      "{\n.reg .pred p;\nsetp.ne.b32 p, %4, 0;\n"
      "tcgen05.mma.cta_group::1.kind::i8 [%0], %1, %2, %3, p;\n}\n" ::"r"(d_tmem),
      "l"(adesc), "l"(bdesc), "r"(oz::IDESC), "r"(accumulate)
      : "memory");
}

__device__ __forceinline__ void tc_commit(uint64_t* bar) {
  asm volatile("tcgen05.commit.cta_group::1.mbarrier::arrive::one.shared::cluster.b64 [%0];" ::"r"(smem_u32(bar))
               : "memory");
}

__device__ __forceinline__ void tc_ld16(uint32_t taddr, uint32_t (&v)[16]) {
  asm volatile(
      "tcgen05.ld.sync.aligned.32x32b.x16.b32 {%0,%1,%2,%3,%4,%5,%6,%7,%8,%9,%10,%11,%12,%13,%14,%15}, [%16];"
      : "=r"(v[0]), "=r"(v[1]), "=r"(v[2]), "=r"(v[3]), "=r"(v[4]), "=r"(v[5]), "=r"(v[6]), "=r"(v[7]), "=r"(v[8]),
        "=r"(v[9]), "=r"(v[10]), "=r"(v[11]), "=r"(v[12]), "=r"(v[13]), "=r"(v[14]), "=r"(v[15])
      : "r"(taddr)
      : "memory");
}

__device__ __forceinline__ double oz_u(const double* A, long ld, const double* DU, int rb, int cb, int r, int kk) {
  return (cb == rb) ? DU[(size_t)rb * TB * TB + r + (size_t)kk * TB] : A[(size_t)rb * TB + r + (size_t)(cb * TB + kk) * ld];
}

__global__ void __launch_bounds__(128) oz_rowmax_kernel(const double* __restrict__ A, long ld,
                                                        const double* __restrict__ DU,
                                                        unsigned long long* __restrict__ rowmax) {
  const int cb = blockIdx.x, rb = blockIdx.y, r = threadIdx.x;
  if (cb < rb) return;
  double m = 0.0;
#pragma unroll 8
  for (int kk = 0; kk < TB; ++kk) m = fmax(m, fabs(oz_u(A, ld, DU, rb, cb, r, kk)));
  atomicMax(rowmax + rb * TB + r, (unsigned long long)__double_as_longlong(m));
}

__global__ void __launch_bounds__(128) oz_split_kernel(const double* __restrict__ A, long ld,
                                                       const double* __restrict__ DU,
                                                       const unsigned long long* __restrict__ rowmax, int nb,
                                                       int8_t* __restrict__ planes, int* __restrict__ ex) {
  using namespace oz;
  const int cb = blockIdx.x, rb = blockIdx.y, r = threadIdx.x;
  if (cb < rb) return;
  const double m = __longlong_as_double((long long)rowmax[rb * TB + r]);
  int e = 0;
  if (m > 0.0) {
    frexp(m, &e);
    ++e;
  }
  if (cb == rb) ex[rb * TB + r] = e;
  const double scale = ldexp(1.0, -e);
#pragma unroll 1
  for (int q = 0; q < TB / 16; ++q) {
    uint32_t w[S][4];
#pragma unroll
    for (int t = 0; t < S; ++t) w[t][0] = w[t][1] = w[t][2] = w[t][3] = 0u;
#pragma unroll
    for (int x16 = 0; x16 < 16; ++x16) {
      double x = oz_u(A, ld, DU, rb, cb, r, q * 16 + x16) * scale;
#pragma unroll
      for (int t = 0; t < S; ++t) {
        x *= 128.0;
        const double d = rint(x);
        x -= d;
        w[t][x16 >> 2] |= ((uint32_t)(int)d & 0xffu) << (8 * (x16 & 3));
      }
    }
    const int c = cb * CPB + q / 2;
    const size_t in_blk = (size_t)(r >> 3) * 256 + (q & 1) * 128 + (r & 7) * 16;
#pragma unroll
    for (int t = 0; t < S; ++t)
      *reinterpret_cast<uint4*>(planes + block_off(nb, t, rb, c) + in_blk) = make_uint4(w[t][0], w[t][1], w[t][2], w[t][3]);
  }
}

__global__ void __launch_bounds__(oz::THREADS, 1) uut_i8_kernel(const int8_t* __restrict__ planes,
                                                                const int* __restrict__ ex, int nb,
                                                                double* __restrict__ C, long ldc) {
  using namespace oz;
  extern __shared__ unsigned char smem_raw[];
  unsigned char* sm = reinterpret_cast<unsigned char*>((reinterpret_cast<uintptr_t>(smem_raw) + 1023) & ~uintptr_t(1023));
  uint64_t* full = reinterpret_cast<uint64_t*>(sm + (size_t)STAGES * STAGE_BYTES);
  uint64_t* empty = full + STAGES;
  uint64_t* done = empty + STAGES;
  uint32_t* tmem_slot = reinterpret_cast<uint32_t*>(done + 1);
  const int warp = threadIdx.x >> 5, lane = threadIdx.x & 31;

  int ti, tj;
  {
    const long L = blockIdx.x;
    long t = (long)((sqrt(4.0 * (double)L + 1.0) - 1.0) * 0.5);
    while (t * (t + 1) > L) --t;
    while ((t + 1) * (t + 2) <= L) ++t;
    ti = (int)t;
    tj = (int)(L - t * (t + 1));
  }
  const int i0 = ti * BM, j0 = tj * BN, jb = tj >> 1, jh = tj & 1;
  const int c_begin = ti * CPB, nchunks = nb * CPB - c_begin;

  if (threadIdx.x == 0) {
    for (int s = 0; s < STAGES; ++s) {
      mbar_init(&full[s], 1);
      mbar_init(&empty[s], 1);
    }
    mbar_init(done, 1);
    fence_mbar_init();
  }
  if (warp == 1) {
    asm volatile("tcgen05.alloc.cta_group::1.sync.aligned.shared::cta.b32 [%0], %1;" ::"r"(smem_u32(tmem_slot)),
                 "r"(TMEM_COLS)
                 : "memory");
    asm volatile("tcgen05.relinquish_alloc_permit.cta_group::1.sync.aligned;" ::: "memory");
  }
  tc_fence_before();
  __syncthreads();
  tc_fence_after();
  const uint32_t tmem = *tmem_slot;

  if (warp == 0) {
    if (lane == 0) {
      for (int it = 0; it < nchunks; ++it) {
        const int s = it % STAGES;
        mbar_wait(&empty[s], ((it / STAGES) & 1) ^ 1);
        mbar_arrive_expect_tx(&full[s], STAGE_BYTES);
        unsigned char* st = sm + (size_t)s * STAGE_BYTES;
        const int c = c_begin + it;
#pragma unroll
        for (int t = 0; t < S; ++t)
          tma_bulk_g2s(st + t * A_PLANE, planes + block_off(nb, t, ti, c), A_PLANE, &full[s]);
#pragma unroll
        for (int t = 0; t < S; ++t)
          tma_bulk_g2s(st + S * A_PLANE + t * B_PLANE, planes + block_off(nb, t, jb, c) + jh * B_PLANE, B_PLANE,
                       &full[s]);
      }
    }
    __syncwarp();
  } else if (warp == 1) {
    if (lane == 0) {
      for (int it = 0; it < nchunks; ++it) {
        const int s = it % STAGES;
        mbar_wait(&full[s], (it / STAGES) & 1);
        tc_fence_after();
        const uint32_t a0 = smem_u32(sm + (size_t)s * STAGE_BYTES), b0 = a0 + S * A_PLANE;
#pragma unroll
        for (int a = 0; a < S; ++a)
#pragma unroll
          for (int b = 0; a + b < S; ++b)
            tc_mma_i8(tmem + (uint32_t)((a + b) * BN), oz_smem_desc(a0 + a * A_PLANE), oz_smem_desc(b0 + b * B_PLANE),
                      (it > 0 || a > 0) ? 1u : 0u);
        tc_commit(&empty[s]);
      }
      tc_commit(done);
    }
    __syncwarp();
  } else {
    mbar_wait(done, 0);
    tc_fence_after();
    const int q = warp & 3;
    const int r = q * 32 + lane, i = i0 + r;
    const int ei = ex[i] - 14;
    const uint32_t trow = tmem + ((uint32_t)(q * 32) << 16);
#pragma unroll 1
    for (int jc = 0; jc < BN / 16; ++jc) {
      uint32_t v[S][16];
#pragma unroll
      for (int g = 0; g < S; ++g) tc_ld16(trow + (uint32_t)(g * BN + jc * 16), v[g]);
      asm volatile("tcgen05.wait::ld.sync.aligned;" ::: "memory");
      double out[16];
#pragma unroll
      for (int j = 0; j < 16; ++j) {
        double acc = (double)(int)v[S - 1][j];
#pragma unroll
        for (int g = S - 2; g >= 0; --g) acc = fma(acc, 0x1p-7, (double)(int)v[g][j]);
        const int col = j0 + jc * 16 + j;
        out[j] = ldexp(acc, ei + ex[col]);
        C[(size_t)col * ldc + i] = out[j];
      }
      double2* ct = reinterpret_cast<double2*>(C + (size_t)i * ldc + j0 + jc * 16);
#pragma unroll
      for (int j = 0; j < 8; ++j) ct[j] = make_double2(out[2 * j], out[2 * j + 1]);
    }
  }
  tc_fence_before();
  __syncthreads();
  if (warp == 1) {
    tc_fence_after();
    asm volatile("tcgen05.dealloc.cta_group::1.sync.aligned.b32 %0, %1;" ::"r"(tmem), "r"(TMEM_COLS) : "memory");
  }
}

struct OzWork {
  int8_t* planes = nullptr;
  unsigned long long* rowmax = nullptr;
  int* ex = nullptr;
};

inline int configure_uut_i8_kernel() {
  ACE_CUDA(cudaFuncSetAttribute(uut_i8_kernel, cudaFuncAttributeMaxDynamicSharedMemorySize, (int)oz::SMEM_BYTES));
  return 0;
}

inline int launch_uut_i8(const OzWork& o, const double* A, const double* DU, int nb, double* C, cudaStream_t st) {
  using namespace oz;
  if ((long)nb * TB > MAX_N) {
    set_error("uut_i8: n_pad beyond the INT32 accumulator bound");
    return -2;
  }
  if (!o.planes || !o.rowmax || !o.ex) {
    set_error("uut_i8: digit-plane workspace not allocated");
    return -2;
  }
  const long ld = (long)nb * TB;
  ACE_CUDA(cudaMemsetAsync(o.rowmax, 0, sizeof(unsigned long long) * (size_t)ld, st));
  const dim3 g2(nb, nb);
  oz_rowmax_kernel<<<g2, TB, 0, st>>>(A, ld, DU, o.rowmax);
  ACE_CUDA(cudaGetLastError());
  oz_split_kernel<<<g2, TB, 0, st>>>(A, ld, DU, o.rowmax, nb, o.planes, o.ex);
  ACE_CUDA(cudaGetLastError());
  const long tiles = (long)nb * (nb + 1);
  uut_i8_kernel<<<(unsigned)tiles, THREADS, SMEM_BYTES, st>>>(o.planes, o.ex, nb, C, ld);
  ACE_CUDA(cudaGetLastError());
  return 0;
}

}
```

additivecausalexpansion_b200/fit.py:

```python
from __future__ import annotations

import ctypes as C

import numpy as np

from ._lib import AceFitConfig, c_double_p, check, lib

KERNELS = {"SE": 0, "Matern32": 1}
OPTIMIZERS = {"Nadam": 0, "Adam": 1, "GD": 2, "NAG": 2}


def _f(a, two_d=False):
    a = np.asfortranarray(np.asarray(a, dtype=np.float64))
    if two_d and a.ndim == 1:
        a = np.asfortranarray(a.reshape(-1, 1))
    return a


def _p(a):
    return None if a is None else a.ctypes.data_as(c_double_p)


class AceFit:
    def __init__(self, y, X, Z, parameters, kernel="SE", optimizer="Nadam", learning_rate=0.01, beta1=0.9,
                 beta2=0.999, momentum=0.0, norm_clip=None, clip_at=1.0, std_y=1.0, device=0, use_graph=True):
        self._h = C.c_void_p(None)
        y, X, Z = _f(y).ravel(), _f(X, True), _f(Z, True)
        par = _f(parameters).ravel()
        self.n, self.p = X.shape
        self.Bz = Z.shape[1]
        self.B = self.Bz + 1
        self.P = 2 + self.B + self.B * self.p
        if y.size != self.n or Z.shape[0] != self.n:
            raise ValueError("y, X, Z disagree on the number of observations")
        if par.size != self.P:
            raise ValueError(f"parameters must have {self.P} entries (2 + B + B*p), got {par.size}")
        if optimizer == "GD":
            momentum = 0.0
        if norm_clip is None:
            norm_clip = optimizer in ("Adam", "Nadam")
        cfg = AceFitConfig()
        lib().ace_fit_default_config(C.byref(cfg))
        cfg.kernel, cfg.optimizer = KERNELS[kernel], OPTIMIZERS[optimizer]
        cfg.learning_rate, cfg.beta1, cfg.beta2, cfg.momentum = learning_rate, beta1, beta2, momentum
        cfg.norm_clip, cfg.clip_at, cfg.std_y = int(bool(norm_clip)), clip_at, std_y
        cfg.device, cfg.use_graph = int(device), int(bool(use_graph))
        self.kernel, self.optimizer = kernel, optimizer
        check(lib().ace_fit_create(C.byref(self._h), _p(y), _p(X), _p(Z), self.n, self.p, self.Bz, _p(par),
                                   C.byref(cfg)), "ace_fit_create")

    def close(self):
        if getattr(self, "_h", None) is not None and self._h:
            lib().ace_fit_destroy(self._h)
            self._h = C.c_void_p(None)

    def __del__(self):
        try:
            self.close()
        except Exception:
            pass

    def __enter__(self):
        return self

    def __exit__(self, *exc):
        self.close()

    def para_update(self, iter):
        st = np.zeros(2)
        gn = C.c_double(0.0)
        check(lib().ace_fit_para_update(self._h, int(iter), _p(st), C.cast(C.byref(gn), c_double_p)),
              "ace_fit_para_update")
        return st, gn.value

    def run(self, iter_start=1, max_iter=1000, tol=1e-4, prev_evidence=0.0):
        stats = np.zeros((2, max_iter), order="F")
        done = C.c_int(0)
        check(lib().ace_fit_run(self._h, int(iter_start), int(max_iter), float(tol), float(prev_evidence),
                                _p(stats), C.byref(done)), "ace_fit_run")
        return done.value, stats[:, :done.value].copy()

    def shard(self, dist):
        rank, world = dist.get_rank(), dist.get_world_size()
        if world == 1:
            return
        buf = C.create_string_buffer(128)
        if rank == 0:
            check(lib().ace_comm_unique_id(buf), "ace_comm_unique_id")
        box = [buf.raw]
        dist.broadcast_object_list(box, src=0)
        check(lib().ace_fit_shard(self._h, box[0], rank, world), "ace_fit_shard")

    def shard_emulate(self, world):
        check(lib().ace_fit_shard_emulate(self._h, int(world)), "ace_fit_shard_emulate")

    def upload_data(self, y=None, X=None, Z=None):
        y = None if y is None else _f(y).ravel()
        X = None if X is None else _f(X, True)
        Z = None if Z is None else _f(Z, True)
        check(lib().ace_fit_upload_data(self._h, _p(y), _p(X), _p(Z)), "ace_fit_upload_data")

    @property
    def kernel_launches(self):
        k = C.c_int(0)
        check(lib().ace_fit_kernel_launches(self._h, C.byref(k)), "ace_fit_kernel_launches")
        return k.value

    def timer_start(self):
        check(lib().ace_fit_timer_start(self._h), "ace_fit_timer_start")

    def timer_stop(self):
        ms = C.c_double(0.0)
        check(lib().ace_fit_timer_stop(self._h, C.cast(C.byref(ms), c_double_p)), "ace_fit_timer_stop")
        return ms.value

    def dbg_set_uut_engine(self, engine):
        check(lib().ace_dbg_fit_set_uut_engine(self._h, int(engine)), "ace_dbg_fit_set_uut_engine")

    def get_train_stats(self):
        st = np.zeros(2)
        check(lib().ace_fit_get_train_stats(self._h, _p(st)), "ace_fit_get_train_stats")
        return st

    @property
    def parameters(self):
        out = np.empty(self.P)
        check(lib().ace_fit_get_parameters(self._h, _p(out)), "ace_fit_get_parameters")
        return out

    @parameters.setter
    def parameters(self, value):
        v = _f(value).ravel()
        if v.size != self.P:
            raise ValueError("wrong parameter length")
        check(lib().ace_fit_set_parameters(self._h, _p(v)), "ace_fit_set_parameters")

    @property
    def gradients(self):
        out = np.empty(self.P)
        check(lib().ace_fit_get_gradients(self._h, _p(out)), "ace_fit_get_gradients")
        return out

    @property
    def optimizer_state(self):
        m, v = np.empty(self.P), np.empty(self.P)
        check(lib().ace_fit_get_optimizer_state(self._h, _p(m), _p(v)), "ace_fit_get_optimizer_state")
        return m, v

    @property
    def invKmatn(self):
        out = np.empty((self.n, self.n), order="F")
        check(lib().ace_fit_get_invKmatn(self._h, _p(out)), "ace_fit_get_invKmatn")
        return out

    @property
    def alpha(self):
        out = np.empty(self.n)
        check(lib().ace_fit_get_alpha(self._h, _p(out)), "ace_fit_get_alpha")
        return out

    @property
    def last_timing_ms(self):
        out = np.zeros(6)
        check(lib().ace_fit_last_timing(self._h, _p(out)), "ace_fit_last_timing")
        return dict(zip(("build", "potrf", "trtri", "uut", "grad", "total"), out))

    def predict(self, X2, Z2, mean_y=0.0, std_y=1.0):
        X2, Z2 = _f(X2, True), _f(Z2, True)
        nx = X2.shape[0]
        m, ci, var = np.empty(nx), np.empty((nx, 2), order="F"), np.empty(nx)
        check(lib().ace_fit_predict(self._h, _p(X2), _p(Z2), nx, float(mean_y), float(std_y), _p(m), _p(ci), _p(var)),
              "ace_fit_predict")
        return {"map": m, "ci": ci, "var": var}

    def predict_marginal(self, X2, Z2, dZ2, mean_y=0.0, std_y=1.0, std_Z=1.0, calculate_ate=False):
        X2, Z2, dZ2 = _f(X2, True), _f(Z2, True), _f(dZ2, True)
        nx = X2.shape[0]
        m, ci, var, avg = np.empty(nx), np.empty((nx, 2), order="F"), np.empty(nx), np.zeros(12)
        check(lib().ace_fit_predict_marginal(self._h, _p(X2), _p(Z2), _p(dZ2), nx, float(mean_y), float(std_y),
                                             float(std_Z), int(bool(calculate_ate)), _p(m), _p(ci), _p(var), _p(avg)),
              "ace_fit_predict_marginal")
        out = {"map": m, "ci": ci, "var": var}
        if calculate_ate:
            for k, name in enumerate(("ate", "att", "atu")):
                out[name] = {"map": avg[4 * k], "ci": avg[4 * k + 1:4 * k + 3].copy(), "var": avg[4 * k + 3]}
        return out

    def predict_marginal_batch(self, X2, Z2, dZ2, subsets, mean_y=0.0, std_y=1.0, std_Z=1.0):
        X2, Z2, dZ2 = _f(X2, True), _f(Z2, True), _f(dZ2, True)
        nx = X2.shape[0]
        sub = np.asfortranarray(np.asarray(subsets).reshape(nx, -1).astype(np.uint8))
        S = sub.shape[1]
        m, ci, var = np.empty(nx), np.empty((nx, 2), order="F"), np.empty(nx)
        avg, cnt = np.zeros((S, 12)), np.zeros((S, 3), dtype=np.int32)
        check(lib().ace_fit_predict_marginal_batch(
            self._h, _p(X2), _p(Z2), _p(dZ2), nx, float(mean_y), float(std_y), float(std_Z),
            sub.ctypes.data_as(C.POINTER(C.c_ubyte)), S, _p(m), _p(ci), _p(var), _p(avg),
            cnt.ctypes.data_as(C.POINTER(C.c_int))), "ace_fit_predict_marginal_batch")
        out = {"map": m, "ci": ci, "var": var, "subsets": []}
        for s in range(S):
            d = {"n": int(cnt[s, 0]), "n_treated": int(cnt[s, 1]), "n_untreated": int(cnt[s, 2])}
            for k, name in enumerate(("ate", "att", "atu")):
                d[name] = {"map": avg[s, 4 * k], "ci": avg[s, 4 * k + 1:4 * k + 3].copy(), "var": avg[s, 4 * k + 3]}
            out["subsets"].append(d)
        return out
```

include/ace_b200.h:

```cpp
#ifndef ACE_B200_H
#define ACE_B200_H

#ifdef __cplusplus
extern "C" {
#endif

#define ACE_OK 0
#define ACE_ERR_NOT_FINITE 1073741824
#define ACE_ERR_USAGE (-1)
#define ACE_ERR_NO_DEVICE (-3)
#define ACE_ERR_UNSUPPORTED (-4)

#define ACE_KERNEL_SE 0
#define ACE_KERNEL_MATERN32 1
#define ACE_OPT_NADAM 0
#define ACE_OPT_ADAM 1
#define ACE_OPT_NESTEROV 2

const char* ace_last_error(void);
const char* ace_version(void);
int ace_device_count(void);
int ace_set_device(int device);


int ace_kernmat_SE_cpp(const double* X1, const double* X2, const double* Z1, const double* Z2, int n1, int n2,
                       int p, int Bz, const double* parameters, double* full, double* elements);
int ace_kernmat_Matern32_cpp(const double* X1, const double* X2, const double* Z1, const double* Z2, int n1,
                             int n2, int p, int Bz, const double* parameters, double* full, double* elements);

int ace_kernmat_SE_symmetric_cpp(const double* X, const double* Z, int n, int p, int Bz,
                                 const double* parameters, double* full, double* elements);
int ace_kernmat_Matern32_symmetric_cpp(const double* X, const double* Z, int n, int p, int Bz,
                                       const double* parameters, double* full, double* elements);

int ace_invkernel_cpp(const double* pdmat, int n, double sigma, double* eigenval, double* inv);

int ace_grad_SE_cpp(const double* y, const double* X, const double* Z, const double* Kfull, const double* K,
                    const double* invKmatn, const double* eigenval, const double* parameters, double* stats,
                    unsigned int B, double std_y, int n, int p, double* gradients);
int ace_grad_Matern_cpp(const double* y, const double* X, const double* Z, const double* Kfull, const double* K,
                        const double* invKmatn, const double* eigenval, const double* parameters, double* stats,
                        unsigned int B, double std_y, int n, int p, double* gradients);

int ace_stats_cpp(const double* y, const double* Kmat, const double* invKmatn, const double* eigenval, double mu,
                  double std_y, int n, double* out);

int ace_mu_solution_cpp(const double* y, const double* invKmat, int n, double* mu);

int ace_pred_cpp(const double* y_X, double sigma, double mu, const double* invK_XX, const double* K_xX,
                 const double* K_xx, double mean_y, double std_y, int nx, int nX, double* map, double* ci,
                 double* var);

int ace_pred_marginal_cpp(const double* y_X, const double* Z_x, double sigma, double mu, const double* invK_XX,
                          const double* K_xX, const double* K_xx, double mean_y, double std_y, double std_Z,
                          int calculate_ate, int nx, int nX, int B, double* map, double* ci, double* var,
                          double* avg);

void ace_norm_clip_cpp(int flag, double* grads, int P, double max_length);
int ace_Nesterov_cpp(double learn_rate, double momentum, double* nu, const double* grad, double* para, int P);
int ace_Nadam_cpp(double iter, double learn_rate, double beta1, double beta2, double eps, double* m, double* v,
                  const double* grad, double* para, int P);
int ace_Adam_cpp(double iter, double learn_rate, double beta1, double beta2, double eps, double* m, double* v,
                 const double* grad, double* para, int P);

typedef struct ace_fit ace_fit;

typedef struct ace_fit_config {
  int kernel;
  int optimizer;
  double learning_rate, beta1, beta2, momentum;
  int norm_clip;
  double clip_at;
  double std_y;
  int device;
  int use_graph;
} ace_fit_config;

void ace_fit_default_config(ace_fit_config* cfg);

int ace_fit_create(ace_fit** out, const double* y, const double* X, const double* Z, int n, int p, int Bz,
                   const double* parameters, const ace_fit_config* cfg);
int ace_fit_destroy(ace_fit* fit);

int ace_fit_para_update(ace_fit* fit, int iter, double* stats, double* gnorm);

int ace_fit_run(ace_fit* fit, int iter_start, int max_iter, double tol, double prev_evidence, double* stats_out,
                int* iters_done);

int ace_fit_get_train_stats(ace_fit* fit, double* stats);

int ace_comm_unique_id(char* id128);
int ace_shard_plan(int n, int world, int rank, int* blocks2, int* width);
int ace_fit_shard(ace_fit* fit, const char* id128, int rank, int world);
int ace_fit_shard_emulate(ace_fit* fit, int world);
int ace_dbg_shard_trace_dump(int rank);

int ace_fit_upload_data(ace_fit* fit, const double* y, const double* X, const double* Z);
int ace_fit_kernel_launches(ace_fit* fit, int* launches);
int ace_fit_timer_start(ace_fit* fit);
int ace_fit_timer_stop(ace_fit* fit, double* ms);

int ace_fit_get_parameters(ace_fit* fit, double* parameters);
int ace_fit_set_parameters(ace_fit* fit, const double* parameters);
int ace_fit_get_gradients(ace_fit* fit, double* gradients);
int ace_fit_get_optimizer_state(ace_fit* fit, double* m, double* v);
int ace_fit_get_invKmatn(ace_fit* fit, double* inv);
int ace_fit_get_alpha(ace_fit* fit, double* alpha);
int ace_fit_dims(ace_fit* fit, int* n, int* p, int* B, int* P);
int ace_fit_last_timing(ace_fit* fit, double* ms6);

int ace_fit_predict(ace_fit* fit, const double* X2, const double* Z2, int nx, double mean_y, double std_y,
                    double* map, double* ci, double* var);
int ace_fit_predict_marginal(ace_fit* fit, const double* X2, const double* Z2, const double* dZ2, int nx,
                             double mean_y, double std_y, double std_Z, int calculate_ate, double* map,
                             double* ci, double* var, double* avg);
int ace_fit_predict_marginal_batch(ace_fit* fit, const double* X2, const double* Z2, const double* dZ2, int nx,
                                   double mean_y, double std_y, double std_Z, const unsigned char* subsets, int S,
                                   double* map, double* ci, double* var, double* avg, int* counts);

int ace_dbg_gemm_nt(const double* A, const double* B, double* C, int M, int N, int K, double alpha, double beta,
                    int lower_only);
int ace_dbg_spd_inverse(const double* A, int n, double* L, double* inv, double* diagL, double* ms3);
int ace_bench_dense(int n, int reps, double* ms3);
int ace_dbg_spd_inverse_fused(const double* A, int n, double* inv, double* diagL);
int ace_dbg_diag_block(const double* A, int n, double* X, double* U, double* diagL, double* Ldiag_tiles);
int ace_dbg_diag_block_timeline(long long* stamps, int count);
int ace_dbg_set_trtri_max_h(int h);
int ace_dbg_trtri_raw(const double* A, int n, double* rawA, double* DX, double* DU, double* rawBf);
int ace_dbg_uut_engines(const double* A, int n, const int* engines, int count, double* ms, double* inv_dmma,
                        double* inv_i8);
int ace_dbg_fit_set_uut_engine(ace_fit* fit, int engine);

int ace_ncs_basis(const double* x, int n, const double* knots, int nknots, double* design);
int ace_ncs_basis_deriv(const double* x, int n, const double* knots, int nknots, double* design);
int ace_normalize_train(double* y, double* X, double* Z, int n, int px, int pz, double* moments);
int ace_normalize_test(double* X, double* Z, int n, int px, int pz, const double* moments);
int ace_normalize_train_gpu(double* y, double* X, double* Z, int n, int px, int pz, double* moments);
int ace_normalize_test_gpu(double* X, double* Z, int n, int px, int pz, const double* moments);

#ifdef __cplusplus
}
#endif
#endif
```

Measured before the change: 7.617.

## Route large triangular-inverse merge GEMMs through the INT8 Ozaki digit-plane engine

Generalizes the INT8 Ozaki-split U·U^T kernel into a batched general oz_gemm (dense/triangular operands, strides, alpha, optional transpose write, k-balancing scaling) and uses it for the trtri merge levels at h >= 32 when n_pad is between 16384 and the INT32 bound. It also splits the digit-plane workspace between the forked left and right trtri subtrees and drops env-var knobs. The aim is to replace FP64 DMMA work in the recursive triangular inverse with INT8 tensor-core work. The risks are extra split, colmax and scaling passes, more workspace, and accuracy limits of the emulation. Small problems keep the old path.

```diff
diff --git a/additivecausalexpansion_b200/_lib.py b/additivecausalexpansion_b200/_lib.py
--- a/additivecausalexpansion_b200/_lib.py
+++ b/additivecausalexpansion_b200/_lib.py
@@ -99,6 +99,8 @@
     "ace_dbg_trtri_raw": (_i, [_p, _i, _p, _p, _p, _p]),
     "ace_dbg_uut_engines": (_i, [_p, _i, C.POINTER(C.c_int), _i, _p, _p, _p]),
     "ace_dbg_fit_set_uut_engine": (_i, [_vp, _i]),
+    "ace_dbg_trtri_engines": (_i, [_p, _i, C.POINTER(C.c_int), _i, _i, _p, _p, _p, _p, _p]),
+    "ace_dbg_fit_set_trtri_engine": (_i, [_vp, _i]),
     "ace_ncs_basis": (_i, [_p, _i, _p, _i, _p]),
     "ace_ncs_basis_deriv": (_i, [_p, _i, _p, _i, _p]),
     "ace_normalize_train": (_i, [_p, _p, _p, _i, _i, _i, _p]),
diff --git a/additivecausalexpansion_b200/api.py b/additivecausalexpansion_b200/api.py
--- a/additivecausalexpansion_b200/api.py
+++ b/additivecausalexpansion_b200/api.py
@@ -237,6 +237,23 @@
     return {"ms": ms, "dmma": inv[1], "i8": inv[2]}
 
 
+def dbg_trtri_engines(A, engines=(1, 2), per_level=False, want_inv=True):
+    A = _f(A)
+    n = A.shape[0]
+    eng = (C.c_int * len(engines))(*engines)
+    nb = -(-n // 128)
+    levels, h = 0, 4
+    while h < nb:
+        levels += 1
+        h *= 2
+    ms = np.zeros((len(engines), levels if per_level else 1))
+    inv = {e: (np.empty((n, n), order="F") if want_inv and e in engines else None) for e in (1, 2)}
+    dl = {e: (np.empty(n) if e in engines else None) for e in (1, 2)}
+    check(lib().ace_dbg_trtri_engines(_p(A), n, eng, len(engines), int(per_level), _p(ms), _p(inv[1]), _p(inv[2]),
+                                      _p(dl[1]), _p(dl[2])), "dbg_trtri_engines")
+    return {"ms": ms if per_level else ms[:, 0], "dmma": inv[1], "i8": inv[2], "diagL_dmma": dl[1], "diagL_i8": dl[2]}
+
+
 def dbg_diag_block(A):
     A = _f(A)
     n = A.shape[0]
diff --git a/additivecausalexpansion_b200/csrc/ace_b200.cu b/additivecausalexpansion_b200/csrc/ace_b200.cu
--- a/additivecausalexpansion_b200/csrc/ace_b200.cu
+++ b/additivecausalexpansion_b200/csrc/ace_b200.cu
@@ -353,7 +353,11 @@
   DBuf<int8_t> oz_planes;
   DBuf<unsigned long long> oz_rowmax;
   DBuf<int> oz_ex;
+  DBuf<unsigned long long> oz_colmax;
+  DBuf<int> oz_ks;
+  size_t oz_bytes = 0;
   int uut_engine = 0;
+  int trtri_engine = 0;
   int panel_blocks = 4;
   cudaEvent_t tev[8] = {};
   DBuf<double> X, Z, LZ, y, theta, m, v, grad, tab, sc, A, Bf, DX, DU, dvec, alpha, uvec, svec, Ka, pu, ps, partials;
@@ -555,20 +559,29 @@
   }
 
   int alloc_uut_engine() {
-    if (uut_engine == 2 && n_pad > oz::MAX_N) {
-      set_error("the INT8 U U^T engine covers n_pad <= " + std::to_string(oz::MAX_N) + " (INT32 accumulator bound)");
+    if ((uut_engine == 2 || trtri_engine == 2) && n_pad > oz::MAX_N) {
+      set_error("the INT8 engine covers n_pad <= " + std::to_string(oz::MAX_N) + " (INT32 accumulator bound)");
       return ACE_ERR_UNSUPPORTED;
     }
-    if (!uut_uses_i8(n_pad, uut_engine)) {
+    const int nb = n_pad / TB;
+    const size_t need = std::max(uut_uses_i8(n_pad, uut_engine) ? uut_i8_bytes(nb) : 0, trtri_i8_bytes(nb, trtri_engine));
+    if (need == 0) {
       oz_planes.release();
       oz_rowmax.release();
       oz_ex.release();
+      oz_colmax.release();
+      oz_ks.release();
+      oz_bytes = 0;
       return 0;
     }
-    if (oz_planes.p) return 0;
-    ACE_TRY(oz_planes.alloc(oz::plane_bytes(n_pad / TB)));
-    ACE_TRY(oz_rowmax.alloc(n_pad));
-    ACE_TRY(oz_ex.alloc(n_pad));
+    if (oz_planes.p && oz_bytes >= need) return 0;
+    oz_planes.release();
+    ACE_TRY(oz_planes.alloc(need));
+    oz_bytes = need;
+    if (!oz_rowmax.p) ACE_TRY(oz_rowmax.alloc(n_pad));
+    if (!oz_ex.p) ACE_TRY(oz_ex.alloc(n_pad));
+    if (!oz_colmax.p) ACE_TRY(oz_colmax.alloc(2 * (size_t)n_pad));
+    if (!oz_ks.p) ACE_TRY(oz_ks.alloc(n_pad));
     return 0;
   }
 
@@ -599,7 +612,10 @@
     w.A = Abuf; w.ld = n_pad; w.nb = n_pad / TB; w.DX = DX.p; w.DU = DU.p; w.dvec = dvec.p; w.info = info.p;
     w.Bf = Bbuf; w.main = st; w.side = side; w.aux = aux; w.bg = bgst; w.ev_half = ev[4]; w.ev_aux = ev[5];
     w.ev_panel[0] = ev[0]; w.ev_panel[1] = ev[1]; w.ev_upd[0] = ev[2]; w.ev_upd[1] = ev[3];
-    w.oz.planes = oz_planes.p; w.oz.rowmax = oz_rowmax.p; w.oz.ex = oz_ex.p; w.uut_engine = uut_engine;
+    w.oz.planes = oz_planes.p; w.oz.bytes = oz_bytes; w.oz.rowmax = oz_rowmax.p; w.oz.ex = oz_ex.p;
+    w.oz.colmax = oz_colmax.p; w.oz.ks = oz_ks.p;
+    w.oz.rows = oz_rowmax.p ? n_pad : 0;
+    w.uut_engine = uut_engine; w.trtri_engine = trtri_engine;
 
     return w;
   }
@@ -977,19 +993,32 @@
   return 0;
 }
 
-int ace_dbg_fit_set_uut_engine(ace_fit* f, int engine) {
+static int fit_set_engine(ace_fit* f, int engine, int* slot, const char* what) {
   if (!f) return usage("null handle");
-  if (engine < 0 || engine > 2) return usage("dbg_fit_set_uut_engine: engine must be 0 (by size), 1 (DMMA) or 2 (INT8)");
+  if (engine < 0 || engine > 2) return usage(std::string(what) + ": engine must be 0 (by size), 1 (DMMA) or 2 (INT8)");
   Core& c = f->c;
   ACE_CUDA(cudaSetDevice(c.device));
   ACE_CUDA(cudaStreamSynchronize(c.st));
-  c.uut_engine = engine;
-  ACE_TRY(c.alloc_uut_engine());
+  const int old = *slot;
+  *slot = engine;
+  const int rc = c.alloc_uut_engine();
+  if (rc != 0) {
+    *slot = old;
+    return rc;
+  }
   if (f->gexec) cudaGraphExecDestroy(f->gexec);
   if (f->graph) cudaGraphDestroy(f->graph);
   f->gexec = nullptr;
   f->graph = nullptr;
   return 0;
+}
+
+int ace_dbg_fit_set_uut_engine(ace_fit* f, int engine) {
+  return fit_set_engine(f, engine, f ? &f->c.uut_engine : nullptr, "dbg_fit_set_uut_engine");
+}
+
+int ace_dbg_fit_set_trtri_engine(ace_fit* f, int engine) {
+  return fit_set_engine(f, engine, f ? &f->c.trtri_engine : nullptr, "dbg_fit_set_trtri_engine");
 }
 
 int ace_fit_get_train_stats(ace_fit* f, double* stats) {
diff --git a/additivecausalexpansion_b200/csrc/chol.cuh b/additivecausalexpansion_b200/csrc/chol.cuh
--- a/additivecausalexpansion_b200/csrc/chol.cuh
+++ b/additivecausalexpansion_b200/csrc/chol.cuh
@@ -4,6 +4,7 @@
 #include "diag_block.cuh"
 #include "uut_i8.cuh"
 
+#include <algorithm>
 #include <cstdlib>
 #include <vector>
 
@@ -274,6 +275,7 @@
   long long* diag_dbg = nullptr;
   OzWork oz;
   int uut_engine = 0;
+  int trtri_engine = 0;
 };
 
 inline int configure_dense_kernels() {
@@ -284,7 +286,7 @@
   ACE_CUDA(cudaFuncSetAttribute(trsm_leaf_kernel, cudaFuncAttributeMaxDynamicSharedMemorySize,
                                 (int)trsml::SMEM_BYTES));
   ACE_TRY(configure_diag_kernel());
-  ACE_TRY(configure_uut_i8_kernel());
+  ACE_TRY(configure_oz_gemm_kernel());
   return 0;
 }
 
@@ -327,7 +329,8 @@
   return potrf_rec(w, c, b, st);
 }
 
-inline int trtri_merge_range(const DenseWork& w, int lo, int hi, cudaStream_t st, double* ws, int h_min = 1);
+inline int trtri_merge_range(const DenseWork& w, int lo, int hi, cudaStream_t st, double* ws, int h_min = 1,
+                             const OzWork* oz = nullptr, int i8_h = 1 << 30);
 
 inline int diag_block_factor_invert(const DenseWork& w, int j0, int j1, cudaStream_t st, int share = 1) {
   if (w.diag_ws != nullptr) {
@@ -343,7 +346,8 @@
   return trtri_merge_range(w, j0, j1, st, w.Wsmall);
 }
 
-inline int potrf_blocked(const DenseWork& w, int fork_at = 0, int fork_when = 0, bool incremental = false) {
+inline int potrf_blocked(const DenseWork& w, int fork_at = 0, int fork_when = 0, bool incremental = false,
+                         const OzWork* fork_oz = nullptr, int fork_i8_h = 1 << 30) {
   const int nb = w.nb, pb = w.panel_blocks;
   bool forked = false;
   ACE_CUDA(cudaMemsetAsync(w.info, 0, sizeof(int), w.main));
@@ -411,7 +415,7 @@
     if (fork_at > 0 && !forked && j1 >= fork_at && j1 >= fork_when && j1 < nb) {
       ACE_CUDA(cudaEventRecord(w.ev_half, w.side));
       ACE_CUDA(cudaStreamWaitEvent(w.aux, w.ev_half, 0));
-      ACE_TRY(trtri_merge_range(w, 0, fork_at, w.aux, w.Bf, w.Wp[0] ? w.panel_blocks : 1));
+      ACE_TRY(trtri_merge_range(w, 0, fork_at, w.aux, w.Bf, w.Wp[0] ? w.panel_blocks : 1, fork_oz, fork_i8_h));
       ACE_CUDA(cudaEventRecord(w.ev_aux, w.aux));
       forked = true;
     }
@@ -441,81 +445,153 @@
   return v;
 }
 
-inline int trtri_level(const DenseWork& w, int lo, int len, int h, cudaStream_t st, double* ws) {
-  const int nodes = (len + 2 * h - 1) / (2 * h);
-  const int s1 = h * TB;
+struct MergeGroup {
+  int a, c, q0, cnt, s1, s2;
+};
+inline int merge_groups(int lo, int len, int h, MergeGroup (&g)[2]) {
+  const int nodes = (len + 2 * h - 1) / (2 * h), s1 = h * TB;
   int nreg = 0;
   while (nreg < nodes && (nreg * 2 * h + 2 * h) <= len) ++nreg;
-  for (int pass = 0; pass < 2; ++pass) {
-    int q0, cnt, s2;
-    if (pass == 0) {
-      q0 = 0; cnt = nreg; s2 = s1;
-    } else {
-      q0 = nreg; cnt = nodes - nreg;
-      if (cnt == 0) break;
-      const int c_local = q0 * 2 * h + h;
-      if (c_local >= len) break;
-      s2 = (len - c_local) * TB;
-    }
-    if (cnt == 0) continue;
-    const int a = lo + q0 * 2 * h, c = a + h;
+  int count = 0;
+  if (nreg > 0) g[count++] = {lo, lo + h, 0, nreg, s1, s1};
+  const int c_local = nreg * 2 * h + h;
+  if (nreg < nodes && c_local < len)
+    g[count++] = {lo + nreg * 2 * h, lo + c_local, nreg, 1, s1, (len - c_local) * TB};
+  return count;
+}
+
+inline void merge_oz_products(const DenseWork& w, const MergeGroup& m, double* Wt, OzGemm& p, OzGemm& r) {
+  const long node_stride = (long)2 * (m.c - m.a) * TB * (w.ld + 1), tile_stride = (long)2 * (m.c - m.a) * TB * TB;
+  p = OzGemm{};
+  p.a.A = blkptr(w, m.a, m.a); p.a.ld = w.ld; p.a.D = w.DU + (size_t)m.a * TB * TB; p.a.tri = oz::UPPER;
+  p.a.rows = p.a.K = m.s1; p.a.sA = node_stride; p.a.sD = tile_stride;
+  p.b.A = blkptr(w, m.c, m.a); p.b.ld = w.ld; p.b.rows = m.s2; p.b.K = m.s1; p.b.sA = node_stride;
+  p.C = Wt; p.ldc = m.s1; p.sC = (long)m.s1 * m.s1; p.alpha = 1.0;
+  r = OzGemm{};
+  r.a.A = blkptr(w, m.c, m.c); r.a.ld = w.ld; r.a.D = w.DX + (size_t)m.c * TB * TB; r.a.tri = oz::LOWER;
+  r.a.rows = r.a.K = m.s2; r.a.sA = node_stride; r.a.sD = tile_stride;
+  r.b.A = Wt; r.b.ld = m.s1; r.b.rows = m.s1; r.b.K = m.s2; r.b.sA = (long)m.s1 * m.s1;
+  r.C = blkptr(w, m.c, m.a); r.ldc = w.ld; r.sC = node_stride;
+  r.Ct = blkptr(w, m.a, m.c); r.ldct = w.ld; r.sCt = node_stride;
+  r.alpha = -1.0;
+}
+
+inline int trtri_level(const DenseWork& w, int lo, int len, int h, cudaStream_t st, double* ws,
+                       const OzWork* oz = nullptr) {
+  MergeGroup g[2];
+  const int count = merge_groups(lo, len, h, g);
+  for (int k = 0; k < count; ++k) {
+    const MergeGroup& m = g[k];
+    double* Wt = ws + (size_t)m.q0 * m.s1 * m.s1;
+    if (oz != nullptr) {
+      OzGemm p, r;
+      merge_oz_products(w, m, Wt, p, r);
+      ACE_TRY(launch_oz_gemm(p, m.cnt, false, *oz, st));
+      ACE_TRY(launch_oz_gemm(r, m.cnt, false, *oz, st, true));
+      continue;
+    }
     const long node_stride = (long)2 * h * TB * (w.ld + 1);
-    double* Wt = ws + (size_t)q0 * s1 * s1;
     GemmNT p{};
-    p.A = blkptr(w, a, a); p.lda = w.ld; p.a_tri = 1; p.Adiag = w.DU + (size_t)a * TB * TB;
-    p.B = blkptr(w, c, a); p.ldb = w.ld;
-    p.C = Wt; p.ldc = s1;
-    p.M = s1; p.N = s2; p.K = s1; p.alpha = 1.0; p.beta = 0.0;
-    p.batch = cnt; p.sA = node_stride; p.sB = node_stride; p.sC = (long)s1 * s1;
+    p.A = blkptr(w, m.a, m.a); p.lda = w.ld; p.a_tri = 1; p.Adiag = w.DU + (size_t)m.a * TB * TB;
+    p.B = blkptr(w, m.c, m.a); p.ldb = w.ld;
+    p.C = Wt; p.ldc = m.s1;
+    p.M = m.s1; p.N = m.s2; p.K = m.s1; p.alpha = 1.0; p.beta = 0.0;
+    p.batch = m.cnt; p.sA = node_stride; p.sB = node_stride; p.sC = (long)m.s1 * m.s1;
     p.sAdiag = (long)2 * h * TB * TB;
     ACE_TRY(launch_gemm_nt(p, st));
     GemmNT r{};
-    r.A = blkptr(w, c, c); r.lda = w.ld; r.a_tri = 2; r.Adiag = w.DX + (size_t)c * TB * TB;
-    r.B = Wt; r.ldb = s1;
-    r.C = blkptr(w, c, a); r.ldc = w.ld;
-    r.Ct = blkptr(w, a, c); r.ldct = w.ld;
-    r.M = s2; r.N = s1; r.K = s2; r.alpha = -1.0; r.beta = 0.0;
-    r.batch = cnt; r.sA = node_stride; r.sB = (long)s1 * s1; r.sC = node_stride; r.sCt = node_stride;
+    r.A = blkptr(w, m.c, m.c); r.lda = w.ld; r.a_tri = 2; r.Adiag = w.DX + (size_t)m.c * TB * TB;
+    r.B = Wt; r.ldb = m.s1;
+    r.C = blkptr(w, m.c, m.a); r.ldc = w.ld;
+    r.Ct = blkptr(w, m.a, m.c); r.ldct = w.ld;
+    r.M = m.s2; r.N = m.s1; r.K = m.s2; r.alpha = -1.0; r.beta = 0.0;
+    r.batch = m.cnt; r.sA = node_stride; r.sB = (long)m.s1 * m.s1; r.sC = node_stride; r.sCt = node_stride;
     r.sAdiag = (long)2 * h * TB * TB;
     ACE_TRY(launch_gemm_nt(r, st));
   }
   return 0;
 }
 
-inline int trtri_merge_range(const DenseWork& w, int lo, int hi, cudaStream_t st, double* ws, int h_min) {
-  for (int h = h_min; h < hi - lo && h <= dbg_trtri_max_h(); h *= 2) ACE_TRY(trtri_level(w, lo, hi - lo, h, st, ws));
+inline int trtri_merge_range(const DenseWork& w, int lo, int hi, cudaStream_t st, double* ws, int h_min,
+                             const OzWork* oz, int i8_h) {
+  for (int h = h_min; h < hi - lo && h <= dbg_trtri_max_h(); h *= 2)
+    ACE_TRY(trtri_level(w, lo, hi - lo, h, st, ws, (oz != nullptr && h >= i8_h) ? oz : nullptr));
   return 0;
 }
 
+inline size_t merge_i8_bytes(int len, int i8_h) {
+  DenseWork w{};
+  size_t need = 0;
+  for (int h = 1; h < len; h *= 2) {
+    if (h < i8_h) continue;
+    MergeGroup g[2];
+    const int count = merge_groups(0, len, h, g);
+    for (int k = 0; k < count; ++k) {
+      OzGemm p, r;
+      merge_oz_products(w, g[k], nullptr, p, r);
+      need = std::max(need, std::max(p.a.plane_bytes(g[k].cnt) + p.b.plane_bytes(g[k].cnt),
+                                     r.a.plane_bytes(g[k].cnt) + r.b.plane_bytes(g[k].cnt)));
+    }
+  }
+  return need;
+}
+
 inline int trtri_hmin(const DenseWork& w) { return w.Wp[0] ? w.panel_blocks : 1; }
 
-inline int trtri_merge(const DenseWork& w) { return trtri_merge_range(w, 0, w.nb, w.main, w.Bf, trtri_hmin(w)); }
-
-inline int potrf_trtri(const DenseWork& w) {
-  const int nb = w.nb;
+constexpr int TRTRI_I8_MIN_N = 16384;
+constexpr int TRTRI_I8_MIN_H = 32;
+
+inline int trtri_i8_min_h(int n_pad, int engine) {
+  if (engine == 2) return 1;
+  if (engine == 0 && n_pad >= TRTRI_I8_MIN_N && n_pad <= oz::MAX_N) return TRTRI_I8_MIN_H;
+  return 1 << 30;
+}
+
+inline int trtri_top_child(int nb) {
   int h_top = 1;
   while (2 * h_top < nb) h_top *= 2;
+  return h_top;
+}
+
+inline size_t trtri_i8_bytes(int nb, int engine) {
+  const int i8_h = trtri_i8_min_h(nb * TB, engine), h_top = trtri_top_child(nb);
+  if (i8_h >= nb) return 0;
+  return std::max(merge_i8_bytes(nb, i8_h), merge_i8_bytes(h_top, i8_h) + merge_i8_bytes(nb - h_top, i8_h));
+}
+
+inline int trtri_merge(const DenseWork& w) {
+  return trtri_merge_range(w, 0, w.nb, w.main, w.Bf, trtri_hmin(w), &w.oz, trtri_i8_min_h(w.nb * TB, w.trtri_engine));
+}
+
+inline int potrf_trtri(const DenseWork& w) {
+  const int nb = w.nb, h_top = trtri_top_child(nb), i8_h = trtri_i8_min_h(nb * TB, w.trtri_engine);
   if (nb < 8 || w.aux == nullptr || dbg_trtri_max_h() < (1 << 30)) {
     int s = potrf_blocked(w);
     if (s < 0) return s;
     return trtri_merge(w);
   }
-  static const int incr = std::getenv("ACE_INCR_TRTRI") ? std::atoi(std::getenv("ACE_INCR_TRTRI")) : 1;
-  if (incr && w.Wp[0] != nullptr) {
+  if (i8_h >= nb && w.Wp[0] != nullptr) {
     const int forked = potrf_blocked(w, 0, 0, true);
     if (forked < 0) return forked;
     if (forked) ACE_CUDA(cudaStreamWaitEvent(w.main, w.ev_aux, 0));
     return 0;
   }
-  double frac = 0.75;
-  if (const char* e = std::getenv("ACE_FORK_FRAC")) frac = std::atof(e);
-  const int forked = potrf_blocked(w, h_top, (int)(frac * nb));
+  constexpr double FORK_FRAC = 0.75;
+  OzWork left = w.oz, right = w.oz;
+  const size_t lb = std::min(w.oz.bytes, merge_i8_bytes(h_top, i8_h));
+  left.bytes = lb; left.rows = (long)h_top * TB;
+  right.planes = w.oz.planes ? w.oz.planes + lb : nullptr; right.bytes = w.oz.bytes - lb;
+  right.rowmax = w.oz.rowmax ? w.oz.rowmax + left.rows : nullptr; right.ex = w.oz.ex ? w.oz.ex + left.rows : nullptr;
+  right.colmax = w.oz.colmax ? w.oz.colmax + 2 * left.rows : nullptr; right.ks = w.oz.ks ? w.oz.ks + left.rows : nullptr;
+  right.rows = std::max(0L, w.oz.rows - left.rows);
+  const int h_min = trtri_hmin(w);
+  const int forked = potrf_blocked(w, h_top, (int)(FORK_FRAC * nb), false, &left, i8_h);
   if (forked < 0) return forked;
   const size_t left_ws = (size_t)(h_top * TB / 2) * (h_top * TB / 2);
-  if (!forked) ACE_TRY(trtri_merge_range(w, 0, h_top, w.main, w.Bf, trtri_hmin(w)));
-  ACE_TRY(trtri_merge_range(w, h_top, nb, w.main, w.Bf + left_ws, trtri_hmin(w)));
+  if (!forked) ACE_TRY(trtri_merge_range(w, 0, h_top, w.main, w.Bf, h_min, &left, i8_h));
+  ACE_TRY(trtri_merge_range(w, h_top, nb, w.main, w.Bf + left_ws, h_min, &right, i8_h));
   if (forked) ACE_CUDA(cudaStreamWaitEvent(w.main, w.ev_aux, 0));
-  return trtri_level(w, 0, nb, h_top, w.main, w.Bf);
+  return trtri_level(w, 0, nb, h_top, w.main, w.Bf, h_top >= i8_h ? &w.oz : nullptr);
 }
 
 constexpr int UUT_I8_MIN_N = 8192;
diff --git a/additivecausalexpansion_b200/csrc/shard_dense.cuh b/additivecausalexpansion_b200/csrc/shard_dense.cuh
--- a/additivecausalexpansion_b200/csrc/shard_dense.cuh
+++ b/additivecausalexpansion_b200/csrc/shard_dense.cuh
@@ -542,7 +542,7 @@
       ACE_TRY(trtri_level_sharded(w, 0, w.nb, h, w.main, w.Bf, cx, true));
     else {
       shard_trace().level_mark(-h, 0, w.main);
-      ACE_TRY(trtri_level(w, 0, w.nb, h, w.main, w.Bf));
+      ACE_TRY(trtri_level(w, 0, w.nb, h, w.main, w.Bf, nullptr));
       for (int k = 1; k < 5; ++k) shard_trace().level_mark(-h, k, w.main);
     }
   }
diff --git a/additivecausalexpansion_b200/csrc/uut_i8.cuh b/additivecausalexpansion_b200/csrc/uut_i8.cuh
--- a/additivecausalexpansion_b200/csrc/uut_i8.cuh
+++ b/additivecausalexpansion_b200/csrc/uut_i8.cuh
@@ -21,13 +21,14 @@
 static_assert((long)S * DMAX * DMAX * MAX_N <= 2147483647L, "INT32 accumulators may overflow");
 constexpr uint32_t IDESC = (2u << 4) | (1u << 7) | (1u << 10) | ((uint32_t)(BN >> 3) << 17) | ((uint32_t)(BM >> 4) << 24);
 
-__host__ __device__ inline size_t block_off(int nb, int t, int rb, int c) {
-  const long nc = (long)nb * CPB;
-  const long per_plane = (long)nb * nc - (long)CPB * nb * (nb - 1) / 2;
-  const long off = (long)rb * nc - (long)CPB * rb * (rb - 1) / 2 + (c - (long)CPB * rb);
-  return ((size_t)t * per_plane + off) * (size_t)(BM * BK);
-}
-inline size_t plane_bytes(int nb) { return block_off(nb, S, 0, 0); }
+enum { DENSE = 0, UPPER = 1, LOWER = 2 };
+__host__ __device__ inline int chunk_lo(int tri, int rb) { return tri == UPPER ? CPB * rb : 0; }
+__host__ __device__ inline int chunk_hi(int tri, int nkc, int rb) { return tri == LOWER ? CPB * (rb + 1) : nkc; }
+__host__ __device__ inline long blocks_before(int tri, int nkc, int rb) {
+  if (tri == UPPER) return (long)rb * nkc - (long)CPB * rb * (rb - 1) / 2;
+  if (tri == LOWER) return (long)CPB * rb * (rb + 1) / 2;
+  return (long)rb * nkc;
+}
 }
 
 __device__ __forceinline__ uint64_t oz_smem_desc(uint32_t saddr) {
@@ -60,44 +61,90 @@
       : "memory");
 }
 
-__device__ __forceinline__ double oz_u(const double* A, long ld, const double* DU, int rb, int cb, int r, int kk) {
-  return (cb == rb) ? DU[(size_t)rb * TB * TB + r + (size_t)kk * TB] : A[(size_t)rb * TB + r + (size_t)(cb * TB + kk) * ld];
-}
-
-__global__ void __launch_bounds__(128) oz_rowmax_kernel(const double* __restrict__ A, long ld,
-                                                        const double* __restrict__ DU,
-                                                        unsigned long long* __restrict__ rowmax) {
-  const int cb = blockIdx.x, rb = blockIdx.y, r = threadIdx.x;
-  if (cb < rb) return;
+struct OzOperand {
+  const double* A;
+  long ld;
+  const double* D;
+  int tri;
+  int rows, K;
+  long sA, sD;
+  const int* ks;
+  int ks_sign;
+  int8_t* planes;
+  unsigned long long* rowmax;
+  int* ex;
+  __host__ __device__ int nkc() const { return K / oz::BK; }
+  __host__ __device__ long per_plane() const { return oz::blocks_before(tri, nkc(), rows / TB); }
+  __host__ __device__ size_t block_off(int q, int t, int rb, int c) const {
+    return (((size_t)q * oz::S + t) * per_plane() + oz::blocks_before(tri, nkc(), rb) + (c - oz::chunk_lo(tri, rb))) *
+           (size_t)(oz::BM * oz::BK);
+  }
+  size_t plane_bytes(int batch) const { return (size_t)batch * oz::S * per_plane() * (oz::BM * oz::BK); }
+};
+
+__device__ __forceinline__ double oz_raw(const OzOperand& o, int q, int rb, int kb, int r, int kk) {
+  if (o.tri != oz::DENSE && kb == rb) return o.D[q * o.sD + (size_t)rb * TB * TB + r + (size_t)kk * TB];
+  return o.A[q * o.sA + (size_t)rb * TB + r + (size_t)(kb * TB + kk) * o.ld];
+}
+__device__ __forceinline__ double oz_elem(const OzOperand& o, int q, int rb, int kb, int r, int kk) {
+  const double v = oz_raw(o, q, rb, kb, r, kk);
+  return o.ks ? ldexp(v, o.ks_sign * o.ks[(size_t)q * o.K + kb * TB + kk]) : v;
+}
+
+__device__ __forceinline__ bool oz_skip_block(const OzOperand& o, int rb, int kb) {
+  return kb * oz::CPB < oz::chunk_lo(o.tri, rb) || kb * oz::CPB >= oz::chunk_hi(o.tri, o.nkc(), rb);
+}
+
+__global__ void __launch_bounds__(128) oz_rowmax_kernel(const OzOperand o) {
+  const int kb = blockIdx.x, rb = blockIdx.y, q = blockIdx.z, r = threadIdx.x;
+  if (oz_skip_block(o, rb, kb)) return;
   double m = 0.0;
 #pragma unroll 8
-  for (int kk = 0; kk < TB; ++kk) m = fmax(m, fabs(oz_u(A, ld, DU, rb, cb, r, kk)));
-  atomicMax(rowmax + rb * TB + r, (unsigned long long)__double_as_longlong(m));
-}
-
-__global__ void __launch_bounds__(128) oz_split_kernel(const double* __restrict__ A, long ld,
-                                                       const double* __restrict__ DU,
-                                                       const unsigned long long* __restrict__ rowmax, int nb,
-                                                       int8_t* __restrict__ planes, int* __restrict__ ex) {
+  for (int kk = 0; kk < TB; ++kk) m = fmax(m, fabs(oz_elem(o, q, rb, kb, r, kk)));
+  atomicMax(o.rowmax + (size_t)q * o.rows + rb * TB + r, (unsigned long long)__double_as_longlong(m));
+}
+
+__global__ void __launch_bounds__(128) oz_colmax_kernel(const OzOperand o, unsigned long long* __restrict__ colmax) {
+  const int kb = blockIdx.x, rb = blockIdx.y, q = blockIdx.z, kk = threadIdx.x;
+  if (oz_skip_block(o, rb, kb)) return;
+  double m = 0.0;
+#pragma unroll 8
+  for (int r = 0; r < TB; ++r) m = fmax(m, fabs(oz_raw(o, q, rb, kb, r, kk)));
+  atomicMax(colmax + (size_t)q * o.K + kb * TB + kk, (unsigned long long)__double_as_longlong(m));
+}
+
+__global__ void oz_kscale_kernel(const unsigned long long* __restrict__ ca, const unsigned long long* __restrict__ cb,
+                                 int* __restrict__ ks, long count) {
+  const long k = (long)blockIdx.x * blockDim.x + threadIdx.x;
+  if (k >= count) return;
+  const double a = __longlong_as_double((long long)ca[k]), b = __longlong_as_double((long long)cb[k]);
+  int ea = 0, eb = 0;
+  frexp(a, &ea);
+  frexp(b, &eb);
+  ks[k] = (a > 0.0 && b > 0.0) ? (eb - ea) >> 1 : 0;
+}
+
+__global__ void __launch_bounds__(128) oz_split_kernel(const OzOperand o) {
   using namespace oz;
-  const int cb = blockIdx.x, rb = blockIdx.y, r = threadIdx.x;
-  if (cb < rb) return;
-  const double m = __longlong_as_double((long long)rowmax[rb * TB + r]);
+  const int kb = blockIdx.x, rb = blockIdx.y, q = blockIdx.z, r = threadIdx.x;
+  if (oz_skip_block(o, rb, kb)) return;
+  const size_t row = (size_t)q * o.rows + rb * TB + r;
+  const double m = __longlong_as_double((long long)o.rowmax[row]);
   int e = 0;
   if (m > 0.0) {
     frexp(m, &e);
     ++e;
   }
-  if (cb == rb) ex[rb * TB + r] = e;
+  if (kb * CPB == chunk_lo(o.tri, rb)) o.ex[row] = e;
   const double scale = ldexp(1.0, -e);
 #pragma unroll 1
-  for (int q = 0; q < TB / 16; ++q) {
+  for (int h = 0; h < TB / 16; ++h) {
     uint32_t w[S][4];
 #pragma unroll
     for (int t = 0; t < S; ++t) w[t][0] = w[t][1] = w[t][2] = w[t][3] = 0u;
 #pragma unroll
     for (int x16 = 0; x16 < 16; ++x16) {
-      double x = oz_u(A, ld, DU, rb, cb, r, q * 16 + x16) * scale;
+      double x = oz_elem(o, q, rb, kb, r, h * 16 + x16) * scale;
 #pragma unroll
       for (int t = 0; t < S; ++t) {
         x *= 128.0;
@@ -106,17 +153,25 @@
         w[t][x16 >> 2] |= ((uint32_t)(int)d & 0xffu) << (8 * (x16 & 3));
       }
     }
-    const int c = cb * CPB + q / 2;
-    const size_t in_blk = (size_t)(r >> 3) * 256 + (q & 1) * 128 + (r & 7) * 16;
+    const int c = kb * CPB + h / 2;
+    const size_t in_blk = (size_t)(r >> 3) * 256 + (h & 1) * 128 + (r & 7) * 16;
 #pragma unroll
     for (int t = 0; t < S; ++t)
-      *reinterpret_cast<uint4*>(planes + block_off(nb, t, rb, c) + in_blk) = make_uint4(w[t][0], w[t][1], w[t][2], w[t][3]);
-  }
-}
-
-__global__ void __launch_bounds__(oz::THREADS, 1) uut_i8_kernel(const int8_t* __restrict__ planes,
-                                                                const int* __restrict__ ex, int nb,
-                                                                double* __restrict__ C, long ldc) {
+      *reinterpret_cast<uint4*>(o.planes + o.block_off(q, t, rb, c) + in_blk) = make_uint4(w[t][0], w[t][1], w[t][2], w[t][3]);
+  }
+}
+
+struct OzGemm {
+  OzOperand a, b;
+  double* C;
+  long ldc, sC;
+  double* Ct;
+  long ldct, sCt;
+  double alpha;
+  int lower_only;
+};
+
+__global__ void __launch_bounds__(oz::THREADS, 1) oz_gemm_i8_kernel(const OzGemm p) {
   using namespace oz;
   extern __shared__ unsigned char smem_raw[];
   unsigned char* sm = reinterpret_cast<unsigned char*>((reinterpret_cast<uintptr_t>(smem_raw) + 1023) & ~uintptr_t(1023));
@@ -125,18 +180,31 @@
   uint64_t* done = empty + STAGES;
   uint32_t* tmem_slot = reinterpret_cast<uint32_t*>(done + 1);
   const int warp = threadIdx.x >> 5, lane = threadIdx.x & 31;
+  const int q = blockIdx.y;
 
   int ti, tj;
   {
     const long L = blockIdx.x;
-    long t = (long)((sqrt(4.0 * (double)L + 1.0) - 1.0) * 0.5);
-    while (t * (t + 1) > L) --t;
-    while ((t + 1) * (t + 2) <= L) ++t;
-    ti = (int)t;
-    tj = (int)(L - t * (t + 1));
+    if (p.lower_only) {
+      long t = (long)((sqrt(4.0 * (double)L + 1.0) - 1.0) * 0.5);
+      while (t * (t + 1) > L) --t;
+      while ((t + 1) * (t + 2) <= L) ++t;
+      ti = (int)t;
+      tj = (int)(L - t * (t + 1));
+    } else {
+      constexpr int GROUP = 8;
+      const int tiles_m = p.a.rows / BM, tiles_n = p.b.rows / BN;
+      const long per_group = (long)GROUP * tiles_n;
+      const int first_m = (int)(L / per_group) * GROUP;
+      const int gsize = min(GROUP, tiles_m - first_m);
+      const int r = (int)(L % per_group);
+      ti = first_m + r % gsize;
+      tj = r / gsize;
+    }
   }
   const int i0 = ti * BM, j0 = tj * BN, jb = tj >> 1, jh = tj & 1;
-  const int c_begin = ti * CPB, nchunks = nb * CPB - c_begin;
+  const int c_begin = max(chunk_lo(p.a.tri, ti), chunk_lo(p.b.tri, jb));
+  const int nchunks = min(chunk_hi(p.a.tri, p.a.nkc(), ti), chunk_hi(p.b.tri, p.b.nkc(), jb)) - c_begin;
 
   if (threadIdx.x == 0) {
     for (int s = 0; s < STAGES; ++s) {
@@ -159,19 +227,21 @@
 
   if (warp == 0) {
     if (lane == 0) {
+      const int8_t* a_src = p.a.planes + p.a.block_off(q, 0, ti, c_begin);
+      const int8_t* b_src = p.b.planes + p.b.block_off(q, 0, jb, c_begin) + jh * B_PLANE;
+      const size_t a_plane = (size_t)p.a.per_plane() * (BM * BK), b_plane = (size_t)p.b.per_plane() * (BM * BK);
       for (int it = 0; it < nchunks; ++it) {
         const int s = it % STAGES;
         mbar_wait(&empty[s], ((it / STAGES) & 1) ^ 1);
         mbar_arrive_expect_tx(&full[s], STAGE_BYTES);
         unsigned char* st = sm + (size_t)s * STAGE_BYTES;
-        const int c = c_begin + it;
+        const size_t step = (size_t)it * (BM * BK);
 #pragma unroll
         for (int t = 0; t < S; ++t)
-          tma_bulk_g2s(st + t * A_PLANE, planes + block_off(nb, t, ti, c), A_PLANE, &full[s]);
+          tma_bulk_g2s(st + t * A_PLANE, a_src + step + t * a_plane, A_PLANE, &full[s]);
 #pragma unroll
         for (int t = 0; t < S; ++t)
-          tma_bulk_g2s(st + S * A_PLANE + t * B_PLANE, planes + block_off(nb, t, jb, c) + jh * B_PLANE, B_PLANE,
-                       &full[s]);
+          tma_bulk_g2s(st + S * A_PLANE + t * B_PLANE, b_src + step + t * b_plane, B_PLANE, &full[s]);
       }
     }
     __syncwarp();
@@ -196,10 +266,12 @@
   } else {
     mbar_wait(done, 0);
     tc_fence_after();
-    const int q = warp & 3;
-    const int r = q * 32 + lane, i = i0 + r;
-    const int ei = ex[i] - 14;
-    const uint32_t trow = tmem + ((uint32_t)(q * 32) << 16);
+    const int qd = warp & 3;
+    const int r = qd * 32 + lane, i = i0 + r;
+    const int ei = p.a.ex[(size_t)q * p.a.rows + i] - 14;
+    const int* exb = p.b.ex + (size_t)q * p.b.rows;
+    double* C = p.C + q * p.sC;
+    const uint32_t trow = tmem + ((uint32_t)(qd * 32) << 16);
 #pragma unroll 1
     for (int jc = 0; jc < BN / 16; ++jc) {
       uint32_t v[S][16];
@@ -213,12 +285,14 @@
 #pragma unroll
         for (int g = S - 2; g >= 0; --g) acc = fma(acc, 0x1p-7, (double)(int)v[g][j]);
         const int col = j0 + jc * 16 + j;
-        out[j] = ldexp(acc, ei + ex[col]);
-        C[(size_t)col * ldc + i] = out[j];
-      }
-      double2* ct = reinterpret_cast<double2*>(C + (size_t)i * ldc + j0 + jc * 16);
-#pragma unroll
-      for (int j = 0; j < 8; ++j) ct[j] = make_double2(out[2 * j], out[2 * j + 1]);
+        out[j] = nchunks > 0 ? p.alpha * ldexp(acc, ei + exb[col]) : 0.0;
+        C[(size_t)col * p.ldc + i] = out[j];
+      }
+      if (p.Ct != nullptr) {
+        double2* ct = reinterpret_cast<double2*>(p.Ct + q * p.sCt + (size_t)i * p.ldct + j0 + jc * 16);
+#pragma unroll
+        for (int j = 0; j < 8; ++j) ct[j] = make_double2(out[2 * j], out[2 * j + 1]);
+      }
     }
   }
   tc_fence_before();
@@ -231,36 +305,91 @@
 
 struct OzWork {
   int8_t* planes = nullptr;
+  size_t bytes = 0;
   unsigned long long* rowmax = nullptr;
   int* ex = nullptr;
+  unsigned long long* colmax = nullptr;
+  int* ks = nullptr;
+  long rows = 0;
 };
 
-inline int configure_uut_i8_kernel() {
-  ACE_CUDA(cudaFuncSetAttribute(uut_i8_kernel, cudaFuncAttributeMaxDynamicSharedMemorySize, (int)oz::SMEM_BYTES));
+inline size_t uut_i8_bytes(int nb) {
+  OzOperand u{};
+  u.tri = oz::UPPER; u.rows = u.K = nb * TB;
+  return u.plane_bytes(1);
+}
+
+inline int configure_oz_gemm_kernel() {
+  ACE_CUDA(cudaFuncSetAttribute(oz_gemm_i8_kernel, cudaFuncAttributeMaxDynamicSharedMemorySize, (int)oz::SMEM_BYTES));
   return 0;
 }
 
-inline int launch_uut_i8(const OzWork& o, const double* A, const double* DU, int nb, double* C, cudaStream_t st) {
-  using namespace oz;
-  if ((long)nb * TB > MAX_N) {
-    set_error("uut_i8: n_pad beyond the INT32 accumulator bound");
-    return -2;
-  }
-  if (!o.planes || !o.rowmax || !o.ex) {
-    set_error("uut_i8: digit-plane workspace not allocated");
-    return -2;
-  }
-  const long ld = (long)nb * TB;
-  ACE_CUDA(cudaMemsetAsync(o.rowmax, 0, sizeof(unsigned long long) * (size_t)ld, st));
-  const dim3 g2(nb, nb);
-  oz_rowmax_kernel<<<g2, TB, 0, st>>>(A, ld, DU, o.rowmax);
+inline int oz_split(const OzOperand& o, int batch, cudaStream_t st) {
+  ACE_CUDA(cudaMemsetAsync(o.rowmax, 0, sizeof(unsigned long long) * (size_t)batch * o.rows, st));
+  const dim3 g(o.K / TB, o.rows / TB, batch);
+  oz_rowmax_kernel<<<g, TB, 0, st>>>(o);
   ACE_CUDA(cudaGetLastError());
-  oz_split_kernel<<<g2, TB, 0, st>>>(A, ld, DU, o.rowmax, nb, o.planes, o.ex);
-  ACE_CUDA(cudaGetLastError());
-  const long tiles = (long)nb * (nb + 1);
-  uut_i8_kernel<<<(unsigned)tiles, THREADS, SMEM_BYTES, st>>>(o.planes, o.ex, nb, C, ld);
+  oz_split_kernel<<<g, TB, 0, st>>>(o);
   ACE_CUDA(cudaGetLastError());
   return 0;
 }
 
-}
+inline int launch_oz_gemm(OzGemm p, int batch, bool same, const OzWork& o, cudaStream_t st, bool kbalance = false) {
+  using namespace oz;
+  batch = batch > 1 ? batch : 1;
+  if (p.a.K != p.b.K || p.a.K > MAX_N || p.a.rows % TB || p.b.rows % TB || p.a.K % TB ||
+      (p.a.tri != DENSE && p.a.rows != p.a.K) || (p.b.tri != DENSE && p.b.rows != p.b.K)) {
+    set_error("oz_gemm: operand shapes outside the INT8 engine (multiples of 128, K <= " + std::to_string(MAX_N) +
+              ", triangular operands square)");
+    return -2;
+  }
+  const size_t abytes = p.a.plane_bytes(batch), bbytes = same ? 0 : p.b.plane_bytes(batch);
+  const long arows = (long)batch * p.a.rows, brows = same ? 0 : (long)batch * p.b.rows;
+  if (!o.planes || abytes + bbytes > o.bytes || arows + brows > o.rows) {
+    set_error("oz_gemm: digit-plane workspace too small");
+    return -2;
+  }
+  p.a.ks = p.b.ks = nullptr;
+  if (kbalance) {
+    const long kc = (long)batch * p.a.K;
+    if (same || !o.colmax || !o.ks || kc > o.rows) {
+      set_error("oz_gemm: k balance needs two operands and its workspace");
+      return -2;
+    }
+    ACE_CUDA(cudaMemsetAsync(o.colmax, 0, sizeof(unsigned long long) * 2 * (size_t)kc, st));
+    const dim3 ga(p.a.K / TB, p.a.rows / TB, batch), gb(p.b.K / TB, p.b.rows / TB, batch);
+    oz_colmax_kernel<<<ga, TB, 0, st>>>(p.a, o.colmax);
+    ACE_CUDA(cudaGetLastError());
+    oz_colmax_kernel<<<gb, TB, 0, st>>>(p.b, o.colmax + kc);
+    ACE_CUDA(cudaGetLastError());
+    oz_kscale_kernel<<<(unsigned)((kc + 255) / 256), 256, 0, st>>>(o.colmax, o.colmax + kc, o.ks, kc);
+    ACE_CUDA(cudaGetLastError());
+    p.a.ks = p.b.ks = o.ks;
+    p.a.ks_sign = 1;
+    p.b.ks_sign = -1;
+  }
+  p.a.planes = o.planes; p.a.rowmax = o.rowmax; p.a.ex = o.ex;
+  ACE_TRY(oz_split(p.a, batch, st));
+  if (same) {
+    p.b.planes = p.a.planes; p.b.rowmax = p.a.rowmax; p.b.ex = p.a.ex;
+  } else {
+    p.b.planes = o.planes + abytes; p.b.rowmax = o.rowmax + arows; p.b.ex = o.ex + arows;
+    ACE_TRY(oz_split(p.b, batch, st));
+  }
+  const long T = p.a.rows / BM;
+  const long tiles = p.lower_only ? T * (T + 1) : T * (p.b.rows / BN);
+  oz_gemm_i8_kernel<<<dim3((unsigned)tiles, (unsigned)batch), THREADS, SMEM_BYTES, st>>>(p);
+  ACE_CUDA(cudaGetLastError());
+  return 0;
+}
+
+inline int launch_uut_i8(const OzWork& o, const double* A, const double* DU, int nb, double* C, cudaStream_t st) {
+  OzGemm p{};
+  p.a.A = A; p.a.ld = (long)nb * TB; p.a.D = DU; p.a.tri = oz::UPPER; p.a.rows = p.a.K = nb * TB;
+  p.b = p.a;
+  p.C = C; p.ldc = (long)nb * TB; p.Ct = C; p.ldct = p.ldc;
+  p.alpha = 1.0; p.lower_only = 1;
+  return launch_oz_gemm(p, 1, true, o, st);
+}
+
+}
diff --git a/additivecausalexpansion_b200/fit.py b/additivecausalexpansion_b200/fit.py
--- a/additivecausalexpansion_b200/fit.py
+++ b/additivecausalexpansion_b200/fit.py
@@ -117,6 +117,9 @@
     def dbg_set_uut_engine(self, engine):
         check(lib().ace_dbg_fit_set_uut_engine(self._h, int(engine)), "ace_dbg_fit_set_uut_engine")
 
+    def dbg_set_trtri_engine(self, engine):
+        check(lib().ace_dbg_fit_set_trtri_engine(self._h, int(engine)), "ace_dbg_fit_set_trtri_engine")
+
     def get_train_stats(self):
         st = np.zeros(2)
         check(lib().ace_fit_get_train_stats(self._h, _p(st)), "ace_fit_get_train_stats")
diff --git a/include/ace_b200.h b/include/ace_b200.h
--- a/include/ace_b200.h
+++ b/include/ace_b200.h
@@ -130,6 +130,9 @@
 int ace_dbg_uut_engines(const double* A, int n, const int* engines, int count, double* ms, double* inv_dmma,
                         double* inv_i8);
 int ace_dbg_fit_set_uut_engine(ace_fit* fit, int engine);
+int ace_dbg_trtri_engines(const double* A, int n, const int* engines, int count, int per_level, double* ms,
+                          double* inv_dmma, double* inv_i8, double* diagL_dmma, double* diagL_i8);
+int ace_dbg_fit_set_trtri_engine(ace_fit* fit, int engine);
 
 int ace_ncs_basis(const double* x, int n, const double* knots, int nknots, double* design);
 int ace_ncs_basis_deriv(const double* x, int n, const double* knots, int nknots, double* design);
```

Result: faster. 8.366, median of 6 (+9.8%).
